# yifangao112/DinoUNet

Measured on AMD Instinct MI355X. Metric: 2D slices/sec training, dinounet_l 512x512 bf16, higher is better.
Workload: dtype bf16; 1 GPU; dinounet_l train step (fwd+loss+bwd+clip+SGD), 512x512x3 slices, batch 8/GPU, frozen ViT + adapter + FAPM + U-Net decoder, random-init weights; global_batch=8, parallelism=dp1

## Files before the change

### dinounet_amd/_build.py

```python
import hashlib
import os
import subprocess
import sys

HERE = os.path.dirname(os.path.abspath(__file__))
CSRC = os.path.join(HERE, "csrc")
LIB = os.path.join(HERE, "libdinounet_hip.so")
SOURCES = ["gemm.hip", "gemm_bf16.hip", "gemm_glds.hip", "gemm_p8.hip", "gemm_rk.hip", "gemm_skinny.hip", "conv_halo.hip", "conv_strip.hip", "attention.hip", "norm.hip", "norm_gemm.hip", "msda.hip", "elementwise.hip", "dwconv.hip", "loss.hip", "optim.hip", "augment.hip", "export.hip", "ensemble.hip", "surface.hip", "cc.hip", "preprocess.hip", "dataload.hip", "fingerprint.hip"]
FLAGS = ["--offload-arch=gfx950", "-O3", "-std=c++17", "-fPIC", "-munsafe-fp-atomics", "-fno-gpu-rdc"]
if os.environ.get("DINOUNET_DEBUG_KNOBS") == "1":
    FLAGS.append("-DDU_DEBUG_KNOBS")
EXTRA_FLAGS = {"attention.hip": ["-mllvm", "-amdgpu-mfma-vgpr-form"], "conv_strip.hip": ["-mllvm", "-amdgpu-mfma-vgpr-form"]}
NO_SCRATCH = ("gemm_bf16.hip", "gemm_glds.hip", "gemm_p8.hip", "gemm_rk.hip", "gemm_skinny.hip", "conv_halo.hip", "conv_strip.hip", "attention.hip", "norm_gemm.hip", "surface.hip", "dwconv.hip", "cc.hip", "preprocess.hip", "dataload.hip", "fingerprint.hip", "ensemble.hip")
REMARK = "-Rpass-analysis=kernel-resource-usage"
import re as _re
_ABLATION = _re.compile(
    r"attn_fwd_kernelILi\d+ELb1EEE"
    r"|attn_fwd_w64_kernelILi\d+ELi\d+ELb1E"
    r"|attn_fwd_w64_kernelILi\d+ELi\d+ELb\dELi\d+ELi[1-9]\d*ELi\d+EEE"
    r"|attn_fwd_pipe_kernelILb1ELi\d+EEE|attn_fwd_pipe_kernelILb\dELi[1-9]\d*EEE")


def _digest():
    h = hashlib.sha256()
    for f in sorted(os.listdir(CSRC)) + ["../../include/dinounet_hip.h"]:
        p = os.path.join(CSRC, f)
        if os.path.isfile(p):
            h.update(f.encode())
            h.update(open(p, "rb").read())
    h.update(" ".join(FLAGS).encode())
    h.update(repr(sorted(EXTRA_FLAGS.items())).encode())
    return h.hexdigest()


def build(force: bool = False, verbose: bool = True) -> str:
    stamp = LIB + ".stamp"
    dig = _digest()
    if not force and os.path.exists(LIB) and os.path.exists(stamp) and open(stamp).read() == dig:
        return LIB
    hipcc = os.environ.get("HIPCC", "/opt/rocm/bin/hipcc")
    objs, procs = [], []
    os.makedirs(os.path.join(HERE, "build"), exist_ok=True)
    for s in SOURCES:
        o = os.path.join(HERE, "build", s.replace(".hip", ".o"))
        objs.append(o)
        cmd = [hipcc, *FLAGS, *EXTRA_FLAGS.get(s, []), *([REMARK] if s in NO_SCRATCH else []), "-c", os.path.join(CSRC, s), "-o", o]
        if verbose:
            print("[dinounet_amd build]", " ".join(cmd), flush=True)
        procs.append((s, subprocess.Popen(cmd, stdout=subprocess.PIPE, stderr=subprocess.STDOUT)))
    for s, p in procs:
        out, _ = p.communicate()
        if p.returncode != 0:
            sys.stderr.write(out.decode())
            raise RuntimeError(f"hipcc failed on {s}")
        if s in NO_SCRATCH:
            name, spills = None, []
            for ln in out.decode().splitlines():
                if "Function Name:" in ln:
                    name = ln.split("Function Name:")[1].split("[")[0].strip()
                elif "ScratchSize [bytes/lane]:" in ln and int(ln.split("ScratchSize [bytes/lane]:")[1].split("[")[0]) > 0 and not _ABLATION.search(name or ""):
                    spills.append(f"{name} ({ln.split('ScratchSize [bytes/lane]:')[1].split('[')[0].strip()} B/lane)")
            if spills:
                raise RuntimeError(f"{s}: kernels spill to scratch: " + "; ".join(spills[:6]))
    cmd = [hipcc, "--offload-arch=gfx950", "-shared", "-fPIC", *objs, "-o", LIB]
    subprocess.check_call(cmd)
    und = subprocess.run(["nm", "-D", "--undefined-only", LIB], capture_output=True, text=True).stdout
    bad = [ln.split()[-1] for ln in und.splitlines() if "_GLOBAL__N_" in ln or ("_Z" in ln and "du_" in ln)]
    if bad:
        os.remove(LIB)
        raise RuntimeError("undefined file-local symbols in libdinounet_hip.so (dropped kernel stubs?): " + ", ".join(bad[:4]))
    open(stamp, "w").write(dig)
    return LIB


if __name__ == "__main__":
    print(build(force="--force" in sys.argv))
```

### dinounet_amd/csrc/gemm_p8.hip

```cpp
#include <algorithm>
#include <vector>
#include "common.h"
#include "gemm_params.h"
#include "gemm_plan.h"
#include "gemm_skinny_body.h"

namespace {

typedef __attribute__((address_space(3))) void lds_void;

constexpr int PBM = 256, PBN = 256, PBK = 64;
constexpr int HALF_B = 128 * PBK * 2;
constexpr int BUF_B = 4 * HALF_B;
constexpr int STG_LD = PBN + 4;

template <typename TC> struct Out4p;
template <> struct Out4p<float> {
  static __device__ __forceinline__ void load(const float* p, float* v) { float4 t = *(const float4*)p; v[0] = t.x; v[1] = t.y; v[2] = t.z; v[3] = t.w; }
  static __device__ __forceinline__ void store(float* p, const float* v) { *(float4*)p = make_float4(v[0], v[1], v[2], v[3]); }
};
template <> struct Out4p<bf16_t> {
  static __device__ __forceinline__ void load(const bf16_t* p, float* v) {
    bf16x4 t = __builtin_bit_cast(bf16x4, *(const uint2*)p);
#pragma unroll
    for (int j = 0; j < 4; j++) v[j] = (float)t[j];
  }
  static __device__ __forceinline__ void store(bf16_t* p, const float* v) {
    bf16x4 t;
#pragma unroll
    for (int j = 0; j < 4; j++) t[j] = (bf16_t)v[j];
    *(uint2*)p = __builtin_bit_cast(uint2, t);
  }
};

typedef unsigned u32x4_t __attribute__((ext_vector_type(4)));
template <int N> struct IC { static constexpr int value = N; };

__device__ __forceinline__ void wait_vm_count(int n) {
  switch (n) {
    case 12: asm volatile("s_waitcnt vmcnt(12)" ::: "memory"); break;
    case 10: asm volatile("s_waitcnt vmcnt(10)" ::: "memory"); break;
    case 8: asm volatile("s_waitcnt vmcnt(8)" ::: "memory"); break;
    case 6: asm volatile("s_waitcnt vmcnt(6)" ::: "memory"); break;
    case 4: asm volatile("s_waitcnt vmcnt(4)" ::: "memory"); break;
    case 2: asm volatile("s_waitcnt vmcnt(2)" ::: "memory"); break;
    default: asm volatile("s_waitcnt vmcnt(0)" ::: "memory"); break;
  }
}

__device__ __forceinline__ void tile_coords_of(const GemmParams& P, int nwg, int bid, int& tm, int& tn);
__device__ __forceinline__ void tile_coords(const GemmParams& P, int& tm, int& tn) {
  tile_coords_of(P, P.main_wgs ? P.main_wgs : (int)gridDim.x, blockIdx.x, tm, tn);
}
__device__ __forceinline__ void tile_coords_of(const GemmParams& P, int nwg, int bid, int& tm, int& tn) {
  const int q = nwg >> 3, r = nwg & 7, xcd = bid & 7, idx = bid >> 3;
  const int tile = (xcd < r ? xcd * (q + 1) : r * (q + 1) + (xcd - r) * q) + idx;
  if (P.group_m > 1) {
    const int band = P.group_m * P.tiles_n;
    const int g = tile / band, l = tile - g * band;
    const int first = g * P.group_m;
    const int gsz = min(P.tiles_m - first, P.group_m);
    tn = l / gsz; tm = first + (l - tn * gsz);
  } else {
    tm = tile / P.tiles_n; tn = tile - tm * P.tiles_n;
  }
}


typedef float f32x2 __attribute__((ext_vector_type(2)));
__device__ __forceinline__ f32x2 splat2(float c) { f32x2 r; r.x = c; r.y = c; return r; }
__device__ __forceinline__ f32x2 gelu_pk(f32x2 v) {
  f32x2 u, m, e;
  u.x = __builtin_amdgcn_fmed3f(fabsf(v.x), 0.f, 5.6f); u.y = __builtin_amdgcn_fmed3f(fabsf(v.y), 0.f, 5.6f);
  m.x = __builtin_amdgcn_fmed3f(v.x, 0.f, __builtin_inff()); m.y = __builtin_amdgcn_fmed3f(v.y, 0.f, __builtin_inff());
  f32x2 q = splat2(-1.99582904e-06f);
  q = q * u + splat2(6.48327432e-05f);
  q = q * u + splat2(-9.56180914e-04f);
  q = q * u + splat2(8.60978469e-03f);
  q = q * u + splat2(-5.41717858e-02f);
  q = q * u + splat2(-4.58246213e-01f);
  q = q * u + splat2(-1.15134465e+00f);
  q = q * u + splat2(-9.99985061e-01f);
  e.x = __builtin_amdgcn_exp2f(q.x); e.y = __builtin_amdgcn_exp2f(q.y);
  return m - u * e;
}

template <int ACT>
__device__ __forceinline__ void stage_block_bf16(const f32x16& a, const float4 (&bv)[4], bf16_t* stg, int ldb, int srow, int scol, int hi) {
#pragma unroll
  for (int g = 0; g < 4; g++) {
    float o[4] = {a[4 * g] + bv[g].x, a[4 * g + 1] + bv[g].y, a[4 * g + 2] + bv[g].z, a[4 * g + 3] + bv[g].w};
    if constexpr (ACT == DU_ACT_SWIGLU) {
      bf16x2 t;
      t[0] = (bf16_t)(o[0] * __builtin_amdgcn_rcpf(1.0f + __expf(-o[0])) * o[1]);
      t[1] = (bf16_t)(o[2] * __builtin_amdgcn_rcpf(1.0f + __expf(-o[2])) * o[3]);
      *(unsigned*)(stg + srow * ldb + ((scol + 8 * g + 4 * hi) >> 1)) = __builtin_bit_cast(unsigned, t);
    } else {
      if constexpr (ACT == DU_ACT_GELU) {
        f32x2 p0 = {o[0], o[1]}, p1 = {o[2], o[3]};
        p0 = gelu_pk(p0); p1 = gelu_pk(p1);
        o[0] = p0.x; o[1] = p0.y; o[2] = p1.x; o[3] = p1.y;
      }
      bf16x4 t;
#pragma unroll
      for (int e = 0; e < 4; e++) t[e] = (bf16_t)o[e];
      *(uint2*)(stg + srow * ldb + scol + 8 * g + 4 * hi) = __builtin_bit_cast(uint2, t);
    }
  }
}
__device__ __forceinline__ void stage_head_rope(const GemmParams& P, const f32x16& lo, const f32x16& hi_, const float4 (&blo)[4],
                                                const float4 (&bhi)[4], bf16_t* stg, int ldb, int srow, int scol, int hi, int m, int which) {
  const int b = m / P.ps_H, t = m - b * P.ps_H;
  const bool rot = which < 2 && t >= P.rope_prefix && m < P.M;
  const float qs = which == 0 ? P.rope_qscale : 1.0f;
  const long trow = rot ? (long)(t - P.rope_prefix) * 64 : 0;
#pragma unroll
  for (int g = 0; g < 4; g++) {
    const int d = 8 * g + 4 * hi;
    float x1[4] = {lo[4 * g] + blo[g].x, lo[4 * g + 1] + blo[g].y, lo[4 * g + 2] + blo[g].z, lo[4 * g + 3] + blo[g].w};
    float x2[4] = {hi_[4 * g] + bhi[g].x, hi_[4 * g + 1] + bhi[g].y, hi_[4 * g + 2] + bhi[g].z, hi_[4 * g + 3] + bhi[g].w};
    float o1[4], o2[4];
    if (rot) {
      const float4 c1 = *(const float4*)(P.rope_cos + trow + d), s1 = *(const float4*)(P.rope_sin + trow + d);
      const float4 c2 = *(const float4*)(P.rope_cos + trow + 32 + d), s2 = *(const float4*)(P.rope_sin + trow + 32 + d);
      const float cc1[4] = {c1.x, c1.y, c1.z, c1.w}, ss1[4] = {s1.x, s1.y, s1.z, s1.w};
      const float cc2[4] = {c2.x, c2.y, c2.z, c2.w}, ss2[4] = {s2.x, s2.y, s2.z, s2.w};
#pragma unroll
      for (int e = 0; e < 4; e++) { o1[e] = x1[e] * cc1[e] - x2[e] * ss1[e]; o2[e] = x2[e] * cc2[e] + x1[e] * ss2[e]; }
    } else {
#pragma unroll
      for (int e = 0; e < 4; e++) { o1[e] = x1[e]; o2[e] = x2[e]; }
    }
    bf16x4 t1, t2;
#pragma unroll
    for (int e = 0; e < 4; e++) { t1[e] = (bf16_t)(o1[e] * qs); t2[e] = (bf16_t)(o2[e] * qs); }
    *(uint2*)(stg + srow * ldb + scol + d) = __builtin_bit_cast(uint2, t1);
    *(uint2*)(stg + srow * ldb + scol + 32 + d) = __builtin_bit_cast(uint2, t2);
  }
}
__device__ __forceinline__ void load_bias4(const GemmParams& P, int ncol0, int hi, float4 (&bv)[4]) {
#pragma unroll
  for (int g = 0; g < 4; g++) {
    const int n = ncol0 + 8 * g + 4 * hi;
    bv[g] = P.bias ? *(const float4*)(P.bias + (n < P.N ? n : 0)) : make_float4(0.f, 0.f, 0.f, 0.f);
  }
}
__device__ __forceinline__ void stage_block_f32(const f32x16& a, float* stg, int ldf, int srow, int scol, int lane) {
  const int hi = lane >> 5;
#pragma unroll
  for (int g = 0; g < 4; g++)
    *(float4*)(stg + srow * ldf + scol + 8 * g + 4 * hi) = make_float4(a[4 * g], a[4 * g + 1], a[4 * g + 2], a[4 * g + 3]);
}
template <int TBN, bool QKV = false, int NTHR = 512>
__device__ __forceinline__ void readout_bf16(const GemmParams& P, const bf16_t* stg, int ldb, int nrows, int mrow0, int n0, int ncols,
                                             bf16_t* Cb, int tid) {
  constexpr int C8 = TBN / 8;
  const bool wide = ((((uintptr_t)Cb) & 15) == 0) && P.ldc % 8 == 0 && (QKV || P.store_mode == DU_STORE_PLAIN || P.ps_C % 8 == 0);
#pragma unroll 4
  for (int v = tid; v < nrows * C8; v += NTHR) {
    const int row = v / C8, c8 = v % C8;
    const int m = mrow0 + row, n = n0 + c8 * 8;
    if (m >= P.M || n >= ncols) continue;
    const uint4 t = *(const uint4*)(stg + row * ldb + c8 * 8);
    if ((P.dbg & 1) && t.x != 0x12345678u) continue;
    bf16_t* dst = Cb + (QKV ? qkv_heads_offset(P, m, n, P.ldc) : out_offset(P, m, n, P.ldc));
    if (wide && n + 8 <= ncols) *(uint4*)dst = t;
    else {
      *(uint2*)dst = make_uint2(t.x, t.y);
      if (n + 4 < ncols) *(uint2*)(dst + 4) = make_uint2(t.z, t.w);
    }
  }
}
template <typename TC, int W> struct RowVec;
template <> struct RowVec<float, 4> {
  static __device__ __forceinline__ void load(const float* p, float* v) { const float4 t = *(const float4*)p; v[0] = t.x; v[1] = t.y; v[2] = t.z; v[3] = t.w; }
  static __device__ __forceinline__ void store(float* p, const float* v) { *(float4*)p = make_float4(v[0], v[1], v[2], v[3]); }
};
template <> struct RowVec<bf16_t, 4> {
  static __device__ __forceinline__ void load(const bf16_t* p, float* v) { Out4p<bf16_t>::load(p, v); }
  static __device__ __forceinline__ void store(bf16_t* p, const float* v) { Out4p<bf16_t>::store(p, v); }
};
template <> struct RowVec<bf16_t, 8> {
  static __device__ __forceinline__ void load(const bf16_t* p, float* v) {
    const bf16x8 t = __builtin_bit_cast(bf16x8, *(const uint4*)p);
#pragma unroll
    for (int j = 0; j < 8; j++) v[j] = (float)t[j];
  }
  static __device__ __forceinline__ void store(bf16_t* p, const float* v) {
    bf16x8 t;
#pragma unroll
    for (int j = 0; j < 8; j++) t[j] = (bf16_t)v[j];
    *(uint4*)p = __builtin_bit_cast(uint4, t);
  }
};

template <typename TC, int TBN, int ACT, int W, int NTHR = 512>
__device__ __forceinline__ void readout_f32(const GemmParams& P, const float* stg, int ldf, int nrows, int mrow0, int n0, TC* Cb, const TC* Rb,
                                            int tid) {
  constexpr int CW = TBN / W, U = W == 8 ? 2 : 4;
  const int total = nrows * CW;
  for (int v0 = tid; v0 < total; v0 += NTHR * U) {
    float rr[U][W];
    bool live[U];
#pragma unroll
    for (int u = 0; u < U; u++) {
      const int v = v0 + u * NTHR;
      const int row = v / CW, cw = v % CW;
      const int m = mrow0 + row, n = n0 + cw * W;
      live[u] = v < total && m < P.M && n < P.N;
#pragma unroll
      for (int e = 0; e < W; e++) rr[u][e] = 0.f;
      if (Rb && live[u]) RowVec<TC, W>::load(Rb + out_offset(P, m, n, P.ldr), rr[u]);
    }
#pragma unroll
    for (int u = 0; u < U; u++) {
      if (!live[u]) continue;
      const int v = v0 + u * NTHR;
      const int row = v / CW, cw = v % CW;
      const int m = mrow0 + row, n = n0 + cw * W;
      float o[W];
#pragma unroll
      for (int h = 0; h < W / 4; h++) {
        const float4 tt = *(const float4*)(stg + row * ldf + cw * W + 4 * h);
        o[4 * h] = tt.x * P.alpha; o[4 * h + 1] = tt.y * P.alpha; o[4 * h + 2] = tt.z * P.alpha; o[4 * h + 3] = tt.w * P.alpha;
        if (P.bias) {
          const float4 bb = *(const float4*)(P.bias + n + 4 * h);
          o[4 * h] += bb.x; o[4 * h + 1] += bb.y; o[4 * h + 2] += bb.z; o[4 * h + 3] += bb.w;
        }
      }
      if constexpr (ACT == DU_ACT_GELU) {
#pragma unroll
        for (int e = 0; e < W; e++) o[e] = apply_act(o[e], DU_ACT_GELU);
      } else if constexpr (ACT < 0) {
#pragma unroll
        for (int e = 0; e < W; e++) o[e] = apply_act(o[e], P.act);
      }
      if (P.gamma) {
#pragma unroll
        for (int h = 0; h < W / 4; h++) {
          const float4 gg = *(const float4*)(P.gamma + n + 4 * h);
          o[4 * h] *= gg.x; o[4 * h + 1] *= gg.y; o[4 * h + 2] *= gg.z; o[4 * h + 3] *= gg.w;
        }
      }
      if (P.row_scale) {
        const float rs = P.row_scale[m / P.rs_rows];
#pragma unroll
        for (int e = 0; e < W; e++) o[e] *= rs;
      }
#pragma unroll
      for (int e = 0; e < W; e++) o[e] += rr[u][e];
      RowVec<TC, W>::store(Cb + out_offset(P, m, n, P.ldc), o);
    }
  }
}
struct ResidualTile { float4 r[16]; };
template <int TBN, int NTHR = 512>
__device__ __forceinline__ void residual_prefetch(const GemmParams& P, const float* Rb, int mrow0, int n0, int tid, ResidualTile& R) {
  constexpr int CW = TBN / 4;
#pragma unroll
  for (int u = 0; u < 16; u++) {
    const int v = tid + u * NTHR;
    const int m = mrow0 + v / CW, n = n0 + (v % CW) * 4;
    R.r[u] = (m < P.M && n < P.N) ? *(const float4*)(Rb + (long)m * P.ldr + n) : make_float4(0.f, 0.f, 0.f, 0.f);
  }
}
template <int TBN, int NTHR = 512>
__device__ __forceinline__ void readout_f32_prefetched(const GemmParams& P, const float* stg, int ldf, int mrow0, int n0, float* Cb, int tid,
                                                       const ResidualTile& R) {
  constexpr int CW = TBN / 4;
#pragma unroll
  for (int u = 0; u < 16; u++) {
    const int v = tid + u * NTHR;
    const int row = v / CW, cw = v % CW;
    const int m = mrow0 + row, n = n0 + cw * 4;
    if (m >= P.M || n >= P.N) continue;
    const float4 tt = *(const float4*)(stg + row * ldf + cw * 4);
    float o[4] = {tt.x * P.alpha, tt.y * P.alpha, tt.z * P.alpha, tt.w * P.alpha};
    if (P.bias) {
      const float4 bb = *(const float4*)(P.bias + n);
      o[0] += bb.x; o[1] += bb.y; o[2] += bb.z; o[3] += bb.w;
    }
    if (P.act != DU_ACT_NONE) {
#pragma unroll
      for (int e = 0; e < 4; e++) o[e] = apply_act(o[e], P.act);
    }
    if (P.gamma) {
      const float4 gg = *(const float4*)(P.gamma + n);
      o[0] *= gg.x; o[1] *= gg.y; o[2] *= gg.z; o[3] *= gg.w;
    }
    if (P.row_scale) {
      const float rs = P.row_scale[m / P.rs_rows];
#pragma unroll
      for (int e = 0; e < 4; e++) o[e] *= rs;
    }
    *(float4*)(Cb + (long)m * P.ldc + n) = make_float4(o[0] + R.r[u].x, o[1] + R.r[u].y, o[2] + R.r[u].z, o[3] + R.r[u].w);
  }
}
template <typename TC, int TBN, int NTHR = 512>
__device__ __forceinline__ void readout_f32_any(const GemmParams& P, const float* stg, int ldf, int nrows, int mrow0, int n0, TC* Cb,
                                                const TC* Rb, int tid) {
  if constexpr (sizeof(TC) == 2) {
    const bool w8 = P.N % 8 == 0 && P.ldc % 8 == 0 && ((((uintptr_t)Cb) & 15) == 0) && (!Rb || (P.ldr % 8 == 0 && ((((uintptr_t)Rb) & 15) == 0))) &&
                    (P.store_mode == DU_STORE_PLAIN || P.ps_C % 8 == 0);
    if (w8) {
      if (P.act == DU_ACT_NONE) readout_f32<TC, TBN, DU_ACT_NONE, 8, NTHR>(P, stg, ldf, nrows, mrow0, n0, Cb, Rb, tid);
      else readout_f32<TC, TBN, -1, 8, NTHR>(P, stg, ldf, nrows, mrow0, n0, Cb, Rb, tid);
      return;
    }
  }
  if (P.act == DU_ACT_NONE) readout_f32<TC, TBN, DU_ACT_NONE, 4, NTHR>(P, stg, ldf, nrows, mrow0, n0, Cb, Rb, tid);
  else if (P.act == DU_ACT_GELU) readout_f32<TC, TBN, DU_ACT_GELU, 4, NTHR>(P, stg, ldf, nrows, mrow0, n0, Cb, Rb, tid);
  else readout_f32<TC, TBN, -1, 4, NTHR>(P, stg, ldf, nrows, mrow0, n0, Cb, Rb, tid);
}
template <int NTHR = 512>
__device__ __forceinline__ void readout_msda_prep(const GemmParams& P, const float* stg, int ldf, int nrows, int mrow0, int tid) {
  const int Mh = P.N / 12, Lq = P.ps_C;
  const float invW = 1.0f / (float)P.ps_W, invH = 1.0f / (float)P.ps_H;
  float* loc = (float*)P.C;
  for (int v = tid; v < nrows * Mh; v += NTHR) {
    const int row = v / Mh, h = v - row * Mh;
    const int m = mrow0 + row;
    if (m >= P.M) continue;
    const int q = m % Lq;
    const float rx = P.rope_sin[q * 2], ry = P.rope_sin[q * 2 + 1];
    const float* so = stg + row * ldf + h * 8;
    const float* sl = stg + row * ldf + Mh * 8 + h * 4;
    float off[8], lg[4];
#pragma unroll
    for (int e = 0; e < 8; e++) off[e] = so[e] + (P.bias ? P.bias[h * 8 + e] : 0.f);
#pragma unroll
    for (int e = 0; e < 4; e++) lg[e] = sl[e] + (P.bias ? P.bias[Mh * 8 + h * 4 + e] : 0.f);
    const float mx = fmaxf(fmaxf(lg[0], lg[1]), fmaxf(lg[2], lg[3]));
    float ex[4], sm = 0.f;
#pragma unroll
    for (int e = 0; e < 4; e++) { ex[e] = expf(lg[e] - mx); sm += ex[e]; }
    const float inv = 1.f / sm;
    float* lo = loc + ((long)m * Mh + h) * 8;
    *(float4*)lo = make_float4(rx + off[0] * invW, ry + off[1] * invH, rx + off[2] * invW, ry + off[3] * invH);
    *(float4*)(lo + 4) = make_float4(rx + off[4] * invW, ry + off[5] * invH, rx + off[6] * invW, ry + off[7] * invH);
    *(float4*)(P.C2 + ((long)m * Mh + h) * 4) = make_float4(ex[0] * inv, ex[1] * inv, ex[2] * inv, ex[3] * inv);
  }
}
__device__ __forceinline__ bool bf16_simple(const GemmParams& P, const void* Rb) {
  return !Rb && !P.gamma && !P.row_scale && P.alpha == 1.0f && (P.act == DU_ACT_NONE || P.act == DU_ACT_GELU || P.act == DU_ACT_SWIGLU);
}

constexpr int P8_STG_LDB = PBN + 8;
constexpr int P8_STG_LDF = PBN + 4;
constexpr int P8_LDS = 256 * P8_STG_LDB * 2;

template <typename TC, int NW = 8, bool SL = false>
__device__ __forceinline__ void p8_tail(const GemmParams& P, unsigned char* smem, int unit = -1) {
  SkinnyEpi E;
  E.qkv_H = 0; E.qkv_N = 0; E.qkv_Npad = 0;
  E.C = (TC*)P.C + (long)P.M * P.ldc; E.ldc = P.ldc;
  if (P.store_mode == DU_STORE_QKV_HEADS) { E.C = P.C; E.qkv_H = P.ps_C; E.qkv_N = P.ps_H; E.qkv_Npad = P.ps_W; }
  E.residual = P.residual ? (const void*)((const TC*)P.residual + (long)P.M * P.ldr) : nullptr; E.ldr = P.ldr;
  E.bias = P.bias; E.gamma = P.gamma; E.row_scale = P.row_scale;
  E.alpha = P.alpha; E.act = P.act; E.rs_rows = P.rs_rows; E.out_bf16 = sizeof(TC) == 2; E.row0 = P.M;
  E.slices = 1; E.slice = 0; E.slab = nullptr; E.cnt = nullptr;
  int u = unit >= 0 ? unit : (int)blockIdx.x - P.main_wgs;
  int k0 = 0, klen = P.K;
  if (SL && P.tail_slices > 1) {
    const int cb = u / P.tail_slices;
    E.slices = P.tail_slices; E.slice = u - cb * P.tail_slices;
    klen = P.K / P.tail_slices; k0 = E.slice * klen;
    E.cnt = (int*)((char*)P.ks_ws + 65536) + cb;
    E.slab = (float*)((char*)P.ks_ws + 131072) + (long)cb * P.tail_slices * (64 * SK_BN);
    u = cb;
  }
  skinny_fused_body<NW, 2, SL, (NW == 8)>((const bf16_t*)P.a.p + (long)P.M * P.a.ld + k0, P.a.ld, (const bf16_t*)P.b.p + k0, P.b.ld, P.tail_rows, P.N, klen, E,
                       (float*)smem, u);
}

template <typename TC, int NW = 8>
__device__ __forceinline__ void p8_tail_inline(const GemmParams& P, unsigned char* smem, int w, int G) {
  const int nunits = (P.N + SK_BN - 1) / SK_BN;
  if (w >= nunits) return;
  asm volatile("s_waitcnt vmcnt(0)" ::: "memory");
  __syncthreads();
  for (int u = w; u < nunits; u += G) {
    p8_tail<TC, NW>(P, smem, u);
    __syncthreads();
  }
}

__device__ __forceinline__ int xcd_linear_index() {
  const int nwg = gridDim.x, bid = blockIdx.x;
  const int q = nwg >> 3, r = nwg & 7, xcd = bid & 7, idx = bid >> 3;
  return (xcd < r ? xcd * (q + 1) : r * (q + 1) + (xcd - r) * q) + idx;
}

template <typename TC, int SCHED, bool TN, bool GA, int GG = 0, bool KS = false>
__device__ __forceinline__ void p8_tile_body(const GemmParams& P, unsigned char* smem, const int lin) {
  static_assert(GG == 0 || ((GG == 2 || GG == 3) && TN && !GA), "general gather: weight-gradient form only");
  static_assert(!KS || (!TN && !GA && sizeof(TC) == 4), "K-split pairs: plain NT products with an fp32 result");
  const int tid = threadIdx.x, lane = tid & 63;
  const int wave = __builtin_amdgcn_readfirstlane(tid >> 6);
  const int wm = wave >> 2, wn = wave & 3;
  int tm, tn;
  int nk = P.K / PBK;
  long kbeg = 0;
  int my_split = 0;
  int ks_split = 0, ks_tile = 0, ks_kt0 = 0;
  if constexpr (TN) {
    const int ntiles = P.tiles_m * P.tiles_n;
    const int split = lin / ntiles, tile = lin - split * ntiles;
    tm = tile / P.tiles_n; tn = tile - tm * P.tiles_n;
    const int npairs = P.K / (2 * PBK), base = npairs / P.split_k, extra = npairs - base * P.split_k;
    const int first = split * base + min(split, extra);
    kbeg = (long)first * (2 * PBK);
    nk = 2 * (base + (split < extra ? 1 : 0));
    my_split = split;
  } else if constexpr (KS) {
    const int bid = blockIdx.x;
    ks_split = (bid >> 3) & 1;
    ks_tile = ((bid >> 4) << 3) | (bid & 7);
    tile_coords_of(P, P.main_wgs >> 1, ks_tile, tm, tn);
    nk >>= 1;
    ks_kt0 = ks_split * nk;
  } else {
    tile_coords(P, tm, tn);
  }
  const int m0 = tm * PBM, n0 = tn * PBN;
  const int batch = TN ? 0 : blockIdx.y;

  const bf16_t *Ab, *Bb;
  long abytes, bbytes;
  if constexpr (TN) {
    Ab = (const bf16_t*)P.a.p + (long)batch * P.a.bstride + kbeg * P.a.ld + m0;
    abytes = ((P.K - kbeg - 1) * P.a.ld + (P.M - m0)) * 2;
    if constexpr (GG != 0) {
      Bb = (const bf16_t*)P.b.p;
      bbytes = P.b.bstride;
      if constexpr (GG == 3) {
        Bb -= (long)(P.b.Wi + 1) * P.b.ld;
        bbytes += (long)(P.b.Wi + 1) * P.b.ld * 2;
      }
    } else if constexpr (GA) {
      const int tapn = n0 / P.b.C, co0 = n0 - tapn * P.b.C;
      const long off = ((long)(tapn >> 1) * P.b.Wi + (tapn & 1)) * P.b.ld + co0;
      Bb = (const bf16_t*)P.b.p + off;
      bbytes = ((long)(P.K / (P.b.Ho * P.b.Wo)) * P.b.Hi * P.b.Wi * P.b.ld - off) * 2;
    } else {
      Bb = (const bf16_t*)P.b.p + (long)batch * P.b.bstride + kbeg * P.b.ld + n0;
      bbytes = ((P.K - kbeg - 1) * P.b.ld + (P.N - n0)) * 2;
    }
  } else {
    if constexpr (GA) {
      Ab = (const bf16_t*)P.a.p;
      abytes = (long)(P.M / (P.a.Ho * P.a.Wo)) * P.a.Hi * P.a.Wi * P.a.ld * 2;
    } else {
      Ab = (const bf16_t*)P.a.p + (long)batch * P.a.bstride + (long)m0 * P.a.ld;
      abytes = ((long)(P.M - m0) * P.a.ld - (P.a.ld - P.K)) * 2;
    }
    Bb = (const bf16_t*)P.b.p + (long)batch * P.b.bstride + (long)n0 * P.b.ld;
    bbytes = ((long)(P.N - n0) * P.b.ld - (P.b.ld - P.K)) * 2;
  }
  if (abytes > 0x7fffffffL) abytes = 0x7fffffffL;
  if (bbytes > 0x7fffff00L) bbytes = 0x7fffff00L;
  const auto ra = __builtin_amdgcn_make_buffer_rsrc((void*)Ab, 0, (int)abytes, 0x00020000);
  const auto rb = __builtin_amdgcn_make_buffer_rsrc((void*)Bb, 0, (int)bbytes, 0x00020000);

  unsigned va[2][2], vb[2][2];
  unsigned kstep_a = PBK * 2, kstep_b = PBK * 2;
  if constexpr (TN) {
    kstep_a = (unsigned)(P.a.ld * 2 * PBK); kstep_b = (unsigned)(P.b.ld * 2 * PBK);
    const int r4 = lane >> 4, lc = (lane & 15) ^ (4 * r4);
#pragma unroll
    for (int h = 0; h < 2; h++)
#pragma unroll
      for (int r = 0; r < 2; r++) {
        const int krow = (r * 8 + wave) * 4 + r4;
        va[h][r] = (unsigned)krow * (unsigned)(P.a.ld * 2) + (h * 128 + lc * 8) * 2;
        vb[h][r] = (unsigned)krow * (unsigned)(P.b.ld * 2) + (h * 128 + lc * 8) * 2;
      }
  } else {
    const int sw = ((wave & 1) << 2) | (lane >> 4);
    const int lc = (lane & 7) ^ sw;
#pragma unroll
    for (int h = 0; h < 2; h++)
#pragma unroll
      for (int r = 0; r < 2; r++) {
        const int row = h * 128 + (r * 8 + wave) * 8 + (lane >> 3);
        if constexpr (GA) {
          const int m = min(m0 + row, P.M - 1);
          const int xo = m % P.a.Wo, t2 = m / P.a.Wo, yo = t2 % P.a.Ho, bb = t2 / P.a.Ho;
          va[h][r] = (unsigned)(((bb * P.a.Hi + 2 * yo) * P.a.Wi + 2 * xo)) * (unsigned)(P.a.ld * 2) + lc * 16;
        } else {
          va[h][r] = (unsigned)row * (unsigned)(P.a.ld * 2) + lc * 16;
        }
        vb[h][r] = (unsigned)row * (unsigned)(P.b.ld * 2) + lc * 16;
      }
  }
  int logW = 0;
  if constexpr ((GA || GG != 0) && TN) logW = __builtin_ctz(P.b.Wo);
  int g_off[2] = {1, 1};
  unsigned g_pv[2][2] = {{0u, 0u}, {0u, 0u}};
  unsigned g_mask = 0u;
  const unsigned g_ldb = (unsigned)(P.b.ld * 2);
  if constexpr (GG != 0) {
    const int r4 = lane >> 4, lc = (lane & 15) ^ (4 * r4);
#pragma unroll
    for (int h = 0; h < 2; h++) {
      const int col0 = n0 + h * 128, tap0 = col0 / P.b.C, ci0 = col0 - tap0 * P.b.C;
      const int ld = (int)P.b.ld;
      int ci = ci0 + lc * 8, tap = tap0;
      while (ci >= P.b.C) { ci -= P.b.C; tap++; }
      const bool exists = col0 + lc * 8 < P.N;
      if constexpr (GG == 2) {
        g_off[h] = exists ? (((tap >> 1) * P.b.Wi + (tap & 1)) * ld + ci) * 2 : 1;
      } else {
        const int ty = tap / 3, tx = tap - ty * 3;
#pragma unroll
        for (int r = 0; r < 2; r++) {
          const int lr = (r * 8 + wave) * 4 + r4;
          g_pv[h][r] = exists ? (unsigned)(((lr + ty * P.b.Wi + tx) * ld + ci) * 2) : 0x7fffff00u;
          const unsigned bits = (ty == 0 ? 1u : 0u) | (ty == 2 ? 2u : 0u) | ((tx == 0 && lr == 0) ? 4u : 0u) | ((tx == 2 && lr == 63) ? 8u : 0u);
          g_mask |= bits << (4 * (2 * h + r));
        }
      }
    }
  }
  const unsigned lds_base = (unsigned)(unsigned long long)(__attribute__((address_space(3))) unsigned char*)smem;
  auto stage = [&](auto which_c, auto buf_c, int kt) {
    constexpr int which = decltype(which_c)::value, buf = decltype(buf_c)::value;
    constexpr int h = which & 1;
    unsigned soff = (KS ? kt + ks_kt0 : kt) * (which < 2 ? kstep_a : kstep_b);
    if constexpr (GA && !TN && which < 2) {
      const int k = kt * PBK, tap = k >> P.a.logC, within = k - (tap << P.a.logC);
      soff = (unsigned)((((tap >> 1) * P.a.Wi + (tap & 1)) * (int)P.a.ld + within) * 2);
    }
    if constexpr ((GA || GG == 2) && TN && which >= 2) soff = 0;
    unsigned tile_bits = 0u;
    if constexpr (GG == 3 && which >= 2) {
      const int p0 = (int)kbeg + kt * PBK;
      const int x0 = p0 & (P.b.Wo - 1), y = (p0 >> logW) & (P.b.Ho - 1);
      soff = (unsigned)p0 * g_ldb;
      tile_bits = (y == 0 ? 1u : 0u) | (y == P.b.Ho - 1 ? 2u : 0u) | (x0 == 0 ? 4u : 0u) | (x0 + PBK == P.b.Wo ? 8u : 0u);
    }
#pragma unroll
    for (int r = 0; r < 2; r++) {
      unsigned voff = which < 2 ? va[h][r] : vb[h][r];
      if constexpr (GG == 3 && which >= 2) {
        voff = ((g_mask >> (4 * (2 * h + r))) & tile_bits) ? 0x7fffff00u : g_pv[h][r];
      }
      if constexpr (GG == 2 && which >= 2) {
        const int krow = (int)kbeg + kt * PBK + (r * 8 + wave) * 4 + (lane >> 4);
        const int x = krow & (P.b.Wo - 1), yy = krow >> logW;
        const int bp = 4 * (yy << logW) + 2 * x;
        voff = g_off[h] != 1 ? (unsigned)bp * g_ldb + (unsigned)g_off[h] : 0x7fffff00u;
      }
      if constexpr (GA && TN && which >= 2) {
        const int r4 = lane >> 4, lc = (lane & 15) ^ (4 * r4);
        const int krow = (int)kbeg + kt * PBK + (r * 8 + wave) * 4 + r4;
        const int yy = krow >> logW, x = krow & (P.b.Wo - 1);
        voff = (unsigned)(2 * yy * P.b.Wi + 2 * x) * (unsigned)(P.b.ld * 2) + (h * 128 + lc * 8) * 2;
      }
      unsigned char* dst = smem + buf * BUF_B + which * HALF_B + (r * 8 + wave) * 1024;
      if constexpr (TN) {
        const unsigned lds_dst = __builtin_amdgcn_readfirstlane(lds_base + buf * BUF_B + which * HALF_B + (r * 8 + wave) * 1024);
        unsigned keep;
        const auto srd = which < 2 ? ra : rb;
        asm volatile("s_mov_b32 %0, m0\n\ts_mov_b32 m0, %4\n\ts_nop 0\n\tbuffer_load_dwordx4 %1, %2, %3 offen lds\n\ts_mov_b32 m0, %0"
                     : "=&s"(keep) : "v"(voff), "s"(srd), "s"(soff), "s"(lds_dst) : "memory");
      } else {
        if constexpr (which < 2) __builtin_amdgcn_raw_ptr_buffer_load_lds(ra, (lds_void*)dst, 16, voff, soff, 0, 0);
        else __builtin_amdgcn_raw_ptr_buffer_load_lds(rb, (lds_void*)dst, 16, voff, soff, 0, 0);
      }
    }
  };

  int L[4];
  int LT[3];
  const int aoff = wm * 64 * 128, boff = wn * 32 * 128;
  if constexpr (TN) {
    const int g = lane >> 4, p = lane & 15, r4 = p >> 2;
    const int common = (g >> 1) * 2048 + r4 * 256 + (2 * (g & 1) + ((p >> 1) & 1)) * 16 + (p & 1) * 8;
    LT[0] = common + (((wm * 2 + 0) ^ r4) << 6);
    LT[1] = common + (((wm * 2 + 1) ^ r4) << 6);
    LT[2] = common + ((wn ^ r4) << 6);
  } else {
    const int x = (lane >> 5) ^ ((lane >> 1) & 7);
#pragma unroll
    for (int kk = 0; kk < 4; kk++) L[kk] = (lane & 31) * 128 + ((x ^ (2 * kk)) << 4);
  }
  auto tr_frag = [&](const unsigned char* q) -> bf16x8 {
    typedef short s16x4_t __attribute__((ext_vector_type(4)));
    typedef short s16x8_t __attribute__((ext_vector_type(8)));
    typedef __attribute__((address_space(3))) s16x4_t lds_v4;
    s16x4_t lo = __builtin_amdgcn_ds_read_tr16_b64_v4i16((lds_v4*)q);
    s16x4_t hi = __builtin_amdgcn_ds_read_tr16_b64_v4i16((lds_v4*)(q + 1024));
    s16x8_t v = __builtin_shufflevector(lo, hi, 0, 1, 2, 3, 4, 5, 6, 7);
    return __builtin_bit_cast(bf16x8, v);
  };

  bf16x8 Af[2][2][4];
  bf16x8 Bf[2][4];
  f32x16 acc[2][2][2];
#pragma unroll
  for (int i = 0; i < 2; i++)
#pragma unroll
    for (int j = 0; j < 2; j++)
#pragma unroll
      for (int b = 0; b < 2; b++)
#pragma unroll
        for (int r = 0; r < 16; r++) acc[i][j][b][r] = 0.f;

  auto readA = [&](auto set_c, auto buf_c) {
    constexpr int set = decltype(set_c)::value, buf = decltype(buf_c)::value;
#pragma unroll
    for (int b = 0; b < 2; b++)
#pragma unroll
      for (int kk = 0; kk < 4; kk++) {
        if constexpr (TN) Af[set][b][kk] = tr_frag(smem + buf * BUF_B + set * HALF_B + kk * 4096 + LT[b]);
        else Af[set][b][kk] = *(const bf16x8*)(smem + buf * BUF_B + set * HALF_B + aoff + b * 4096 + L[kk]);
      }
  };
  auto readB = [&](auto set_c, auto half_c, auto buf_c) {
    constexpr int set = decltype(set_c)::value, half = decltype(half_c)::value, buf = decltype(buf_c)::value;
#pragma unroll
    for (int kk = 0; kk < 4; kk++) {
      if constexpr (TN) Bf[set][kk] = tr_frag(smem + buf * BUF_B + (2 + half) * HALF_B + kk * 4096 + LT[2]);
      else Bf[set][kk] = *(const bf16x8*)(smem + buf * BUF_B + (2 + half) * HALF_B + boff + L[kk]);
    }
  };
  auto mma = [&](auto i_c, auto j_c, auto bset_c) {
    constexpr int i = decltype(i_c)::value, j = decltype(j_c)::value, bset = decltype(bset_c)::value;
#pragma unroll
    for (int kk = 0; kk < 4; kk++)
#pragma unroll
      for (int b = 0; b < 2; b++) {
        if constexpr (TN) acc[i][j][b] = __builtin_amdgcn_mfma_f32_32x32x16_bf16(Af[i][b][kk], Bf[bset][kk], acc[i][j][b], 0, 0, 0);
        else acc[i][j][b] = __builtin_amdgcn_mfma_f32_32x32x16_bf16(Bf[bset][kk], Af[i][b][kk], acc[i][j][b], 0, 0, 0);
      }
  };
  const bool colsum_on = TN && P.a_colsum != nullptr && wn == 0 && tn == my_split % P.tiles_n;
  float csum[2][2] = {{0.f, 0.f}, {0.f, 0.f}};
  auto colsum_acc = [&](auto i_c) {
    constexpr int i = decltype(i_c)::value;
    if constexpr (TN) {
      if (colsum_on) {
#pragma unroll
// ... 1733 lines not shown
```

### dinounet_amd/ops.py

```python
import ctypes as C
import math
import os
import weakref

import torch

from . import _lib
from ._lib import (ACT_GELU, ACT_LEAKY, ACT_NONE, ACT_RELU, ACT_SWIGLU, DU_BF16, DU_F32, IM2COL_COL, IM2COL_ROW, PLAIN_COL,
                   PLAIN_ROW, STORE_MSDA_PREP, STORE_PIXEL_SHUFFLE2, STORE_QKV_HEADS, STORE_QKV_ROPE, STORE_SLABS, ConvGeom, GemmArgs)

__all__ = ["mm", "linear", "conv2d", "conv_transpose2x2", "norm_act", "layer_norm", "msda", "dwconv3x3",
           "maxpool3x3s2", "bilinear_add", "bilinear_resize", "squeeze_excite", "dice_ce_loss", "dice_ce_masked_loss", "dice_bce_loss",
           "labels_to_regions", "val_dice_ce", "val_dice_bce"]


def _code(dt):
    if dt == torch.bfloat16:
        return DU_BF16
    if dt == torch.float32:
        return DU_F32
    raise RuntimeError(f"dinounet_amd: unsupported dtype {dt} (bf16 / fp32 only)")


def _req(*ts):
    for t in ts:
        if t is not None and not t.is_cuda:
            raise RuntimeError("dinounet_amd ops run on the GPU through libdinounet_hip.so only (no CPU fallback); "
                               "got a CPU tensor")


def _p(t):
    return None if t is None else C.c_void_p(t.data_ptr())


def _st():
    return C.c_void_p(torch.cuda.current_stream().cuda_stream)


def _f32(t):
    if t is None:
        return None
    return t if (t.dtype == torch.float32 and t.is_contiguous()) else t.float().contiguous()


def _rows2d(t):
    assert t.dim() == 2 and t.stride(1) == 1, (t.shape, t.stride())
    return t.shape[0], t.shape[1], t.stride(0)


def _nhwc(t):
    assert t.dim() == 4 and t.stride(3) == 1, (t.shape, t.stride())
    B, H, W, Cc = t.shape
    ld = t.stride(2)
    assert (H == 1 or t.stride(1) == W * ld) and (B == 1 or t.stride(0) == H * W * ld), (t.shape, t.stride())
    return B, H, W, Cc, ld


class KernelProfile:

    def __init__(self, detail=False):
        self.rec = []
        self.detail = detail

    def start(self):
        e = torch.cuda.Event(enable_timing=True)
        e.record()
        return e

    def stop(self, name, e0, flops, nbytes):
        e1 = torch.cuda.Event(enable_timing=True)
        e1.record()
        self.rec.append((name, e0, e1, flops, nbytes))

    def roofline(self, peak_tflops, peak_gbs, steps):
        torch.cuda.synchronize()
        agg = {}
        for name, e0, e1, fl, nb in self.rec:
            a = agg.setdefault(name, [0.0, 0, 0.0, 0.0])
            a[0] += e0.elapsed_time(e1) * 1e-3
            a[1] += 1
            a[2] += fl
            a[3] += nb
        rows = sorted(agg.items(), key=lambda kv: -kv[1][0])
        brk = [{"kernel": k, "launches_per_step": round(v[1] / steps, 1), "ms_per_step": round(v[0] / steps * 1e3, 3),
                "tflops": round(v[2] / v[0] / 1e12, 1), "gbs": round(v[3] / v[0] / 1e9, 1)} for k, v in rows[:12]]
        k, v = rows[0]
        mfma_frac = v[2] / v[0] / 1e12 / peak_tflops
        hbm_frac = v[3] / v[0] / 1e9 / peak_gbs
        if mfma_frac >= hbm_frac:
            roof = {"kernel": k, "bound": "mfma", "achieved": round(v[2] / v[0] / 1e12, 2), "peak": peak_tflops, "unit": "TFLOP/s",
                    "frac": round(mfma_frac, 4), "traffic": None, "avg_launch_us": round(v[0] / v[1] * 1e6, 2)}
        else:
            roof = {"kernel": k, "bound": "hbm", "achieved": round(v[3] / v[0] / 1e9, 1), "peak": peak_gbs, "unit": "GB/s",
                    "frac": round(hbm_frac, 4), "traffic": None, "avg_launch_us": round(v[0] / v[1] * 1e6, 2)}
        return roof, brk


PROFILE = None


CAPTURE_CUT = None
SMALL_COLLECTIVES = None


_FORCE_SMALL = os.environ.get("DINOUNET_FORCE_SMALL_COLLECTIVES") == "1"


def sync_active(group=None):
    d = torch.distributed
    if not (d.is_available() and d.is_initialized()):
        return False
    return d.get_world_size(group) > 1 or _FORCE_SMALL


def _small_all_reduce(t, group, what):
    capturing = t.is_cuda and torch.cuda.is_current_stream_capturing()
    if capturing and CAPTURE_CUT is not None:
        CAPTURE_CUT(lambda: torch.distributed.all_reduce(t, group=group), what)
        return
    rec = SMALL_COLLECTIVES is not None and t.is_cuda and not capturing
    if rec:
        e0 = torch.cuda.Event(enable_timing=True)
        e0.record()
    torch.distributed.all_reduce(t, group=group)
    if rec:
        e1 = torch.cuda.Event(enable_timing=True)
        e1.record()
        SMALL_COLLECTIVES.append((what, e0, e1))
_MODE_NAMES = {(0, 0): "linear", (0, 1): "linear_dgrad", (1, 1): "linear_wgrad", (2, 0): "conv_im2col", (1, 3): "conv_wgrad"}


_ROUTE_NAMES = {0: "gemm_kernel", 1: "gemm_bf16_kernel", 2: "gemm_nt_glds_kernel", 3: "gemm_nt_p8_kernel", 4: "gemm_nt_p8n_kernel", 5: "gemm_tn_p8_kernel",
                6: "gemm_nt_pp_kernel", 7: "gemm_nt_rk_kernel", 8: "gemm_nt_p8ks_kernel"}


_AB_KNOBS = os.environ.get("DINOUNET_AB_KNOBS") == "1"


def _ab_env(name, default):
    return os.environ.get(name, default) if _AB_KNOBS else default


_WGRAD_COLSUM = _ab_env("DINOUNET_WGRAD_COLSUM", "1") == "1"
_KSCALE = _ab_env("DINOUNET_WGRAD_KSCALE", "1") == "1"


def gemm_route(**kw):
    return gemm_raw(route_only=True, **kw)


TRACK_ROUTE = False
LAST_GEMM_ROUTE = -1
ROUTES = []


_KS_PAIRS = _ab_env("DINOUNET_KS_PAIRS", "1") == "1"
_KS_SCRATCH = {}
_KS_RETIRED = []
_KS_NEED = 4 << 20


def _ks_scratch(nbytes, stream=None):
    global _KS_NEED
    _KS_NEED = max(_KS_NEED, nbytes)
    st = torch.cuda.current_stream() if stream is None else stream
    key = (st.device.index, st.cuda_stream)
    buf = _KS_SCRATCH.get(key)
    if buf is None or buf.numel() < nbytes:
        if torch.cuda.is_current_stream_capturing():
            return None
        if buf is not None:
            _KS_RETIRED.append(buf)
        buf = torch.empty(_KS_NEED, dtype=torch.uint8, device=torch.device("cuda", key[0]))
        buf[:131072].zero_()
        if stream is not None:
            torch.cuda.current_stream().synchronize()
        _KS_SCRATCH[key] = buf
    return buf


def ks_scratch_prepare(stream):
    assert not torch.cuda.is_current_stream_capturing()
    return _ks_scratch(_KS_NEED, stream)


def capture(graph, **kw):
    ctx = torch.cuda.graph(graph, **kw)
    ks_scratch_prepare(ctx.capture_stream)
    return ctx


def gemm_raw(*, dtype, out_dtype, a_mode, b_mode, M, N, K, A, lda, B, ldb, Cmat, ldc, batch=1, abs_=0, bbs=0, cbs=0,
             split_k=1, alpha=1.0, bias=None, act=ACT_NONE, gamma=None, row_scale=None, rs_rows=0, residual=None, ldr=0,
             store_mode=0, ps=(0, 0, 0), geom=None, a_colsum=None, b_colsum=None, rope=None, c2=None, route_only=False):
    a = GemmArgs()
    a.dtype, a.out_dtype, a.a_mode, a.b_mode = dtype, out_dtype, a_mode, b_mode
    a.M, a.N, a.K = M, N, K
    a.A, a.lda, a.a_batch_stride = A, lda, abs_
    a.B, a.ldb, a.b_batch_stride = B, ldb, bbs
    a.C, a.ldc, a.c_batch_stride = Cmat, ldc, cbs
    a.batch, a.split_k, a.alpha = batch, split_k, alpha
    a.bias = bias
    a.act = act
    a.gamma = gamma
    a.row_scale, a.rs_rows = row_scale, rs_rows
    a.residual, a.ldr = residual, ldr
    a.store_mode = store_mode
    a.ps_H, a.ps_W, a.ps_C = ps
    if geom is not None:
        a.geom = geom
    a.a_colsum = a_colsum
    a.b_colsum = b_colsum
    a.C2 = c2
    if rope is not None:
        a.rope_sin, a.rope_cos, a.rope_prefix, a.rope_qscale = rope
    if route_only:
        return int(_lib.lib().du_gemm_route(C.byref(a)))
    ws = None
    if dtype == DU_BF16 and a_mode == PLAIN_ROW and b_mode == PLAIN_ROW and M >= 1024 and 0 < M % 128 <= 64:
        n_ws = int(_lib.lib().du_gemm_ws_elems(C.byref(a)))
        if n_ws > 0:
            ws = torch.empty(n_ws, dtype=torch.float32, device=torch.device("cuda", torch.cuda.current_device()))
            a.ws, a.ws_elems = ws.data_ptr(), n_ws
    if _KS_PAIRS and dtype == DU_BF16 and a_mode == PLAIN_ROW and b_mode == PLAIN_ROW and store_mode == 0 and M >= 1024 and K >= 1024 and (
            out_dtype == DU_F32 or 0 < M % 256 <= 64):
        n_ks = int(_lib.lib().du_gemm_ks_ws_bytes(C.byref(a)))
        if n_ks > 0:
            ks = _ks_scratch(n_ks)
            if ks is not None:
                a.ks_ws, a.ks_ws_bytes = ks.data_ptr(), n_ks
    global LAST_GEMM_ROUTE
    if TRACK_ROUTE:
        LAST_GEMM_ROUTE = int(_lib.lib().du_gemm_route(C.byref(a)))
        ROUTES.append((a_mode, b_mode, LAST_GEMM_ROUTE))
    if PROFILE is not None:
        e0 = PROFILE.start()
        _lib.check(_lib.lib().du_gemm(C.byref(a), _st()), "du_gemm")
        es = 2 if dtype == DU_BF16 else 4
        eo = 2 if out_dtype == DU_BF16 else 4
        kin = K if geom is None else K // max(geom.KH * geom.KW, 1) if a_mode == IM2COL_ROW else K
        kname = _ROUTE_NAMES[int(_lib.lib().du_gemm_route(C.byref(a)))]
        mode = _MODE_NAMES.get((a_mode, b_mode), 'other')
        if residual is not None and out_dtype == DU_BF16:
            mode += "+res"
        tag = f"{kname}<{'bf16' if dtype == DU_BF16 else 'f32'},{mode}>"
        if PROFILE.detail:
            tag += f" M{M} N{N} K{K} b{batch} sk{split_k}" + (f" k{geom.KH}s{geom.stride}t{geom.transposed}" if geom is not None else "")
        PROFILE.stop(tag, e0,
                     2.0 * M * N * K * batch, float(batch) * (M * kin * es + N * K * es + M * N * eo * (2 if residual is not None else 1)))
        return
    _lib.check(_lib.lib().du_gemm(C.byref(a), _st()), "du_gemm")


def set_corun(n):
    _lib.check(_lib.lib().du_set_option(9, int(n)), "du_set_option(9)")


def _dp(t):
    return None if t is None else t.data_ptr()



PK_CAST, PK_CONV_FWD, PK_CONV_DGRAD, PK_CONV_DGRAD_FLIP, PK_CONVT_FWD, PK_CONVT_DGRAD, PK_TRANSPOSE = 0, 1, 2, 3, 4, 5, 6


class WeightPack:

    def __init__(self):
        self.enabled = _ab_env("DINOUNET_WEIGHT_PACK", "1") != "0"
        self.entries = {}
        self.order = []
        self.dirty = False
        self.table = None
        self.prefix = None
        self.total = 0
        self.nbuilt = 0

    @staticmethod
    def _shape(srcs, kind, cp):
        w = srcs[0]
        if kind == PK_CAST:
            rows = sum(t.shape[0] for t in srcs)
            return (rows,) + tuple(w.flatten(1).shape[1:]) if w.dim() > 1 else (rows,)
        if kind == PK_CONV_FWD:
            return (w.shape[0], w.shape[2] * w.shape[3] * cp)
        if kind in (PK_CONV_DGRAD, PK_CONV_DGRAD_FLIP):
            return (w.shape[1], w.shape[2] * w.shape[3] * w.shape[0])
        if kind == PK_CONVT_FWD:
            return (4 * w.shape[1], w.shape[0])
        if kind == PK_CONVT_DGRAD:
            return (w.shape[0], 4 * w.shape[1])
        if kind == PK_TRANSPOSE:
            return (w.flatten(1).shape[1], sum(t.shape[0] for t in srcs))
        raise ValueError(kind)

    @staticmethod
    def _base(t):
        return t._base if t._base is not None else t

    def get(self, srcs, kind, dt=torch.bfloat16, cp=0):
        if not self.enabled:
            return None
        if torch.is_tensor(srcs):
            srcs = (srcs,)
        w = srcs[0]
        if not w.is_cuda or w.dtype != torch.float32 or dt not in (torch.bfloat16, torch.float32):
            return None
        for t in srcs:
            bt = self._base(t)
            if not (t.is_contiguous() and bt.is_leaf and isinstance(bt, torch.nn.Parameter)):
                return None
        if kind == PK_CONV_FWD and cp == 0:
            cp = w.shape[1]
        key = (tuple(t.data_ptr() for t in srcs), tuple(w.shape), kind, dt, cp)
        e = self.entries.get(key)
        if e is not None and any(r() is None for r in e["refs"]):
            self._drop(key)
            e = None
        if e is None:
            dst = torch.zeros(self._shape(srcs, kind, cp), dtype=dt, device=w.device)
            e = {"key": key, "refs": [weakref.ref(self._base(t)) for t in srcs], "ptrs": [t.data_ptr() for t in srcs],
                 "nels": [t.numel() for t in srcs], "wshape": tuple(w.shape), "dst": dst, "kind": kind, "cp": cp, "vers": None,
                 "built": False}
            self.entries[key] = e
            self.order.append(e)
            self.dirty = True
            return None
        if not e["built"] or e["vers"] != tuple(r()._version for r in e["refs"]):
            return None
        return e["dst"]

    def invalidate(self):
        for e in self.order:
            e["vers"] = None

    def _drop(self, key):
        e = self.entries.pop(key, None)
        if e is not None:
            self.order = [x for x in self.order if x is not e]
            self.dirty = True

    def refresh(self):
        if not self.enabled or not self.order:
            return
        capturing = torch.cuda.is_current_stream_capturing()
        if not capturing:
            for e in [x for x in self.order if any(r() is None for r in x["refs"])]:
                self._drop(e["key"])
        if self.dirty and not capturing:
            if not self.order:
                self.table = None
                return
            rows, prefix, tot = [], [0], 0
            dev = self.order[0]["dst"].device
            for e in self.order:
                off = 0
                k = e["kind"]
                ws = e["wshape"]
                for ptr, nel in zip(e["ptrs"], e["nels"]):
                    if k == PK_CAST:
                        A, B, T, Cp, n = 0, 0, 0, 0, nel
                    elif k == PK_TRANSPOSE:
                        rows_i = nel // e["dst"].shape[0]
                        A, B, T, Cp, n = rows_i, e["dst"].shape[0], (e["dst"].shape[1] if len(e["ptrs"]) > 1 else 0), 0, nel
                    elif k in (PK_CONV_FWD, PK_CONV_DGRAD, PK_CONV_DGRAD_FLIP):
                        A, B, T, Cp, n = ws[0], ws[1], ws[2] * ws[3], e["cp"], e["dst"].numel()
                    else:
                        A, B, T, Cp, n = ws[0], ws[1], 4, 0, e["dst"].numel()
                    rows.append([ptr, e["dst"].data_ptr() + off * e["dst"].element_size(),
                                 k | ((1 if e["dst"].dtype == torch.float32 else 0) << 8), A, B, T, Cp, n])
                    off += A if (k == PK_TRANSPOSE and T) else n
                    tot += ((A + 63) // 64) * ((B + 63) // 64) if k == PK_TRANSPOSE else (n + 4095) // 4096
                    prefix.append(tot)
                e["built"] = True
            self.table = torch.tensor(rows, dtype=torch.int64).to(dev)
            self.prefix = torch.tensor(prefix, dtype=torch.int64).to(dev)
            self.total, self.nbuilt, self.dirty = tot, len(rows), False
        if self.table is None:
            return
        _lib.check(_lib.lib().du_pack_weights(_p(self.table), _p(self.prefix), self.nbuilt, self.total, _st()), "du_pack_weights")
        for e in self.order:
            if e["built"]:
                e["vers"] = tuple((r()._version if r() is not None else -1) for r in e["refs"])


PACK = WeightPack()

def mm(x, w, *, out=None, out_dtype=None, bias=None, act=ACT_NONE, gamma=None, residual=None, row_scale=None,
       rs_rows=0, alpha=1.0):
    _req(x, w)
    M, K, lda = _rows2d(x)
    N, K2, ldb = _rows2d(w)
    assert K == K2 and x.dtype == w.dtype, (x.shape, w.shape, x.dtype, w.dtype)
    od = out_dtype or (out.dtype if out is not None else x.dtype)
    if out is None:
        out = torch.empty((M, N), dtype=od, device=x.device)
    _, _, ldc = _rows2d(out)
    ldr = 0
    if residual is not None:
        assert residual.dtype == out.dtype
        ldr = residual.stride(0)
    gemm_raw(dtype=_code(x.dtype), out_dtype=_code(out.dtype), a_mode=PLAIN_ROW, b_mode=PLAIN_ROW, M=M, N=N, K=K,
             A=x.data_ptr(), lda=lda, B=w.data_ptr(), ldb=ldb, Cmat=out.data_ptr(), ldc=ldc, alpha=alpha,
             bias=_dp(bias), act=act, gamma=_dp(gamma), row_scale=_dp(row_scale), rs_rows=rs_rows,
             residual=_dp(residual), ldr=ldr)
    return out


def interleave_pairs(w1, w2):
    return torch.stack((w1, w2), dim=1).reshape((2 * w1.shape[0],) + tuple(w1.shape[1:])).contiguous()


def mm_swiglu(x, w12, b12=None):
    _req(x, w12)
    M, K, lda = _rows2d(x)
    N2, K2, ldb = _rows2d(w12)
    assert K == K2 and N2 % 2 == 0 and x.dtype == w12.dtype
    h = N2 // 2
    out = torch.empty((M, h), dtype=x.dtype, device=x.device)
    if x.dtype == torch.bfloat16:
        a = GemmArgs()
        a.dtype = a.out_dtype = DU_BF16
        a.a_mode = a.b_mode = PLAIN_ROW
        a.M, a.N, a.K = M, N2, K
        a.A, a.lda, a.B, a.ldb, a.C, a.ldc = x.data_ptr(), lda, w12.data_ptr(), ldb, out.data_ptr(), h
        a.batch, a.split_k, a.alpha, a.act = 1, 1, 1.0, ACT_SWIGLU
        a.bias = _dp(b12)
        e0 = PROFILE.start() if PROFILE is not None else None
        rc = _lib.lib().du_gemm(C.byref(a), _st())
        if rc == 0:
            if PROFILE is not None:
                PROFILE.stop("gemm_nt_p8_kernel<bf16,swiglu>", e0, 2.0 * M * N2 * K, 2.0 * (M * K + N2 * K + M * h))
            return out
        if rc != -2:
            _lib.check(rc, "du_gemm (swiglu)")
    u = mm(x, w12, bias=b12)
    _lib.check(_lib.lib().du_swiglu_pairs(_code(x.dtype), _p(u), _p(out), M, h, _st()), "du_swiglu_pairs")
    return out


def sample_gather(x, idx):
    _req(x, idx)
    assert x.dtype == torch.float32 and x.is_contiguous() and idx.dtype == torch.int64
    n = x[0].numel()
    out = torch.empty((idx.numel(),) + tuple(x.shape[1:]), dtype=torch.float32, device=x.device)
    _lib.check(_lib.lib().du_sample_copy(_p(x), _p(out), _p(idx), idx.numel(), n, 0, _st()), "du_sample_copy")
    return out


def sample_scatter_(x, src, idx):
    _req(x, src, idx)
    assert x.dtype == torch.float32 and src.dtype == torch.float32 and x.is_contiguous() and src.is_contiguous()
    _lib.check(_lib.lib().du_sample_copy(_p(src), _p(x), _p(idx), idx.numel(), x[0].numel(), 1, _st()), "du_sample_copy")
    return x


def mm_dgrad(dy, w, out=None):
    _req(dy, w)
    M, N, lda = _rows2d(dy)
    N2, K, ldb = _rows2d(w)
    assert N == N2 and dy.dtype == w.dtype
    if out is None:
        out = torch.empty((M, K), dtype=dy.dtype, device=dy.device)
    gemm_raw(dtype=_code(dy.dtype), out_dtype=_code(out.dtype), a_mode=PLAIN_ROW, b_mode=PLAIN_COL, M=M, N=K, K=N,
             A=dy.data_ptr(), lda=lda, B=w.data_ptr(), ldb=ldb, Cmat=out.data_ptr(), ldc=out.stride(0))
    return out


class ZeroPool:
    ALIGN = 64

    def __init__(self):
        self.enabled = _ab_env("DINOUNET_ZERO_POOL", "1") != "0"
        self.plan = None
        self.rec = []
        self._reset()

    def _reset(self):
        self.buf = None
        self.idx = 0
        self.off = 0
        self.ok = True

    def new_step(self):
        if self.rec:
            self.plan = self.rec
        self.rec = []
        self._reset()

    def zeros(self, shape, device):
        n = 1
        for d in shape:
            n *= int(d)
        if not self.enabled:
            return torch.zeros(shape, dtype=torch.float32, device=device)
        self.rec.append(n)
        if self.ok and self.plan is not None and self.idx < len(self.plan) and self.plan[self.idx] == n and \
                (self.buf is None or self.buf.device == device):
            if self.buf is None:
                if self.idx != 0:
                    self.ok = False
                    return torch.zeros(shape, dtype=torch.float32, device=device)
                total = sum((m + self.ALIGN - 1) // self.ALIGN * self.ALIGN for m in self.plan)
                self.buf = torch.zeros(total, dtype=torch.float32, device=device)
            v = self.buf[self.off:self.off + n].view(shape)
            self.off += (n + self.ALIGN - 1) // self.ALIGN * self.ALIGN
            self.idx += 1
            return v
        self.ok = False
        return torch.zeros(shape, dtype=torch.float32, device=device)


ZEROS = ZeroPool()

_SPLIT_TARGET = int(_ab_env("DU_SPLIT_TARGET", "0"))
_SPLIT_MINK = int(_ab_env("DU_SPLIT_MINK", "1024"))


def _split_for(tiles, kdim, target=512):
    s = max(1, min((_SPLIT_TARGET or target) // max(tiles, 1), kdim // _SPLIT_MINK))
    return max(1, s)


class WgradQueue:

    trace = None

    def __init__(self):
        self.enabled = os.environ.get("DINOUNET_WGRAD_DEFER", "1") != "0"
        self.jobs = []
        self.keep = []
        self.flops = 0.0
        self.nbytes = 0.0
        self._armed_task = None
        self.keep_bytes = 0
        self.keep_limit = int(os.environ.get("DINOUNET_WGRAD_KEEP_MB", "16384")) << 20
        self.state = {}
        self.groups = {}
        self.flush_aware_hooks = 0
        self.launches = 0
        self.queued = 0

    @staticmethod
    def _param(w):
        b = w._base if w._base is not None else w
        if not (isinstance(b, torch.nn.Parameter) and b.is_leaf):
            return None
        if w is not b and not (w.numel() == b.numel() and w.is_contiguous() and b.is_contiguous()):
            return None
        return b

    def note_use(self, *ws):
        if not self.enabled:
            return None
        if getattr(torch.nn.parallel.DistributedDataParallel, "_active_ddp_module", None) is not None:
            return None
        ps = [self._param(w) for w in ws]
        if any(p is None for p in ps):
            return None
        return [weakref.ref(p) for p in ps]

    def _arm(self):
        tid = torch._C._current_graph_task_id()
        if tid == -1:
            return False
        if self._armed_task != tid:
            if self._armed_task is not None:
                self._armed_task = None
                self.flush()
            try:
                torch.autograd.Variable._execution_engine.queue_callback(self._end_of_pass)
            except RuntimeError:
                return False
            self._armed_task = tid
        return True

    def _drop(self):
        self.jobs, self.keep, self.flops, self.nbytes, self.keep_bytes = [], [], 0.0, 0.0, 0
        self.groups.clear()
        self.state.clear()
        self._armed_task = None

    def reset(self):
        self._drop()

    def _hand_over(self, ids):
        for i in ids:
            key = self.state.get(i)
            if key not in (None, "done") and self.groups.get(key, {}).get("jobs"):
                self.flush()
                break
        for i in ids:
            key = self.state.get(i)
            if key not in (None, "done"):
                self.groups.pop(key, None)
            self.state[i] = "done"

    def begin(self, refs):
        if not self.enabled or refs is None:
            return None
        ps = [r() for r in refs]
        if any(p is None for p in ps) or not self._arm():
            return None
        ids = tuple(id(p) for p in ps)
        ok = True
        for p in ps:
            if p.grad is not None or p._backward_hooks:
                ok = False
            if getattr(p, "_post_accumulate_grad_hooks", None) and not self.flush_aware_hooks:
                ok = False
        if not ok or any(self.state.get(i) not in (None, ids) for i in ids):
            self._hand_over(ids)
            return None
        grp = self.groups.get(ids)
        if grp is None:
            grp = {"key": ids, "bufs": {}, "jobs": [], "first": True, "ret": True, "refs": list(refs)}
            self.groups[ids] = grp
            for i in ids:
                self.state[i] = ids
        else:
            grp["first"] = grp["ret"] = False
            for j in grp["jobs"]:
                j.accumulate = 1
        return grp

    def abort(self, grp):
        self._hand_over(grp["key"])
        self.groups.pop(grp["key"], None)
        grp["ret"] = True

    def buffer(self, grp, name, shape, device):
        if grp is None:
            return ZEROS.zeros(shape, device)
        t = grp["bufs"].get(name)
        if t is None:
            t = grp["bufs"][name] = ZEROS.zeros(shape, device)
        return t.view(t.shape)

    def legal(self, job):
        return bool(_lib.lib().du_gemm_tn_group_legal(C.byref(job)))

    def add(self, job, keep, grp=None):
        if grp is not None:
            if not grp["first"]:
                job.accumulate = 1
            grp["jobs"].append(job)
        self.jobs.append(job)
        self.keep.extend(keep)
        self.keep_bytes += sum(t.numel() * t.element_size() for t in keep)
        self.queued += 1
        self.flops += 2.0 * job.M * job.N * job.K
        self.nbytes += 2.0 * job.K * (job.M + job.N) + 4.0 * job.M * job.N
        if not self._arm():
            self.flush()
        elif self.keep_bytes > self.keep_limit:
            self.flush()

    def _end_of_pass(self):
        self._armed_task = None
        self.flush()
        self.state.clear()
        self.groups.clear()

    def flush(self):
        done = []
        for ids, grp in list(self.groups.items()):
            if not grp["jobs"]:
                continue
            for i in ids:
                self.state[i] = "done"
            done.append(self.groups.pop(ids))
        if not self.jobs:
            return
        n = len(self.jobs)
        arr = (_lib.TnJob * n)(*self.jobs)
        if self.trace is not None:
            self.trace.append([(int(j.gather), int(j.M), int(j.N), int(j.K), bool(j.alpha), int(j.accumulate)) for j in self.jobs])
        e0 = PROFILE.start() if PROFILE is not None else None
        rc = _lib.lib().du_gemm_tn_group(arr, n, _st())
        fl, nb = self.flops, self.nbytes
        self.jobs, self.keep, self.flops, self.nbytes, self.keep_bytes = [], [], 0.0, 0.0, 0
        _lib.check(rc, "du_gemm_tn_group")
        self.launches += 1
        for grp in done:
            refs = grp.get("refs", ())
            if len(refs) > 2:
                continue
            for name, r in zip(("dw", "db"), refs):
                buf, p = grp["bufs"].get(name), r()
                if buf is None or p is None or p.grad is None or p.grad.numel() != buf.numel():
                    continue
                if p.grad.untyped_storage().data_ptr() != buf.untyped_storage().data_ptr():
                    p.grad.add_(buf.view(p.grad.shape).to(p.grad.dtype))
        if PROFILE is not None:
            PROFILE.stop("gemm_tn_group_kernel<bf16,wgrad>" + (f" jobs{n}" if PROFILE.detail else ""), e0, fl, nb)


WGRAD = WgradQueue()


def _pow2(v):
    return v > 0 and (v & (v - 1)) == 0


def _queue_conv_wgrad(grp, kind, a, lda, srcs, dyB, Hs, Ws, M, w_shape, want_bias):
    K = dyB * Hs * Ws
    taps = 9 if kind == 3 else 4
    ctot = sum(c for _, _, c in srcs)
# ... 72 lines not shown

def _reduce_ws(dt, G, P, Cc, device):
    n = int(_lib.lib().du_reduce_ws_elems(_code(dt), G, P, Cc))
    return torch.empty(max(n, 1), dtype=torch.float32, device=device), n


def colsum(x2d):
    rows, Cc, ld = _rows2d(x2d)
    out = torch.empty(Cc, dtype=torch.float32, device=x2d.device)
    ws, n = _reduce_ws(x2d.dtype, 1, rows, Cc, x2d.device)
    _lib.check(_lib.lib().du_colsum(_code(x2d.dtype), _p(x2d), ld, _p(out), rows, Cc, _p(ws), n, _st()), "du_colsum")
    return out


def _geom(src, KH, KW, stride, pad, Ho, Wo, transposed, src2=None):
    B, Hi, Wi, C1, ld = _nhwc(src)
    g = ConvGeom()
    Ct = C1
    if src2 is not None:
        B2, H2, W2, C2, ld2 = _nhwc(src2)
        assert (B2, H2, W2) == (B, Hi, Wi) and src2.dtype == src.dtype
        g.p2, g.ld2 = src2.data_ptr(), ld2
        Ct = C1 + C2
    g.C1 = C1
    g.Hi, g.Wi, g.C = Hi, Wi, Ct
    g.KH, g.KW, g.stride, g.pad = KH, KW, stride, pad
    g.Ho, g.Wo, g.transposed = Ho, Wo, transposed
    return g, B, ld, Ct


def pack_conv_weight(w, dt):
    return w.permute(0, 2, 3, 1).reshape(w.shape[0], -1).to(dt).contiguous()


def pack_conv_weight_dgrad(w, dt):
    return w.permute(1, 2, 3, 0).reshape(w.shape[1], -1).to(dt).contiguous()


def pack_conv_weight_dgrad_flipped(w, dt):
    return w.flip(2, 3).permute(1, 2, 3, 0).reshape(w.shape[1], -1).to(dt).contiguous()


def conv3x3_halo(x, wp, bias, x2=None, want_stats=False):
    if x.dtype != torch.bfloat16:
        return None
    B, H, W, C1, ld = _nhwc(x)
    Cout, Kc, ldb = _rows2d(wp)
    Cin = Kc // 9
    if ldb != Kc or Kc != 9 * Cin:
        return None
    C2, ld2 = _nhwc(x2)[3:] if x2 is not None else (0, 0)
    if C1 + C2 != Cin or (x2 is not None and x2.shape[:3] != x.shape[:3]):
        return None
    p2 = _p(x2)
    y = torch.empty((B, H, W, Cout), dtype=x.dtype, device=x.device)
    L, plan = _lib.lib(), (C.c_int64 * 4)()
    L.du_conv3x3_plan_describe(_p(x), ld, p2, ld2, C1, Cin, Cout, B, H, W, _p(wp), _p(y), Cout, 1 if want_stats else 0, plan, 4)
    rc, kernel, _, nparts = plan
    if rc == -2:
        return None
    _lib.check(rc, "du_conv3x3_plan_describe")
    part = torch.empty((nparts, Cout, 2), dtype=torch.float32, device=x.device) if nparts else None
    e0 = PROFILE.start() if PROFILE is not None else None
    _lib.check(L.du_conv3x3_halo(_p(x), ld, p2, ld2, C1, Cin, Cout, B, H, W, _p(wp), _p(bias), _p(y), Cout, _p(part), _st()), "du_conv3x3_halo")
    if PROFILE is not None:
        kname = "conv3x3_strip_kernel<bf16>" if kernel == 1 else ("conv3x3_halo_kernel<bf16>" if Cout <= 64 else "conv3x3_halo_c128_kernel<bf16>")
        PROFILE.stop(kname + (f" {H}x{W} {Cin}->{Cout}" if PROFILE.detail else ""), e0,
                     2.0 * B * H * W * Cin * Cout * 9, 2.0 * B * H * W * (Cin + Cout))
    return y, part


_CONV_SPLITK = _ab_env("DINOUNET_CONV_SPLITK", "1") == "1"


def _im2col_split(M, N, K):
    tiles = ((M + 127) // 128) * ((N + 127) // 128)
    if not _CONV_SPLITK or tiles > 128 or K < 1024 or N % 4:
        return 0
    return max(2, min(8, 256 // tiles, K // 256))


def _conv_splitk(sk, M, N, K, a, lda, w, ldb, g, out):
    slabs = torch.empty((sk, M, N), dtype=torch.float32, device=a.device)
    kw = dict(dtype=DU_BF16, out_dtype=DU_F32, a_mode=IM2COL_ROW, b_mode=PLAIN_ROW, M=M, N=N, K=K, A=a.data_ptr(), lda=lda,
              B=w.data_ptr(), ldb=ldb, Cmat=slabs.data_ptr(), ldc=N, split_k=sk, store_mode=STORE_SLABS, geom=g)
    if gemm_route(**kw) != 1:
        return False
    used = int(_lib.lib().du_gemm_slab_count(K, sk))
    gemm_raw(**kw)
    _lib.check(_lib.lib().du_splitk_reduce_bf16(_p(slabs), _p(out), used, M * N, _st()), "du_splitk_reduce_bf16")
    return True


def conv_fwd(x, wp, bias, KH, KW, stride, pad, x2=None, out=None, act=ACT_NONE):
    _req(x, wp)
    if KH == 3 and KW == 3 and stride == 1 and pad == 1 and out is None and act == ACT_NONE:
        r = conv3x3_halo(x, wp, bias, x2)
        if r is not None:
            return r[0]
    B, Hi, Wi, _, _ = _nhwc(x)
    Ho = (Hi + 2 * pad - KH) // stride + 1
    Wo = (Wi + 2 * pad - KW) // stride + 1
    g, B, ld, Ct = _geom(x, KH, KW, stride, pad, Ho, Wo, 0, x2)
    Cout, Kc, ldb = _rows2d(wp)
    assert Kc == KH * KW * Ct and wp.dtype == x.dtype, (wp.shape, KH, KW, Ct)
    if out is None:
        out = torch.empty((B, Ho, Wo, Cout), dtype=x.dtype, device=x.device)
    _, _, _, _, ldc = _nhwc(out)
    sk = _im2col_split(B * Ho * Wo, Cout, Kc) if (x.dtype == torch.bfloat16 and bias is None and act == ACT_NONE and out.is_contiguous()) else 0
    if sk and _conv_splitk(sk, B * Ho * Wo, Cout, Kc, x, ld, wp, ldb, g, out):
        return out
    gemm_raw(dtype=_code(x.dtype), out_dtype=_code(out.dtype), a_mode=IM2COL_ROW, b_mode=PLAIN_ROW, M=B * Ho * Wo, N=Cout,
             K=Kc, A=x.data_ptr(), lda=ld, B=wp.data_ptr(), ldb=ldb, Cmat=out.data_ptr(), ldc=ldc, bias=_dp(bias), act=act,
             geom=g)
    return out


def conv_dgrad(dy, wd, KH, KW, stride, pad, Hin, Win, out=None):
    _req(dy, wd)
    g, B, ld, Cout = _geom(dy, KH, KW, stride, pad, Hin, Win, 1)
    Cin, Kc, ldb = _rows2d(wd)
    assert Kc == KH * KW * Cout
    if out is None:
        out = torch.empty((B, Hin, Win, Cin), dtype=dy.dtype, device=dy.device)
    _, _, _, _, ldc = _nhwc(out)
    sk = _im2col_split(B * Hin * Win, Cin, Kc) if (dy.dtype == torch.bfloat16 and out.is_contiguous()) else 0
    if sk and _conv_splitk(sk, B * Hin * Win, Cin, Kc, dy, ld, wd, ldb, g, out):
        return out
    gemm_raw(dtype=_code(dy.dtype), out_dtype=_code(out.dtype), a_mode=IM2COL_ROW, b_mode=PLAIN_ROW, M=B * Hin * Win, N=Cin,
             K=Kc, A=dy.data_ptr(), lda=ld, B=wd.data_ptr(), ldb=ldb, Cmat=out.data_ptr(), ldc=ldc, geom=g)
    return out


def _wgrad3x3_args(x, dy, x2):
    B, H, W, C1, ld = _nhwc(x)
    C2, ld2 = _nhwc(x2)[3:] if x2 is not None else (0, 0)
    return _p(x), ld, _p(x2), ld2, C1, C1 + C2, dy.shape[-1], B, H, W, _p(dy), _nhwc(dy)[4]


def conv3x3_wgrad_plan(x, dy, x2=None):
    plan = (C.c_int64 * 4)(-2)
    if x.dtype == torch.bfloat16 and dy.shape[1:3] == x.shape[1:3]:
        _lib.lib().du_conv3x3_wgrad_plan_describe(*_wgrad3x3_args(x, dy, x2), plan, 4)
    return plan


def conv3x3_wgrad_halo(x, dy, x2=None, with_db=False, plan=None):
    rc, kernel, _, blocks = plan if plan is not None else conv3x3_wgrad_plan(x, dy, x2)
    if rc == -2:
        return None
    _lib.check(rc, "du_conv3x3_wgrad_plan_describe")
    args = _wgrad3x3_args(x, dy, x2)
    Cin, Cout, B, H, W = args[5:10]
    nel = Cout * 9 * Cin + (Cout if with_db else 0)
    part = torch.empty((blocks, nel), dtype=torch.float32, device=x.device)
    out = torch.empty(nel, dtype=torch.float32, device=x.device)
    dw = out[:Cout * 9 * Cin].view(Cout, 9 * Cin)
    e0 = PROFILE.start() if PROFILE is not None else None
    _lib.check(_lib.lib().du_conv3x3_wgrad_halo(*args, _p(part), _p(out), 1 if with_db else 0, _st()), "du_conv3x3_wgrad_halo")
    if PROFILE is not None:
        wk = "conv3x3_wgrad_rows_kernel<bf16>" if kernel == 1 else "conv3x3_wgrad_halo_kernel<bf16>"
        PROFILE.stop(wk + (f" {H}x{W} {Cin}->{Cout}" if PROFILE.detail else ""), e0,
                     2.0 * B * H * W * Cin * Cout * 9, 2.0 * B * H * W * (Cin + Cout))
    return (dw, out[Cout * 9 * Cin:]) if with_db else dw


def conv_wgrad(x, dy, KH, KW, stride, pad, x2=None, with_db=False, plan3x3=None):
    _req(x, dy)
    if KH == 3 and KW == 3 and stride == 1 and pad == 1:
        r = conv3x3_wgrad_halo(x, dy, x2, with_db and _WGRAD_COLSUM, plan3x3)
        if r is not None:
            if with_db and not _WGRAD_COLSUM:
                return r, colsum(dy.view(-1, dy.shape[-1]))
            return r
    Bo, Ho, Wo, Cout, lddy = _nhwc(dy)
    g, B, ld, Ct = _geom(x, KH, KW, stride, pad, Ho, Wo, 0, x2)
    Ncol = KH * KW * Ct
    out = ZEROS.zeros((Cout, Ncol), x.device)
    npix = B * Ho * Wo
    tiles = ((Cout + 127) // 128) * ((Ncol + 127) // 128)
    kw = dict(dtype=_code(x.dtype), out_dtype=DU_F32, a_mode=PLAIN_COL, b_mode=IM2COL_COL, M=Cout, N=Ncol, K=npix,
              A=dy.data_ptr(), lda=lddy, B=x.data_ptr(), ldb=ld, Cmat=out.data_ptr(), ldc=Ncol,
              split_k=_split_for(tiles, npix, 1024), geom=g)
    if not with_db:
        gemm_raw(**kw)
        return out
    if _WGRAD_COLSUM and x.dtype == torch.bfloat16 and gemm_route(**kw) == 1:
        db = ZEROS.zeros((Cout,), x.device)
        gemm_raw(a_colsum=db.data_ptr(), **kw)
        return out, db
    gemm_raw(**kw)
    return out, colsum(dy.view(-1, dy.shape[-1]))


_STATS32 = _ab_env("DINOUNET_CONV_STATS32", "1") != "0"


class _Conv2d(torch.autograd.Function):

    @staticmethod
    def forward(ctx, x, x2, w, bias, stride, pad, want_stats):
        KH, KW = w.shape[2], w.shape[3]
        wp = PACK.get(w, PK_CONV_FWD, x.dtype)
        if wp is None:
            wp = pack_conv_weight(w, x.dtype)
        part = None
        r = None
        if KH == 3 and KW == 3 and stride == 1 and pad == 1:
            r = conv3x3_halo(x, wp, _f32(bias), x2, want_stats and (w.shape[0] >= 64 or _STATS32))
        if r is not None:
            y, part = r
        else:
            y = conv_fwd(x, wp, _f32(bias), KH, KW, stride, pad, x2)
        ctx.save_for_backward(x, x2, w)
        ctx.conf = (KH, KW, stride, pad, bias is not None)
        ctx.wrefs = WGRAD.note_use(*([w] if bias is None else [w, bias]))
        if part is None:
            part = torch.empty(0, device=x.device)
        ctx.mark_non_differentiable(part)
        ctx.set_materialize_grads(False)
        return y, part

    @staticmethod
    def backward(ctx, dy, _dpart):
        x, x2, w = ctx.saved_tensors
        KH, KW, stride, pad, has_bias = ctx.conf
        dy = dy.contiguous()
        B, Hi, Wi, C1, _ = _nhwc(x)
        dx = dx2 = dw = db = None
        need_dx = ctx.needs_input_grad[0] or (x2 is not None and ctx.needs_input_grad[1])
        if need_dx:
            done = False
            if KH == 3 and KW == 3 and stride == 1 and pad == 1 and dy.dtype == torch.bfloat16:
                wf = PACK.get(w, PK_CONV_DGRAD_FLIP, dy.dtype)
                if wf is None:
                    wf = pack_conv_weight_dgrad_flipped(w, dy.dtype)
                if x2 is None:
                    r = conv3x3_halo(dy, wf, None)
                    if r is not None:
                        dx, done = r[0], True
                else:
                    r1 = conv3x3_halo(dy, wf[:C1], None)
                    r2 = conv3x3_halo(dy, wf[C1:], None) if r1 is not None else None
                    if r1 is not None and r2 is not None:
                        dx, dx2, done = r1[0], r2[0], True
            if not done:
                wd = PACK.get(w, PK_CONV_DGRAD, dy.dtype)
                if wd is None:
                    wd = pack_conv_weight_dgrad(w, dy.dtype)
                dfull = conv_dgrad(dy, wd, KH, KW, stride, pad, Hi, Wi)
                if x2 is None:
                    dx = dfull
                else:
                    dx, dx2 = dfull[..., :C1], dfull[..., C1:]
        want_db = has_bias and ctx.needs_input_grad[3]
        if ctx.needs_input_grad[2]:
            r = None
            Bo, Ho, Wo, Cout, lddy = _nhwc(dy)
            wplan = conv3x3_wgrad_plan(x, dy, x2) if (KH, KW, stride, pad) == (3, 3, 1, 1) else None
            if wplan is not None and dy.dtype == torch.bfloat16 and wplan[0] != 0 and _pow2(Hi) and _pow2(Wi) and (_WGRAD_COLSUM or not want_db):
                grp = WGRAD.begin(ctx.wrefs)
                if grp is not None:
                    srcs = [(x, _nhwc(x)[4], C1)] + ([(x2, _nhwc(x2)[4], x2.shape[-1])] if x2 is not None else [])
                    r = _queue_conv_wgrad(grp, 3, dy, lddy, srcs, B, Hi, Wi, Cout, tuple(w.shape), want_db)
                    if r is None:
                        WGRAD.abort(grp)
                    elif not grp["ret"]:
                        r = (None, None)
            if r is not None:
                dw, db = r
            else:
                g = conv_wgrad(x, dy, KH, KW, stride, pad, x2, with_db=want_db, plan3x3=wplan)
                if want_db:
                    g, db = g
                dw = g.view(w.shape[0], KH, KW, w.shape[1]).permute(0, 3, 1, 2).contiguous()
        elif want_db:
            db = colsum(dy.view(-1, dy.shape[-1]))
        return dx, dx2, dw, db, None, None, None


def conv2d(x, w, bias=None, stride=1, pad=1, x2=None):
    return _Conv2d.apply(x, x2, w, bias, stride, pad, False)[0]


def conv2d_stats(x, w, bias=None, stride=1, pad=1, x2=None):
    y, part = _Conv2d.apply(x, x2, w, bias, stride, pad, True)
    return y, (part if part.numel() else None)


_DGRAD_NT = _ab_env("DINOUNET_DGRAD_NT", "1") == "1"


class _Linear(torch.autograd.Function):

    @staticmethod
    def forward(ctx, x, w, bias, residual, row_scale, rs_rows, out_dtype):
        wq = w
        if w.dtype != x.dtype:
            wq = PACK.get(w, PK_CAST, x.dtype)
            if wq is None:
                wq = w.to(x.dtype)
            elif wq.dim() != 2:
                wq = wq.view(w.shape[0], -1)
        y = mm(x, wq, bias=_f32(bias), residual=residual, row_scale=row_scale, rs_rows=rs_rows, out_dtype=out_dtype)
        ctx.wT = PACK.get(w, PK_TRANSPOSE, x.dtype) if (_DGRAD_NT and w.dtype != x.dtype and w.shape[0] % 64 == 0) else None
        ctx.save_for_backward(x, wq, row_scale)
        ctx.wrefs = WGRAD.note_use(*([w] if bias is None else [w, bias]))
        ctx.rs_rows = rs_rows
        ctx.has_bias = bias is not None
        ctx.has_res = residual is not None
        return y

    @staticmethod
    def backward(ctx, dy):
        x, wq, row_scale = ctx.saved_tensors
        dres = dy if ctx.has_res else None
        dyc = dy if dy.stride(1) == 1 else dy.contiguous()
        if dyc.dtype != x.dtype:
            dyc = cast(dyc, x.dtype)
        ks = None
        if row_scale is not None:
            if _KSCALE and dyc.dtype == torch.bfloat16 and ctx.rs_rows % 64 == 0 and ctx.wT is not None:
                ks = (row_scale, ctx.rs_rows)
            else:
                dyc = (dyc.view(row_scale.numel(), ctx.rs_rows, -1) * row_scale.view(-1, 1, 1).to(dyc.dtype)).view(dyc.shape)
        dx = None
        if ctx.needs_input_grad[0]:
            if ctx.wT is not None:
                dx = mm(dyc, ctx.wT, row_scale=ks[0], rs_rows=ks[1]) if ks is not None else mm(dyc, ctx.wT)
            else:
                dx = mm_dgrad(dyc, wq)
        dw = db = None
        want_db = ctx.has_bias and ctx.needs_input_grad[2]
        if ctx.needs_input_grad[1]:
            grp = WGRAD.begin(ctx.wrefs)
            if want_db:
                dw, db = mm_wgrad(dyc, x, with_colsum=True, k_scale=ks, defer=grp)
            else:
                dw = mm_wgrad(dyc, x, k_scale=ks, defer=grp)
            if grp is not None and not grp["ret"]:
                dw = db = None
        elif want_db:
            dys = dyc if ks is None else (dyc.view(row_scale.numel(), ctx.rs_rows, -1) * row_scale.view(-1, 1, 1).to(dyc.dtype)).view(dyc.shape)
            db = colsum(dys)
        return dx, dw, db, dres, None, None, None


def linear(x, w, bias=None, residual=None, row_scale=None, rs_rows=0, out_dtype=None):
    shp = x.shape
    x2 = x.reshape(-1, shp[-1])
    r2 = residual.reshape(-1, residual.shape[-1]) if residual is not None else None
    y = _Linear.apply(x2, w, bias, r2, row_scale, rs_rows, out_dtype)
    return y.view(*shp[:-1], w.shape[0])


class _LinearCat(torch.autograd.Function):

    @staticmethod
    def forward(ctx, x, w1, w2, b1, b2, out_dtype):
        y = _linear_cat_fwd(ctx, x, w1, w2, b1, b2, out_dtype)
        ctx.save_for_backward(*ctx.lc_saved)
        ctx.lc_saved = None
        return y

    @staticmethod
    def backward(ctx, dy):
        x = ctx.saved_tensors[0]
        dyc = dy if dy.stride(1) == 1 else dy.contiguous()
        if dyc.dtype != x.dtype:
            dyc = cast(dyc, x.dtype)
        return (*_linear_cat_bwd(ctx, dyc), None)


def _linear_cat_fwd(ctx, x, w1, w2, b1, b2, out_dtype, product=None):
    n1 = w1.shape[0]
    wq = PACK.get((w1.reshape(n1, -1), w2.reshape(w2.shape[0], -1)), PK_CAST, x.dtype)
    if wq is None:
        wq = torch.cat([w1.reshape(n1, -1), w2.reshape(w2.shape[0], -1)], 0).to(x.dtype)
    bq = None
    if b1 is not None:
        bq = PACK.get((b1, b2), PK_CAST, torch.float32)
        if bq is None:
            bq = torch.cat([b1, b2], 0).float()
    y = mm(x, wq, bias=bq, out_dtype=out_dtype) if product is None else product(x, wq, bq)
    ctx.wT = None
    if _DGRAD_NT and w1.dtype != x.dtype and (n1 + w2.shape[0]) % 64 == 0:
        ctx.wT = PACK.get((w1.reshape(n1, -1), w2.reshape(w2.shape[0], -1)), PK_TRANSPOSE, x.dtype)
    ctx.lc_saved = (x, wq)
    ctx.conf = (n1, tuple(w1.shape), tuple(w2.shape), b1 is not None)
    ctx.wrefs = WGRAD.note_use(*([w1, w2] if b1 is None else [w1, w2, b1, b2]))
    return y


def _linear_cat_bwd(ctx, dyc, x=None, wq=None):
    if x is None:
        x, wq = ctx.saved_tensors[:2]
    n1, s1, s2, has_bias = ctx.conf
    dx = None
    if ctx.needs_input_grad[0]:
        dx = mm(dyc, ctx.wT) if ctx.wT is not None else mm_dgrad(dyc, wq)
    db1 = db2 = None
    grp = WGRAD.begin(ctx.wrefs)
    if has_bias:
        dw, db = mm_wgrad(dyc, x, with_colsum=True, defer=grp)
        db1, db2 = db[:n1], db[n1:]
    else:
        dw = mm_wgrad(dyc, x, defer=grp)
    if grp is not None and not grp["ret"]:
        return dx, None, None, None, None
    return dx, dw[:n1].view(s1), dw[n1:].view(s2), db1, db2


def linear_cat(x, w1, w2, b1=None, b2=None, out_dtype=None):
    shp = x.shape
    y = _LinearCat.apply(x.reshape(-1, shp[-1]), w1, w2, b1, b2, out_dtype)
    return y.view(*shp[:-1], y.shape[-1])


def _pixel_rows(x, rows, Cc, ld):
    if ld == Cc and x.is_contiguous():
        return x.view(rows, Cc)
    return x.as_strided((rows, Cc), (ld, 1), x.storage_offset())


def conv1x1_cat(x, w1, w2, b1=None, b2=None, out_dtype=None):
    B, H, W, Cc, ld = _nhwc(x)
    xm = _pixel_rows(x, B * H * W, Cc, ld)
    y = _LinearCat.apply(xm, w1, w2, b1, b2, out_dtype)
    return y.view(B, H, W, y.shape[-1])


class _FAPMProject(torch.autograd.Function):

    @staticmethod
    def forward(ctx, x, ws, wp, bs, bp, wf, bf):
        B, H, W, Cc, ld = _nhwc(x)
        rows = B * H * W
        R = ws.shape[0]
        xm = x.as_strided((rows, Cc), (ld, 1), x.storage_offset())
        dt = x.dtype
        wq = PACK.get((ws.reshape(R, -1), wp.reshape(R, -1)), PK_CAST, dt)
        if wq is None:
            wq = torch.cat([ws.reshape(R, -1), wp.reshape(R, -1)], 0).to(dt)
        bq = None
        if bs is not None:
            bq = PACK.get((bs, bp), PK_CAST, torch.float32)
            if bq is None:
                bq = torch.cat([bs, bp], 0).float()
        wfq = PACK.get(wf.reshape(2 * R, -1), PK_CAST, dt)
        if wfq is None:
            wfq = wf.reshape(2 * R, -1).to(dt)
        ctx.wqT = ctx.wfT = None
        if _DGRAD_NT and ws.dtype != dt and (2 * R) % 64 == 0:
            ctx.wqT = PACK.get((ws.reshape(R, -1), wp.reshape(R, -1)), PK_TRANSPOSE, dt)
            ctx.wfT = PACK.get(wf.reshape(2 * R, -1), PK_TRANSPOSE, dt)
        ctx.wrefs = (WGRAD.note_use(*([ws] if bs is None else [ws, bs])), WGRAD.note_use(*([wp] if bp is None else [wp, bp])),
                     WGRAD.note_use(*([wf] if bf is None else [wf, bf])))
        z2 = mm(xm, wq, bias=bq)
        gb = mm(z2[:, :R], wfq, bias=_f32(bf))
        z = torch.empty((rows, R), dtype=dt, device=x.device)
        _lib.check(_lib.lib().du_film_fwd(_code(dt), _p(gb), _p(z2), _p(z), rows, R, _st()), "du_film_fwd")
        ctx.save_for_backward(xm, wq, wfq, z2, gb)
        ctx.conf = (R, tuple(ws.shape), tuple(wp.shape), tuple(wf.shape), bs is not None, bf is not None, (B, H, W, Cc))
        return z.view(B, H, W, R)

    @staticmethod
    def backward(ctx, dz):
        xm, wq, wfq, z2, gb = ctx.saved_tensors
        R, s_ws, s_wp, s_wf, has_b, has_bf, (B, H, W, Cc) = ctx.conf
        rows = xm.shape[0]
        dt = xm.dtype
        dz = dz.contiguous().view(rows, R)
        dgb = torch.empty((rows, 2 * R), dtype=dt, device=dz.device)
        dz2 = torch.empty((rows, 2 * R), dtype=dt, device=dz.device)
        _lib.check(_lib.lib().du_film_bwd(_code(dt), _p(dz), _p(gb), _p(z2), _p(dgb), _p(dz2), rows, R, _st()), "du_film_bwd")
        if ctx.wfT is not None:
            mm(dgb, ctx.wfT, out=dz2[:, :R])
        else:
            mm_dgrad(dgb, wfq, out=dz2[:, :R])
        g_s, g_p, g_f = (WGRAD.begin(r) for r in ctx.wrefs)
        if has_bf:
            dwf, dbf = mm_wgrad(dgb, z2[:, :R], with_colsum=True, defer=g_f if g_f is not None else False)
        else:
            dwf, dbf = mm_wgrad(dgb, z2[:, :R], defer=g_f if g_f is not None else False), None
        if g_f is not None and not g_f["ret"]:
            dwf = dbf = None
        dx = None
        if ctx.needs_input_grad[0]:
            dx = (mm(dz2, ctx.wqT) if ctx.wqT is not None else mm_dgrad(dz2, wq)).view(B, H, W, Cc)
        dbs = dbp = None
        if g_s is None and g_p is None:
            if has_b:
                dw, db = mm_wgrad(dz2, xm, with_colsum=True)
                dbs, dbp = db[:R], db[R:]
            else:
                dw = mm_wgrad(dz2, xm)
            dws, dwp = dw[:R], dw[R:]
        else:
            rs = mm_wgrad(dz2[:, :R], xm, with_colsum=has_b, defer=g_s if g_s is not None else False)
            rp = mm_wgrad(dz2[:, R:], xm, with_colsum=has_b, defer=g_p if g_p is not None else False)
            (dws, dbs), (dwp, dbp) = (rs, rp) if has_b else ((rs, None), (rp, None))
            if g_s is not None and not g_s["ret"]:
                dws = dbs = None
            if g_p is not None and not g_p["ret"]:
                dwp = dbp = None
        return (dx, None if dws is None else dws.view(s_ws), None if dwp is None else dwp.view(s_wp), dbs, dbp,
                None if dwf is None else dwf.view(s_wf), dbf)


def fapm_project(x, ws, wp, bs, bp, wf, bf):
    return _FAPMProject.apply(x, ws, wp, bs, bp, wf, bf)


def conv1x1(x, w, bias=None, out_dtype=None):
    B, H, W, Cc, ld = _nhwc(x)
    xm = _pixel_rows(x, B * H * W, Cc, ld)
    y = _Linear.apply(xm, w.view(w.shape[0], -1), bias, None, None, 0, out_dtype)
    return y.view(B, H, W, w.shape[0])


class _ConvT2x2(torch.autograd.Function):

    @staticmethod
    def forward(ctx, x, w, bias, residual=None):
        B, H, W, Cin, ld = _nhwc(x)
        Cout = w.shape[1]
        wp = PACK.get(w, PK_CONVT_FWD, x.dtype)
        if wp is None:
            wp = w.permute(2, 3, 1, 0).reshape(4 * Cout, Cin).to(x.dtype).contiguous()
        out = torch.empty((B, 2 * H, 2 * W, Cout), dtype=x.dtype, device=x.device)
        _, _, _, _, ldc = _nhwc(out)
        b4 = None
        if bias is not None:
            b4 = PACK.get((bias, bias, bias, bias), PK_CAST, torch.float32)
            if b4 is None:
                b4 = _f32(bias).repeat(4)
        ldr = 0
        if residual is not None:
            Br, Hr, Wr, Cr, ldr = _nhwc(residual)
            assert (Br, Hr, Wr, Cr) == (B, 2 * H, 2 * W, Cout) and residual.dtype == x.dtype
        gemm_raw(dtype=_code(x.dtype), out_dtype=_code(out.dtype), a_mode=PLAIN_ROW, b_mode=PLAIN_ROW, M=B * H * W,
                 N=4 * Cout, K=Cin, A=x.data_ptr(), lda=ld, B=wp.data_ptr(), ldb=Cin, Cmat=out.data_ptr(), ldc=ldc,
                 bias=_dp(b4), residual=_dp(residual), ldr=ldr, store_mode=STORE_PIXEL_SHUFFLE2, ps=(H, W, Cout))
        ctx.save_for_backward(x, w)
        ctx.has_bias = bias is not None
        ctx.has_res = residual is not None
        ctx.wrefs = WGRAD.note_use(*([w] if bias is None else [w, bias]))
        return out

    @staticmethod
    def backward(ctx, dy):
        x, w = ctx.saved_tensors
        B, H, W, Cin, ld = _nhwc(x)
        Cout = w.shape[1]
        if not (dy.stride(3) == 1 and dy.stride(1) == dy.shape[2] * dy.stride(2)):
            dy = dy.contiguous()
        dx = dw = db = None
        g, _, lddy, _ = _geom(dy, 2, 2, 2, 0, H, W, 0)
        if ctx.needs_input_grad[0]:
            wd = PACK.get(w, PK_CONVT_DGRAD, dy.dtype)
            if wd is None:
                wd = w.permute(0, 2, 3, 1).reshape(Cin, 4 * Cout).to(dy.dtype).contiguous()
            dx = torch.empty((B, H, W, Cin), dtype=dy.dtype, device=dy.device)
            gemm_raw(dtype=_code(dy.dtype), out_dtype=_code(dx.dtype), a_mode=IM2COL_ROW, b_mode=PLAIN_ROW, M=B * H * W,
                     N=Cin, K=4 * Cout, A=dy.data_ptr(), lda=lddy, B=wd.data_ptr(), ldb=4 * Cout, Cmat=dx.data_ptr(),
                     ldc=Cin, geom=g)
        want_db = ctx.has_bias and ctx.needs_input_grad[2]
        queued = None
        if ctx.needs_input_grad[1] and dy.dtype == torch.bfloat16 and _pow2(W) and (_WGRAD_COLSUM or not want_db):
            grp = WGRAD.begin(ctx.wrefs)
            if grp is not None:
                queued = _queue_conv_wgrad(grp, 2, x, ld, [(dy, lddy, Cout)], B, H, W, Cin, tuple(w.shape), want_db)
                if queued is None:
                    WGRAD.abort(grp)
                elif not grp["ret"]:
                    queued = (None, None)
        if queued is not None:
            dw, db = queued
            want_db = False
        elif ctx.needs_input_grad[1]:
            gw = ZEROS.zeros((Cin, 4 * Cout), dy.device)
            npix = B * H * W
            tiles = ((Cin + 127) // 128) * ((4 * Cout + 127) // 128)
            kw = dict(dtype=_code(dy.dtype), out_dtype=DU_F32, a_mode=PLAIN_COL, b_mode=IM2COL_COL, M=Cin, N=4 * Cout,
                      K=npix, A=x.data_ptr(), lda=ld, B=dy.data_ptr(), ldb=lddy, Cmat=gw.data_ptr(), ldc=4 * Cout,
                      split_k=_split_for(tiles, npix, 1024), geom=g)
            if want_db and _WGRAD_COLSUM and dy.dtype == torch.bfloat16 and gemm_route(**kw) in (1, 5):
                db = ZEROS.zeros((Cout,), dy.device)
                gemm_raw(b_colsum=db.data_ptr(), **kw)
                want_db = False
            else:
                gemm_raw(**kw)
            dw = gw.view(Cin, 2, 2, Cout).permute(0, 3, 1, 2).contiguous()
        if want_db:
            Bo, Ho, Wo, Co, ldo = _nhwc(dy)
            db = colsum(dy.as_strided((Bo * Ho * Wo, Co), (ldo, 1), dy.storage_offset()))
        return dx, dw, db, (dy if ctx.has_res else None)


def conv_transpose2x2(x, w, bias=None, residual=None):
    return _ConvT2x2.apply(x, w, bias, residual)


def chan_stats(x, G):
    B, H, W, Cc, ld = _nhwc(x)
    P = (B // G) * H * W
    sums = torch.empty((G, Cc, 2), dtype=torch.float32, device=x.device)
    ws, n = _reduce_ws(x.dtype, G, P, Cc, x.device)
    _lib.check(_lib.lib().du_chan_stats(_code(x.dtype), _p(x), ld, _p(sums), G, P, Cc, _p(ws), n, _st()), "du_chan_stats")
    return sums, P


def _norm_fwd(x, mean, rstd, w, b, G, P, act):
    B, H, W, Cc, ld = _nhwc(x)
    y = torch.empty((B, H, W, Cc), dtype=x.dtype, device=x.device)
    _lib.check(_lib.lib().du_norm_act_fwd(_code(x.dtype), _p(x), ld, _p(y), Cc, _p(mean), _p(rstd), _p(w), _p(b), G, P, Cc, act,
                                          _st()), "du_norm_act_fwd")
    return y


class _NormAct(torch.autograd.Function):

    @staticmethod
    def forward(ctx, x, w, b, kind, act, eps, training, running_mean, running_var, momentum, group, stats_part=None):
        B, H, W, Cc, ld = _nhwc(x)
        wf, bf = _f32(w), _f32(b)
        use_batch = (kind == "in") or training
        count = None
        if use_batch:
            G = B if kind == "in" else 1
            P = (B // G) * H * W
            count = float(P)
# ... 7 lines not shown
                if stats_part is not None:
                    _lib.check(L.du_strip_finalize_norm(_p(stats_part), None, G, stats_part.shape[0] // G, Cc, count, eps, _p(mean), _p(rstd),
                                                        rm, rv, float(momentum), _st()), "du_strip_finalize_norm")
                else:
                    ws, n = _reduce_ws(x.dtype, G, P, Cc, x.device)
                    _lib.check(L.du_chan_stats_norm(_code(x.dtype), _p(x), ld, None, G, P, Cc, _p(ws), n, count, eps, _p(mean), _p(rstd),
                                                    rm, rv, float(momentum), _st()), "du_chan_stats_norm")
            else:
                if stats_part is not None:
                    sums = torch.empty((G, Cc, 2), dtype=torch.float32, device=x.device)
                    _lib.check(L.du_strip_finalize(_p(stats_part), _p(sums), G, stats_part.shape[0] // G, Cc, _st()), "du_strip_finalize")
                else:
                    sums, P = chan_stats(x, G)
                sums = sums.clone()
                _small_all_reduce(sums, group, "syncbn_fwd")
                count = count * torch.distributed.get_world_size(group)
                _lib.check(L.du_norm_stats_finalize(_p(sums), count, eps, _p(mean), _p(rstd), G, Cc, rm, rv, float(momentum), _st()),
                           "du_norm_stats_finalize")
        else:
            G, P = 1, B * H * W
            mean = running_mean.float().view(1, Cc)
            rstd = torch.rsqrt(running_var.float() + eps).view(1, Cc)
        mean, rstd = mean.contiguous(), rstd.contiguous()
        y = _norm_fwd(x, mean, rstd, wf, bf, G, P, act)
        ctx.save_for_backward(x, mean, rstd, wf, bf)
        ctx.conf = (G, P, act, use_batch, count, kind, group)
        return y

    @staticmethod
    def backward(ctx, dy):
        x, mean, rstd, wf, bf = ctx.saved_tensors
        G, P, act, use_batch, count, kind, group = ctx.conf
        B, H, W, Cc, ld = _nhwc(x)
        dy = dy.contiguous()
        L = _lib.lib()
        bs = torch.empty((G, Cc, 2), dtype=torch.float32, device=x.device)
        ws, n = _reduce_ws(x.dtype, G, P, Cc, x.device)
        dw = torch.empty(Cc, dtype=torch.float32, device=x.device)
        db = torch.empty(Cc, dtype=torch.float32, device=x.device)
        _lib.check(L.du_norm_act_bwd_stats_grads(_code(x.dtype), _p(x), ld, _p(dy), Cc, _p(mean), _p(rstd), _p(wf), _p(bf), _p(bs), _p(dw),
                                                 _p(db), G, P, Cc, act, _p(ws), n, _st()), "du_norm_act_bwd_stats_grads")
        bsr = bs
        if kind == "bn" and use_batch and group is not None and sync_active(group):
            bsr = bs.clone()
            _small_all_reduce(bsr, group, "syncbn_bwd")
        dx = torch.empty((B, H, W, Cc), dtype=x.dtype, device=x.device)
        _lib.check(L.du_norm_act_bwd_dx(_code(x.dtype), _p(x), ld, _p(dy), Cc, _p(dx), Cc, _p(mean), _p(rstd), _p(wf), _p(bf),
                                        _p(bsr), G, P, Cc, act, float(count or 0.0), 1 if use_batch else 0, _st()),
                   "du_norm_act_bwd_dx")
        return dx, dw, db, None, None, None, None, None, None, None, None, None


def norm_act(x, w, b, kind, act=ACT_NONE, eps=1e-5, training=True, running_mean=None, running_var=None, momentum=0.1,
             group=None, stats_part=None):
    return _NormAct.apply(x, w, b, kind, act, eps, training, running_mean, running_var, momentum, group, stats_part)


class _SyncBNMulti(torch.autograd.Function):

    @staticmethod
    def forward(ctx, group, act, n, *args):
        xs, ws, bs = args[:n], args[n:2 * n], args[2 * n:3 * n]
        mods = args[3 * n]
        L = _lib.lib()
        world = torch.distributed.get_world_size(group)
        geo = [_nhwc(x) for x in xs]
        offs, tot = [], 0
        for (_, _, _, Cc, _) in geo:
            offs.append(tot)
            tot += 2 * Cc
        flat = torch.empty(tot, dtype=torch.float32, device=xs[0].device)
        for x, (B, H, W, Cc, ld), o in zip(xs, geo, offs):
            wsb, nws = _reduce_ws(x.dtype, 1, B * H * W, Cc, x.device)
            _lib.check(L.du_chan_stats(_code(x.dtype), _p(x), ld, C.c_void_p(flat.data_ptr() + 4 * o), 1, B * H * W, Cc, _p(wsb), nws, _st()),
                       "du_chan_stats")
        _small_all_reduce(flat, group, "syncbn_fwd")
        ys, saved = [], []
        for j, (x, (B, H, W, Cc, ld), o) in enumerate(zip(xs, geo, offs)):
            eps, rm, rv, mom = mods[j]
            count = float(B * H * W * world)
            mean = torch.empty((1, Cc), dtype=torch.float32, device=x.device)
            rstd = torch.empty((1, Cc), dtype=torch.float32, device=x.device)
            _lib.check(L.du_norm_stats_finalize(C.c_void_p(flat.data_ptr() + 4 * o), count, eps, _p(mean), _p(rstd), 1, Cc,
                                                _p(rm) if rm is not None else None, _p(rv) if rm is not None else None, float(mom), _st()),
                       "du_norm_stats_finalize")
            wf, bf = _f32(ws[j]), _f32(bs[j])
            ys.append(_norm_fwd(x, mean, rstd, wf, bf, 1, B * H * W, act))
            saved += [x, mean, rstd, wf, bf]
        ctx.save_for_backward(*saved)
        ctx.conf = (group, act, n, world, geo, offs, tot)
        return tuple(ys)

    @staticmethod
    def backward(ctx, *dys):
        group, act, n, world, geo, offs, tot = ctx.conf
        sv = ctx.saved_tensors
        L = _lib.lib()
        dev = sv[0].device
        flat = torch.empty(tot, dtype=torch.float32, device=dev)
        dws, dbs, dyc = [], [], []
        for j in range(n):
            x, mean, rstd, wf, bf = sv[5 * j:5 * j + 5]
            B, H, W, Cc, ld = geo[j]
            dy = dys[j].contiguous()
            dyc.append(dy)
            wsb, nws = _reduce_ws(x.dtype, 1, B * H * W, Cc, dev)
            bsj = C.c_void_p(flat.data_ptr() + 4 * offs[j])
            _lib.check(L.du_norm_act_bwd_stats(_code(x.dtype), _p(x), ld, _p(dy), Cc, _p(mean), _p(rstd), _p(wf), _p(bf), bsj, 1, B * H * W,
                                               Cc, act, _p(wsb), nws, _st()), "du_norm_act_bwd_stats")
            dw = torch.empty(Cc, dtype=torch.float32, device=dev)
            db = torch.empty(Cc, dtype=torch.float32, device=dev)
            _lib.check(L.du_norm_param_grads(bsj, _p(dw), _p(db), 1, Cc, _st()), "du_norm_param_grads")
            dws.append(dw); dbs.append(db)
        _small_all_reduce(flat, group, "syncbn_bwd")
        dxs = []
        for j in range(n):
            x, mean, rstd, wf, bf = sv[5 * j:5 * j + 5]
            B, H, W, Cc, ld = geo[j]
            dx = torch.empty((B, H, W, Cc), dtype=x.dtype, device=dev)
            _lib.check(L.du_norm_act_bwd_dx(_code(x.dtype), _p(x), ld, _p(dyc[j]), Cc, _p(dx), Cc, _p(mean), _p(rstd), _p(wf), _p(bf),
                                            C.c_void_p(flat.data_ptr() + 4 * offs[j]), 1, B * H * W, Cc, act, float(B * H * W * world), 1, _st()),
                       "du_norm_act_bwd_dx")
            dxs.append(dx)
        return (None, None, None, *dxs, *dws, *dbs, None)


def sync_bn_multi(xs, bns, act, group):
    n = len(xs)
    mods = [(bn.eps, bn.running_mean, bn.running_var, bn.momentum if bn.momentum is not None else 0.1) for bn in bns]
    return list(_SyncBNMulti.apply(group, act, n, *xs, *[bn.weight for bn in bns], *[bn.bias for bn in bns], mods))


def layernorm_raw(x2d, w, b, eps, out_dtype, want_stats=False, out=None):
    rows, D, ld = _rows2d(x2d)
    if out is None:
        y = torch.empty((rows, D), dtype=out_dtype, device=x2d.device)
    else:
        y = out
        assert y.shape == (rows, D) and y.dtype == out_dtype and y.is_contiguous()
    mean = rstd = None
    if want_stats:
        mean = torch.empty(rows, dtype=torch.float32, device=x2d.device)
        rstd = torch.empty(rows, dtype=torch.float32, device=x2d.device)
    _lib.check(_lib.lib().du_layernorm_fwd(_code(x2d.dtype), _code(out_dtype), _p(x2d), ld, _p(w), _p(b), _p(y), D, _p(mean),
                                           _p(rstd), rows, D, eps, _st()), "du_layernorm_fwd")
    return y, mean, rstd


class _LayerNorm(torch.autograd.Function):

    @staticmethod
    def forward(ctx, x, w, b, eps, with_res):
        xc = x.contiguous()
        wf, bf = _f32(w), _f32(b)
        y, mean, rstd = layernorm_raw(xc.view(-1, xc.shape[-1]), wf, bf, eps, xc.dtype, True)
        ctx.save_for_backward(xc, wf, mean, rstd)
        ctx.with_res = with_res
        ctx.set_materialize_grads(False)
        if with_res:
            return y.view(x.shape), xc.view(x.shape).view_as(xc)
        return y.view(x.shape)

    @staticmethod
    def backward(ctx, dy, dres=None):
        xc, wf, mean, rstd = ctx.saved_tensors
        D = xc.shape[-1]
        if dy is None:
            return dres, None, None, None, None
        dyc = dy.contiguous()
        dx = torch.empty_like(xc)
        dwdb = torch.empty((2, D), dtype=torch.float32, device=xc.device)
        ws, n = _reduce_ws(xc.dtype, 1, xc.numel() // D, D, xc.device)
        dr = None
        if dres is not None:
            dr = dres.contiguous()
            if dr.dtype != xc.dtype:
                dr = cast(dr, xc.dtype)
        _lib.check(_lib.lib().du_layernorm_bwd(_code(xc.dtype), _p(xc), _p(dyc), _p(wf), _p(mean), _p(rstd), _p(dx), _p(dwdb),
                                               xc.numel() // D, D, _p(ws), n, _p(dr), _st()), "du_layernorm_bwd")
        return dx, dwdb[0], dwdb[1], None, None


def layer_norm(x, w, b, eps):
    return _LayerNorm.apply(x, w, b, eps, False)


def layer_norm_res(x, w, b, eps):
    return _LayerNorm.apply(x, w, b, eps, True)


def msda_forward_raw(value, shapes, lsi, loc, attn):
    _req(value, shapes, lsi, loc, attn)
    N, S, M, D = value.shape
    _, Lq, _, L, P, _ = loc.shape
    out = torch.empty((N, Lq, M * D), dtype=value.dtype, device=value.device)
    e0 = PROFILE.start() if PROFILE is not None else None
    _lib.check(_lib.lib().du_msda_forward(_code(value.dtype), _p(value), _p(shapes), _p(lsi), _p(loc), _p(attn), _p(out), N, S, M, D,
                                          L, Lq, P, _st()), "du_msda_forward")
    if PROFILE is not None:
        PROFILE.stop("msda_fwd<gather>", e0, 8.0 * N * Lq * M * L * P * D,
                     float(value.numel() * value.element_size() + loc.numel() * 4 + attn.numel() * 4 + out.numel() * out.element_size()))
    return out


def msda_backward_raw(value, shapes, lsi, loc, attn, grad_out, gv_like_value=False):
    _req(value, shapes, lsi, loc, attn, grad_out)
    N, S, M, D = value.shape
    _, Lq, _, L, P, _ = loc.shape
    gl = torch.empty(loc.shape, dtype=torch.float32, device=value.device)
    ga = torch.empty(attn.shape, dtype=torch.float32, device=value.device)
    n = int(_lib.lib().du_msda_bwd_ws_elems(N, S, M, D, L, Lq, P))
    ws = torch.empty(max(n, 1), dtype=torch.float32, device=value.device)
    e0 = PROFILE.start() if PROFILE is not None else None

    def _prof(gv):
        if PROFILE is not None:
            PROFILE.stop("msda_bwd<gather>", e0, 24.0 * N * Lq * M * L * P * D,
                         float(value.numel() * value.element_size() + loc.numel() * 8 + attn.numel() * 8
                               + grad_out.numel() * grad_out.element_size() + gv.numel() * gv.element_size()))
    if gv_like_value and value.dtype == torch.bfloat16:
        gvb = torch.empty((N, S, M, D), dtype=torch.bfloat16, device=value.device)
        rc = _lib.lib().du_msda_backward_bf16gv(_p(value), _p(shapes), _p(lsi), _p(loc), _p(attn), _p(grad_out), _p(gvb), _p(gl), _p(ga),
                                                N, S, M, D, L, Lq, P, _p(ws), n, _st())
        if rc == 0:
            _prof(gvb)
            return gvb, gl, ga
        if rc != -2:
            _lib.check(rc, "du_msda_backward_bf16gv")
    gv = torch.empty((N, S, M, D), dtype=torch.float32, device=value.device)
    _lib.check(_lib.lib().du_msda_backward(_code(value.dtype), _p(value), _p(shapes), _p(lsi), _p(loc), _p(attn), _p(grad_out), _p(gv),
                                           _p(gl), _p(ga), N, S, M, D, L, Lq, P, _p(ws), n, _st()), "du_msda_backward")
    _prof(gv)
    return gv, gl, ga


class _MSDA(torch.autograd.Function):

    @staticmethod
    def forward(ctx, value, shapes, lsi, loc, attn):
        value, loc, attn = value.contiguous(), loc.contiguous(), attn.contiguous()
        out = msda_forward_raw(value, shapes, lsi, loc, attn)
        ctx.save_for_backward(value, shapes, lsi, loc, attn)
        return out

    @staticmethod
    def backward(ctx, go):
        value, shapes, lsi, loc, attn = ctx.saved_tensors
        gv, gl, ga = msda_backward_raw(value, shapes, lsi, loc, attn, go.contiguous(), gv_like_value=True)
        return (gv if gv.dtype == value.dtype else gv.to(value.dtype)), None, None, gl, ga


def msda(value, shapes, lsi, loc, attn):
    return _MSDA.apply(value, shapes, lsi, loc, attn)


class _MSDAPrep(torch.autograd.Function):

    @staticmethod
    def forward(ctx, raw, ref, Lq, M, P, Hs, Ws):
        rows, ncol, ld = _rows2d(raw)
        assert ncol == M * P * 3
        loc = torch.empty((rows, M, P, 2), dtype=torch.float32, device=raw.device)
        attn = torch.empty((rows, M, P), dtype=torch.float32, device=raw.device)
        _lib.check(_lib.lib().du_msda_prep(_code(raw.dtype), _p(raw), ld, _p(ref), _p(loc), _p(attn), rows, Lq, M, P, Hs, Ws, _st()),
                   "du_msda_prep")
        ctx.save_for_backward(attn)
        ctx.conf = (M, P, Hs, Ws, raw.dtype, ncol)
        return loc, attn

    @staticmethod
    def backward(ctx, gloc, gattn):
        (attn,) = ctx.saved_tensors
        M, P, Hs, Ws, dt, ncol = ctx.conf
        rows = attn.shape[0]
        graw = torch.empty((rows, ncol), dtype=dt, device=attn.device)
        _lib.check(_lib.lib().du_msda_prep_bwd(_code(dt), _p(attn), _p(gloc.contiguous()), _p(gattn.contiguous()), _p(graw), ncol, rows,
                                               M, P, Hs, Ws, _st()), "du_msda_prep_bwd")
        return graw, None, None, None, None, None, None


def msda_prep(raw, ref, Lq, M, P, Hs, Ws):
    return _MSDAPrep.apply(raw, ref, Lq, M, P, Hs, Ws)


_MSDA_PREP_FUSED = _ab_env("DINOUNET_MSDA_PREP_FUSED", "1") == "1"


class _OffsetsPrep(torch.autograd.Function):

    @staticmethod
    def forward(ctx, x, w1, w2, b1, b2, ref, Lq, M, P, Hs, Ws):
        rows = x.shape[0]
        ncol = M * P * 3
        loc = torch.empty((rows, M, P, 2), dtype=torch.float32, device=x.device)
        attn = torch.empty((rows, M, P), dtype=torch.float32, device=x.device)

        def product(xm, wq, bq):
            _, K, lda = _rows2d(xm)
            Nw, _, ldb = _rows2d(wq)
            if _MSDA_PREP_FUSED and P == 4 and xm.dtype == torch.bfloat16 and Nw == ncol:
                kw = dict(dtype=DU_BF16, out_dtype=DU_F32, a_mode=PLAIN_ROW, b_mode=PLAIN_ROW, M=rows, N=Nw, K=K, A=xm.data_ptr(), lda=lda,
                          B=wq.data_ptr(), ldb=ldb, Cmat=loc.data_ptr(), ldc=Nw, bias=_dp(bq), store_mode=STORE_MSDA_PREP, ps=(Hs, Ws, Lq),
                          rope=(ref.data_ptr(), None, 0, 1.0), c2=attn.data_ptr())
                if gemm_route(**kw) == 3:
                    gemm_raw(**kw)
                    return None
            raw = mm(xm, wq, bias=bq, out_dtype=torch.float32)
            _, _, ld = _rows2d(raw)
            _lib.check(_lib.lib().du_msda_prep(_code(raw.dtype), _p(raw), ld, _p(ref), _p(loc), _p(attn), rows, Lq, M, P, Hs, Ws, _st()),
                       "du_msda_prep")
            return None

        assert w1.shape[0] + w2.shape[0] == ncol
        _linear_cat_fwd(ctx, x, w1, w2, b1, b2, torch.float32, product=product)
        xs, wq = ctx.lc_saved
        ctx.lc_saved = None
        ctx.save_for_backward(xs, wq, attn)
        ctx.prep = (M, P, Hs, Ws, ncol)
        return loc, attn

    @staticmethod
    def backward(ctx, gloc, gattn):
        x, wq, attn = ctx.saved_tensors
        M, P, Hs, Ws, ncol = ctx.prep
        rows = attn.shape[0]
        graw = torch.empty((rows, ncol), dtype=x.dtype, device=attn.device)
        _lib.check(_lib.lib().du_msda_prep_bwd(_code(x.dtype), _p(attn), _p(gloc.contiguous()), _p(gattn.contiguous()), _p(graw), ncol, rows,
                                               M, P, Hs, Ws, _st()), "du_msda_prep_bwd")
        return (*_linear_cat_bwd(ctx, graw, x, wq), None, None, None, None, None, None)


def offsets_prep(x, w1, w2, b1, b2, ref, Lq, M, P, Hs, Ws):
    return _OffsetsPrep.apply(x.reshape(-1, x.shape[-1]), w1, w2, b1, b2, ref, Lq, M, P, Hs, Ws)


_LN_BWD_PROD = _ab_env("DINOUNET_LN_BWD_PROD", "1") == "1"


class _SubCtx:

    def save_for_backward(self, *ts):
        self.saved_tensors = ts

    def set_materialize_grads(self, v):
        pass


def layernorm_bwd_prod_plan(xc, G, wT, dx, dres):
    if wT is None or G.dim() != 2 or wT.dim() != 2 or G.stride(1) != 1 or wT.stride(1) != 1 or G.shape[1] != wT.shape[1]:
        return None
    if not (xc.is_contiguous() and dx.is_contiguous() and (dres is None or dres.is_contiguous())) or wT.shape[0] != xc.shape[-1]:
        return None
    if G.dtype != xc.dtype or wT.dtype != xc.dtype or xc.dtype not in (torch.bfloat16, torch.float32):
        return None
    D = xc.shape[-1]
    out = (C.c_int64 * 6)()
    rc = _lib.lib().du_layernorm_bwd_prod_plan(_code(xc.dtype), _p(xc), _p(G), G.stride(0), _p(wT), wT.stride(0), G.shape[1], _p(dx), _p(dres),
                                               xc.numel() // D, D, out, 6)
    return list(out) if rc == 6 and out[0] == 1 else None


def _ln_bwd_of_product(ln_saved, G, wT, wq, dres):
    xc, wf, mean, rstd = ln_saved
    D = xc.shape[-1]
    rows = xc.numel() // D
    dx = torch.empty_like(xc)
    dwdb = torch.empty((2, D), dtype=torch.float32, device=xc.device)
    dr = None
    if dres is not None:
        dr = dres.contiguous()
        if dr.dtype != xc.dtype:
            dr = cast(dr, xc.dtype)
    L = _lib.lib()
    plan = layernorm_bwd_prod_plan(xc, G, wT, dx, dr) if _LN_BWD_PROD else None
    if plan is not None:
        K = G.shape[1]
        ws = torch.empty(max(plan[4], 1), dtype=torch.float32, device=xc.device)
        e0 = PROFILE.start() if PROFILE is not None else None
        _lib.check(L.du_layernorm_bwd_prod(_code(xc.dtype), _p(xc), _p(G), G.stride(0), _p(wT), wT.stride(0), K, _p(wf), _p(mean), _p(rstd),
                                           _p(dx), _p(dwdb), rows, D, _p(ws), plan[4], _p(dr), _st()), "du_layernorm_bwd_prod")
        if PROFILE is not None:
            PROFILE.stop(f"layernorm_bwd_prod<K{K}>", e0, 2.0 * rows * D * K,
                         float(xc.element_size() * (rows * D * (3 if dr is not None else 2) + rows * K)))
        return dx, dwdb[0], dwdb[1]
    dy = mm(G, wT) if wT is not None else mm_dgrad(G, wq)
    ws, n = _reduce_ws(xc.dtype, 1, rows, D, xc.device)
    _lib.check(L.du_layernorm_bwd(_code(xc.dtype), _p(xc), _p(dy), _p(wf), _p(mean), _p(rstd), _p(dx), _p(dwdb), rows, D, _p(ws), n, _p(dr),
                                  _st()), "du_layernorm_bwd")
    return dx, dwdb[0], dwdb[1]


class _LayerNormLinear(torch.autograd.Function):

    @staticmethod
    def forward(ctx, x, lnw, lnb, eps, w, bias):
        ln, li = _SubCtx(), _SubCtx()
        y, xres = _LayerNorm.forward(ln, x, lnw, lnb, eps, True)
        h = _Linear.forward(li, y.view(-1, y.shape[-1]), w, bias, None, None, 0, None)
        ctx.save_for_backward(*ln.saved_tensors, *li.saved_tensors[:2])
        ctx.wT, ctx.wrefs, ctx.has_bias = li.wT, li.wrefs, li.has_bias
        ctx.set_materialize_grads(False)
        return h, xres

    @staticmethod
    def backward(ctx, dh, dres=None):
        xc, wf, mean, rstd, y, wq = ctx.saved_tensors
        if dh is None:
            return dres, None, None, None, None, None
        G = dh if dh.stride(1) == 1 else dh.contiguous()
        if G.dtype != y.dtype:
            G = cast(G, y.dtype)
        li = _SubCtx()
        li.saved_tensors = (y, wq, None)
        li.wT, li.wrefs, li.has_bias, li.has_res, li.rs_rows = ctx.wT, ctx.wrefs, ctx.has_bias, False, 0
        li.needs_input_grad = (False, ctx.needs_input_grad[4], ctx.needs_input_grad[5])
        _, dw, db, *_ = _Linear.backward(li, G)
        dx, dlw, dlb = _ln_bwd_of_product((xc, wf, mean, rstd), G, ctx.wT, wq, dres)
        return dx, dlw, dlb, None, dw, db


def layer_norm_linear(x, lnw, lnb, eps, w, bias=None):
    if not x.is_cuda:
        f, xres = layer_norm_res(x, lnw, lnb, eps)
        return linear(f, w, bias), xres
    h, xres = _LayerNormLinear.apply(x, lnw, lnb, eps, w, bias)
    return h.view(*x.shape[:-1], w.shape[0]), xres


class _LayerNormOffsetsPrep(torch.autograd.Function):

    @staticmethod
    def forward(ctx, x, lnw, lnb, eps, w1, w2, b1, b2, ref, Lq, M, P, Hs, Ws):
        ln, op = _SubCtx(), _SubCtx()
        y, xres = _LayerNorm.forward(ln, x, lnw, lnb, eps, True)
        loc, attn = _OffsetsPrep.forward(op, y.view(-1, y.shape[-1]), w1, w2, b1, b2, ref, Lq, M, P, Hs, Ws)
        ctx.save_for_backward(*ln.saved_tensors, *op.saved_tensors)
        ctx.wT, ctx.wrefs, ctx.conf, ctx.prep = op.wT, op.wrefs, op.conf, op.prep
        ctx.set_materialize_grads(False)
        return loc, attn, xres

    @staticmethod
    def backward(ctx, gloc, gattn, dres=None):
        xc, wf, mean, rstd, y, wq, attn = ctx.saved_tensors
        if gloc is None and gattn is None:
            return (dres,) + (None,) * 13
        if gloc is None:
            gloc = torch.zeros((*attn.shape, 2), dtype=torch.float32, device=attn.device)
        if gattn is None:
            gattn = torch.zeros_like(attn)
        M, P, Hs, Ws, ncol = ctx.prep
        rows = attn.shape[0]
        graw = torch.empty((rows, ncol), dtype=y.dtype, device=attn.device)
        _lib.check(_lib.lib().du_msda_prep_bwd(_code(y.dtype), _p(attn), _p(gloc.contiguous()), _p(gattn.contiguous()), _p(graw), ncol, rows,
                                               M, P, Hs, Ws, _st()), "du_msda_prep_bwd")
        op = _SubCtx()
        op.wT, op.wrefs, op.conf = ctx.wT, ctx.wrefs, ctx.conf
        op.needs_input_grad = (False,)
        _, dw1, dw2, db1, db2 = _linear_cat_bwd(op, graw, y, wq)
        dx, dlw, dlb = _ln_bwd_of_product((xc, wf, mean, rstd), graw, ctx.wT, wq, dres)
        return dx, dlw, dlb, None, dw1, dw2, db1, db2, None, None, None, None, None, None


def layer_norm_offsets_prep(x, lnw, lnb, eps, w1, w2, b1, b2, ref, Lq, M, P, Hs, Ws):
    if not x.is_cuda:
        q, xres = layer_norm_res(x, lnw, lnb, eps)
        return (*offsets_prep(q, w1, w2, b1, b2, ref, Lq, M, P, Hs, Ws), xres)
    return _LayerNormOffsetsPrep.apply(x, lnw, lnb, eps, w1, w2, b1, b2, ref, Lq, M, P, Hs, Ws)


def _dwconv_fwd(ctx, x, w, bias, geom, act):
    x = x.contiguous()
    Cc = w.shape[0]
    wf = _f32(w).view(Cc, 9)
    y = torch.empty_like(x)
    z = torch.empty_like(x) if act != ACT_NONE else None
    ld, bs, B, H, W, pyramid = geom
    _lib.check(_lib.lib().du_dwconv3x3_fwd(_code(x.dtype), _p(x), _p(wf), _p(_f32(bias)), _p(y), _p(z), ld, bs, B, H, W, Cc, pyramid, act, _st()),
               "du_dwconv3x3_fwd")
    ctx.save_for_backward(x, wf, z)
    ctx.conf = (geom, act, bias is not None)
    return y


def _dwconv_bwd(ctx, dy):
    x, wf, z = ctx.saved_tensors
    (ld, bs, B, H, W, pyramid), act, has_bias = ctx.conf
    Cc = wf.shape[0]
    L = _lib.lib()
    code = _code(x.dtype)
    dy = dy.contiguous()
    dz = torch.empty_like(dy) if act != ACT_NONE else None
    dx = torch.empty_like(x)
    dw = torch.empty((Cc, 9), dtype=torch.float32, device=x.device)
    db = torch.empty(Cc, dtype=torch.float32, device=x.device) if has_bias else None
    n = int(L.du_dwconv3x3_bwd_ws_elems(code, ld, bs, B, H, W, Cc, pyramid, act))
    ws = torch.empty(max(n, 1), dtype=torch.float32, device=x.device)
    _lib.check(L.du_dwconv3x3_bwd(code, _p(z), _p(dy), _p(x), _p(wf), _p(dx), _p(dw), _p(db), _p(dz), ld, bs, B, H, W, Cc, pyramid, act,
                                  _p(ws), n, _st()), "du_dwconv3x3_bwd")
    return dx, dw.view(Cc, 1, 3, 3), db


class _DWConv(torch.autograd.Function):

    @staticmethod
    def forward(ctx, x, w, bias, act):
        B, H, W, Cc = x.shape
        return _dwconv_fwd(ctx, x, w, bias, (Cc, H * W * Cc, B, H, W, 0), act)

    @staticmethod
    def backward(ctx, dy):
        return (*_dwconv_bwd(ctx, dy), None)


def dwconv3x3(x, w, bias=None, act=ACT_NONE):
    return _DWConv.apply(x, w, bias, act)


class _DWConvTokens(torch.autograd.Function):

    @staticmethod
    def forward(ctx, x, w, bias, H, W, act):
        B, N, Cc = x.shape
        return _dwconv_fwd(ctx, x, w, bias, (Cc, N * Cc, B, H, W, 1), act)

    @staticmethod
    def backward(ctx, dy):
        return (*_dwconv_bwd(ctx, dy), None, None, None)


def dwconv_tokens(x, w, bias, H, W, act=ACT_GELU):
    B, N, Cc = x.shape
    assert N == 21 * ((H * W) // 4) and H % 2 == 0 and W % 2 == 0, (N, H, W)
    return _DWConvTokens.apply(x, w, bias, H, W, act)


class _MaxPool(torch.autograd.Function):
    @staticmethod
    def forward(ctx, x):
        x = x.contiguous()
        B, H, W, Cc = x.shape
        Ho, Wo = (H - 1) // 2 + 1, (W - 1) // 2 + 1
        y = torch.empty((B, Ho, Wo, Cc), dtype=x.dtype, device=x.device)
        idx = torch.empty((B, Ho, Wo, Cc), dtype=torch.uint8, device=x.device)
        _lib.check(_lib.lib().du_maxpool3x3s2_fwd(_code(x.dtype), _p(x), _p(y), _p(idx), B, H, W, Cc, _st()), "du_maxpool3x3s2_fwd")
        ctx.save_for_backward(idx)
        ctx.shape = (B, H, W, Cc, x.dtype)
        return y

    @staticmethod
    def backward(ctx, dy):
        (idx,) = ctx.saved_tensors
        B, H, W, Cc, dt = ctx.shape
        dx = torch.empty((B, H, W, Cc), dtype=dt, device=dy.device)
        _lib.check(_lib.lib().du_maxpool3x3s2_bwd(_code(dt), _p(idx), _p(dy.contiguous()), _p(dx), B, H, W, Cc, _st()),
                   "du_maxpool3x3s2_bwd")
        return dx


def maxpool3x3s2(x):
    return _MaxPool.apply(x)


class _BilinearAdd(torch.autograd.Function):

    @staticmethod
    def forward(ctx, src, base):
        B, Hs, Ws, Cc, lds = _nhwc(src)
        Bo, Ho, Wo, Co, ldb = _nhwc(base)
        out = torch.empty((Bo, Ho, Wo, Co), dtype=base.dtype, device=base.device)
        _lib.check(_lib.lib().du_bilinear_add_fwd(_code(src.dtype), _code(base.dtype), _p(src), lds, _p(base), ldb, _p(out), Co, B, Hs,
                                                  Ws, Ho, Wo, Cc, _st()), "du_bilinear_add_fwd")
        return out

    @staticmethod
    def backward(ctx, dy):
        return None, dy


def bilinear_add(src, base):
    return _BilinearAdd.apply(src, base)


class _BilinearResize(torch.autograd.Function):

    @staticmethod
    def forward(ctx, x, Ho, Wo):
        B, Hs, Ws, Cc, lds = _nhwc(x)
        out = torch.empty((B, Ho, Wo, Cc), dtype=x.dtype, device=x.device)
        _lib.check(_lib.lib().du_bilinear_add_fwd(_code(x.dtype), _code(x.dtype), _p(x), lds, None, 0, _p(out), Cc, B, Hs, Ws, Ho, Wo,
                                                  Cc, _st()), "du_bilinear_add_fwd")
        ctx.geo = (B, Hs, Ws, Ho, Wo, Cc)
        return out

    @staticmethod
    def backward(ctx, dy):
        B, Hs, Ws, Ho, Wo, Cc = ctx.geo
        dy = dy.contiguous()
        dx = torch.empty((B, Hs, Ws, Cc), dtype=dy.dtype, device=dy.device)
        _lib.check(_lib.lib().du_bilinear_resize_bwd(_code(dy.dtype), _p(dy), Cc, _p(dx), Cc, B, Hs, Ws, Ho, Wo, Cc, _st()),
                   "du_bilinear_resize_bwd")
        return dx, None, None


def bilinear_resize(x, size):
    return _BilinearResize.apply(x, int(size[0]), int(size[1]))


class _SqueezeExcite(torch.autograd.Function):

    @staticmethod
    def forward(ctx, x, w1, b1, w2, b2, shortcut):
        B, H, W, Cc, ld = _nhwc(x)
        P = H * W
        R = w1.shape[0]
        L = _lib.lib()
        w1f, b1f, w2f, b2f = _f32(w1.reshape(R, Cc)), _f32(b1), _f32(w2.reshape(Cc, R)), _f32(b2)
        sums, _ = chan_stats(x, B)
        hidden = torch.empty((B, R), dtype=torch.float32, device=x.device)
        gate = torch.empty((B, Cc), dtype=torch.float32, device=x.device)
        _lib.check(L.du_se_gate_fwd(_p(sums), 1.0 / P, _p(w1f), _p(b1f), _p(w2f), _p(b2f), _p(hidden), _p(gate), B, Cc, R, _st()),
                   "du_se_gate_fwd")
        y = torch.empty((B, H, W, Cc), dtype=x.dtype, device=x.device)
        lds = 0
        if shortcut is not None:
            Bs, Hs, Ws, Cs, lds = _nhwc(shortcut)
            assert (Bs, Hs, Ws, Cs) == (B, H, W, Cc) and shortcut.dtype == x.dtype
        _lib.check(L.du_se_scale_fwd(_code(x.dtype), _p(x), ld, _p(gate), _p(shortcut), lds, _p(y), Cc, B, P, Cc, _st()), "du_se_scale_fwd")
        ctx.save_for_backward(x, sums, hidden, gate, w1f, w2f)
        ctx.shapes = (w1.shape, w2.shape, shortcut is not None)
        return y

    @staticmethod
    def backward(ctx, dy):
        x, sums, hidden, gate, w1f, w2f = ctx.saved_tensors
        w1s, w2s, has_sc = ctx.shapes
        B, H, W, Cc, ld = _nhwc(x)
        P = H * W
        R = w1f.shape[0]
        L = _lib.lib()
        dy = dy.contiguous()
        dsum = torch.empty((B, Cc, 2), dtype=torch.float32, device=x.device)
        ws, n = _reduce_ws(x.dtype, B, P, Cc, x.device)
        _lib.check(L.du_chan_dot(_code(x.dtype), _p(dy), Cc, _p(x), ld, _p(dsum), B, P, Cc, _p(ws), n, _st()), "du_chan_dot")
        dpool = torch.empty((B, Cc), dtype=torch.float32, device=x.device)
        dw1 = torch.empty((R, Cc), dtype=torch.float32, device=x.device)
        db1 = torch.empty(R, dtype=torch.float32, device=x.device)
        dw2 = torch.empty((Cc, R), dtype=torch.float32, device=x.device)
        db2 = torch.empty(Cc, dtype=torch.float32, device=x.device)
        _lib.check(L.du_se_gate_bwd(_p(dsum), _p(sums), 1.0 / P, _p(gate), _p(hidden), _p(w1f), _p(w2f), _p(dpool), _p(dw1), _p(db1),
                                    _p(dw2), _p(db2), B, Cc, R, _st()), "du_se_gate_bwd")
        dx = torch.empty((B, H, W, Cc), dtype=x.dtype, device=x.device)
        _lib.check(L.du_se_scale_bwd(_code(x.dtype), _p(dy), Cc, _p(gate), _p(dpool), _p(dx), Cc, B, P, Cc, _st()), "du_se_scale_bwd")
        return dx, dw1.view(w1s), db1, dw2.view(w2s), db2, (dy if has_sc else None)


def squeeze_excite(x, w1, b1, w2, b2, shortcut=None):
    return _SqueezeExcite.apply(x, w1, b1, w2, b2, shortcut)


class _DiceCE(torch.autograd.Function):

    @staticmethod
    def forward(ctx, logits, target, smooth, group):
        logits = logits.float().contiguous()
        B, K, H, W = logits.shape
        HW = H * W
        tgt = target.reshape(B, HW)
        if tgt.dtype != torch.int64:
            tgt = tgt.long()
        tgt = tgt.contiguous()
        L = _lib.lib()
        n = int(L.du_dice_ce_ws_elems(B, K, HW))
        if n <= 0:
            raise RuntimeError(f"dinounet_hip: fused Dice+CE supports 2..8 classes, got {K}")
        ws = torch.empty(n, dtype=torch.float32, device=logits.device)
        sums = torch.empty(1 + 3 * (K - 1), dtype=torch.float32, device=logits.device)
        _lib.check(L.du_dice_ce_sums(_p(logits), _p(tgt), _p(sums), B, K, HW, _p(ws), n, _st()), "du_dice_ce_sums")
        mult = 1.0
        if group is not None and torch.distributed.is_initialized():
            _small_all_reduce(sums[1:], group, "dice_sums")
            mult = float(torch.distributed.get_world_size(group))
        loss = torch.empty(1, dtype=torch.float32, device=logits.device)
        coef = torch.empty(2 * (K - 1), dtype=torch.float32, device=logits.device)
        _lib.check(L.du_dice_ce_finish(_p(sums), _p(loss), _p(coef), K, B * HW, float(smooth), mult, _st()), "du_dice_ce_finish")
        ctx.save_for_backward(logits, tgt, coef)
        return loss.view(())

    @staticmethod
    def backward(ctx, go):
        logits, tgt, coef = ctx.saved_tensors
        B, K, H, W = logits.shape
        dl = torch.empty_like(logits)
        gof = go.float().contiguous()
        _lib.check(_lib.lib().du_dice_ce_bwd(_p(logits), _p(tgt), _p(coef), _p(gof), _p(dl), B, K, H * W, _st()), "du_dice_ce_bwd")
        return dl, None, None, None


def dice_ce_loss(logits, target, smooth=1e-5, group=None):
    _req(logits, target)
# ... 380 lines not shown
```

### include/dinounet_hip.h

```cpp
#ifndef DINOUNET_HIP_H
#define DINOUNET_HIP_H

#include <stdint.h>

#ifdef __cplusplus
extern "C" {
#endif

#define DU_OK 0
#define DU_ERR_BAD_ARG (-1)
#define DU_ERR_UNSUPPORTED (-2)
#define DU_ERR_LAUNCH (-3)

#define DU_F32 0
#define DU_BF16 1

#define DU_PLAIN_ROW 0
#define DU_PLAIN_COL 1
#define DU_IM2COL_ROW 2
#define DU_IM2COL_COL 3

#define DU_ACT_NONE 0
#define DU_ACT_GELU 1
#define DU_ACT_RELU 2
#define DU_ACT_LEAKY 3
#define DU_ACT_SWIGLU 4

#define DU_STORE_PLAIN 0
#define DU_STORE_SLABS 4
#define DU_STORE_QKV_HEADS 5
#define DU_STORE_MSDA_PREP 6
#define DU_STORE_TAPS 3
#define DU_STORE_QKV_ROPE 2
#define DU_STORE_PIXEL_SHUFFLE2 1

typedef struct {
  const void* p2;
  int64_t ld2;
  int32_t C1;
  int32_t Hi, Wi;
  int32_t C;
  int32_t KH, KW, stride, pad;
  int32_t Ho, Wo;
  int32_t transposed;
} du_conv_geom;

typedef struct {
  int32_t dtype;
  int32_t out_dtype;
  int32_t a_mode, b_mode;
  int32_t M, N, K;
  const void* A; int64_t lda; int64_t a_batch_stride;
  const void* B; int64_t ldb; int64_t b_batch_stride;
  void* C; int64_t ldc; int64_t c_batch_stride;
  int32_t batch;
  int32_t split_k;
  float alpha;
  const float* bias;
  int32_t act;
  const float* gamma;
  const float* row_scale; int32_t rs_rows;
  const void* residual; int64_t ldr;
  int32_t store_mode;
  int32_t ps_H, ps_W, ps_C;
  du_conv_geom geom;
  float* ws; int64_t ws_elems;
  const float* rope_sin; const float* rope_cos; int32_t rope_prefix; float rope_qscale;
  float* a_colsum;
  float* b_colsum;
  float* C2;
  void* ks_ws;
  int64_t ks_ws_bytes;
} du_gemm_args;

int du_gemm(const du_gemm_args* args, void* stream);
int64_t du_gemm_ws_elems(const du_gemm_args* args);
int64_t du_gemm_ks_ws_bytes(const du_gemm_args* args);
int du_gemm_route(const du_gemm_args* args);
int du_gemm_plan_describe(const du_gemm_args* args, int64_t* out, int n);

typedef struct du_tn_job {
  const void* A; int64_t lda;
  const void* B; int64_t ldb;
  float* C; int64_t ldc;
  float* a_colsum;
  const float* alpha;
  int32_t M, N, K;
  int32_t accumulate;
  float* b_colsum;
  int32_t gather, Hs, Ws, Cb, taps, inner, inner_total, c_off;
} du_tn_job;
int du_gemm_tn_group_legal(const du_tn_job* job);
int du_gemm_tn_group(const du_tn_job* jobs, int njobs, void* stream);

int du_conv3x3_halo(const void* x, int64_t ldx, const void* x2, int64_t ldx2, int C1, int Cin, int Cout, int B, int H, int W,
                    const void* w, const float* bias, void* y, int64_t ldy, float* stats_part, void* stream);
int du_conv3x3_plan_describe(const void* x, int64_t ldx, const void* x2, int64_t ldx2, int C1, int Cin, int Cout, int B, int H, int W,
                             const void* w, const void* y, int64_t ldy, int want_stats, int64_t* out, int n);
int du_conv3x3_halo_parts(int C1, int Cin, int Cout, int B, int H, int W);
int du_conv3x3_strip(const void* x, int64_t ldx, const void* x2, int64_t ldx2, int C1, int Cin, int Cout, int B, int H, int W,
                     const void* w, const float* bias, void* y, int64_t ldy, float* stats_part, void* stream);
int du_conv3x3_wgrad_halo(const void* x, int64_t ldx, const void* x2, int64_t ldx2, int C1, int Cin, int Cout, int B, int H, int W,
                          const void* dy, int64_t lddy, float* part, float* dw, int with_db, void* stream);
int du_conv3x3_wgrad_plan_describe(const void* x, int64_t ldx, const void* x2, int64_t ldx2, int C1, int Cin, int Cout, int B, int H, int W,
                                   const void* dy, int64_t lddy, int64_t* out, int n);
int du_conv3x3_wgrad_halo_blocks(int C1, int Cin, int Cout, int B, int H, int W);
int du_strip_finalize(const float* part, float* out, int G, int strips, int C, void* stream);

int du_qkv_rope_split(int dtype, const void* qkv, void* q, void* k, void* v, const float* sin_t, const float* cos_t,
                      int B, int N, int Npad, int H, int Dh, int prefix, float qscale, void* stream);
int du_qkv_rope_split_rows(int dtype, const void* qkv_rows, void* q, void* k, void* v, const float* sin_t, const float* cos_t, int B, int N,
                           int Npad, int H, int Dh, int prefix, float qscale, int64_t m_begin, int m_count, void* stream);
int du_qkv_rope_inplace(int dtype, void* q, void* k, const float* sin_t, const float* cos_t, int B, int N, int Npad, int H, int Dh,
                        int prefix, float qscale, int64_t m_limit, void* stream);
int du_attention_fwd(const void* q, const void* k, const void* v, void* out, int B, int H, int N, int Npad, int Dh,
                     void* stream);
int du_softmax_rows_f32(float* x, int64_t rows, int cols, int64_t ld, void* stream);

int du_layernorm_fwd(int in_dtype, int out_dtype, const void* x, int64_t ldx, const float* w, const float* b, void* y,
                     int64_t ldy, float* mean_out, float* rstd_out, int64_t rows, int D, float eps, void* stream);
int64_t du_reduce_ws_elems(int dtype, int G, int64_t pix_per_group, int C);
int du_layernorm_bwd(int dtype, const void* x, const void* dy, const float* w, const float* mean, const float* rstd,
                     void* dx, float* dwdb, int64_t rows, int D, float* ws, int64_t ws_elems, const void* dres, void* stream);
int du_layernorm_bwd_prod_plan(int dtype, const void* x, const void* G, int64_t ldg, const void* Wt, int64_t ldw, int K, const void* dx,
                               const void* dres, int64_t rows, int D, int64_t* out, int n);
int du_layernorm_bwd_prod(int dtype, const void* x, const void* G, int64_t ldg, const void* Wt, int64_t ldw, int K, const float* w,
                          const float* mean, const float* rstd, void* dx, float* dwdb, int64_t rows, int D, float* ws, int64_t ws_elems,
                          const void* dres, void* stream);

int du_chan_stats(int dtype, const void* x, int64_t ldx, float* sums, int G, int64_t pix_per_group, int C, float* ws,
                  int64_t ws_elems, void* stream);
int du_colsum(int dtype, const void* x, int64_t ldx, float* out, int64_t rows, int C, float* ws, int64_t ws_elems, void* stream);
int du_chan_dot(int dtype, const void* a, int64_t lda, const void* b, int64_t ldb, float* sums, int G, int64_t pix_per_group, int C,
                float* ws, int64_t ws_elems, void* stream);
int du_norm_stats_finalize(const float* sums, float count, float eps, float* mean, float* rstd, int G, int C, float* run_mean,
                           float* run_var, float momentum, void* stream);
int du_norm_param_grads(const float* bsums, float* dw, float* db, int G, int C, void* stream);
int du_chan_stats_norm(int dtype, const void* x, int64_t ldx, float* sums, int G, int64_t pix_per_group, int C, float* ws, int64_t ws_elems,
                       float count, float eps, float* mean, float* rstd, float* run_mean, float* run_var, float momentum, void* stream);
int du_strip_finalize_norm(const float* part, float* sums, int G, int strips, int C, float count, float eps, float* mean, float* rstd,
                           float* run_mean, float* run_var, float momentum, void* stream);
int du_norm_act_bwd_stats_grads(int dtype, const void* x, int64_t ldx, const void* dy, int64_t lddy, const float* mean, const float* rstd,
                                const float* w, const float* b, float* bsums, float* dw, float* db, int G, int64_t pix_per_group, int C,
                                int act, float* ws, int64_t ws_elems, void* stream);
int du_norm_act_fwd(int dtype, const void* x, int64_t ldx, void* y, int64_t ldy, const float* mean, const float* rstd,
                    const float* w, const float* b, int G, int64_t pix_per_group, int C, int act, void* stream);
int du_norm_act_bwd_stats(int dtype, const void* x, int64_t ldx, const void* dy, int64_t lddy, const float* mean,
                          const float* rstd, const float* w, const float* b, float* bsums, int G, int64_t pix_per_group,
                          int C, int act, float* ws, int64_t ws_elems, void* stream);
int du_norm_act_bwd_dx(int dtype, const void* x, int64_t ldx, const void* dy, int64_t lddy, void* dx, int64_t lddx,
                       const float* mean, const float* rstd, const float* w, const float* b, const float* bsums, int G,
                       int64_t pix_per_group, int C, int act, float count, int use_batch_stats, void* stream);

int du_msda_forward(int dtype, const void* value, const int64_t* spatial_shapes, const int64_t* level_start_index,
                    const float* sampling_loc, const float* attn_weight, void* out, int N, int S, int M, int D, int L,
                    int Lq, int P, void* stream);
int64_t du_msda_bwd_ws_elems(int N, int S, int M, int D, int L, int Lq, int P);
int du_msda_backward(int dtype, const void* value, const int64_t* spatial_shapes, const int64_t* level_start_index,
                     const float* sampling_loc, const float* attn_weight, const void* grad_out, float* grad_value,
                     float* grad_sampling_loc, float* grad_attn_weight, int N, int S, int M, int D, int L, int Lq, int P,
                     float* ws, int64_t ws_elems, void* stream);

int du_msda_forward_f64(const double* value, const int64_t* spatial_shapes, const int64_t* level_start_index, const double* sampling_loc,
                        const double* attn_weight, double* out, int N, int S, int M, int D, int L, int Lq, int P, void* stream);
int du_msda_backward_f64(const double* value, const int64_t* spatial_shapes, const int64_t* level_start_index, const double* sampling_loc,
                         const double* attn_weight, const double* grad_out, double* grad_value, double* grad_sampling_loc,
                         double* grad_attn_weight, int N, int S, int M, int D, int L, int Lq, int P, void* stream);

int du_msda_backward_bf16gv(const void* value, const int64_t* spatial_shapes, const int64_t* level_start_index, const float* sampling_loc,
                            const float* attn_weight, const void* grad_out, void* grad_value_bf16, float* grad_sampling_loc,
                            float* grad_attn_weight, int N, int S, int M, int D, int L, int Lq, int P, float* ws, int64_t ws_elems,
                            void* stream);

int du_msda_prep(int dtype, const void* raw, int64_t ldr, const float* ref, float* loc, float* attn, int64_t rows, int Lq,
                 int M, int P, int Hs, int Ws, void* stream);
int du_msda_prep_bwd(int dtype, const float* attn, const float* gloc, const float* gattn, void* graw, int64_t ldr,
                     int64_t rows, int M, int P, int Hs, int Ws, void* stream);

int du_dwconv3x3_fwd(int dtype, const void* x, const float* w, const float* bias, void* y, void* z, int64_t ld, int64_t bs, int B, int H,
                     int W, int C, int pyramid, int act, void* stream);
int64_t du_dwconv3x3_bwd_ws_elems(int dtype, int64_t ld, int64_t bs, int B, int H, int W, int C, int pyramid, int act);
int du_dwconv3x3_bwd(int dtype, const void* z, const void* dy, const void* x, const float* w, void* dx, float* dw, float* db, void* dz,
                     int64_t ld, int64_t bs, int B, int H, int W, int C, int pyramid, int act, float* ws, int64_t ws_elems, void* stream);
int du_dwconv3x3_plan_describe(int dtype, int64_t ld, int64_t bs, int B, int H, int W, int C, int pyramid, int act, int64_t* out, int n);
int du_maxpool3x3s2_fwd(int dtype, const void* x, void* y, uint8_t* idx, int B, int H, int W, int C, void* stream);
int du_maxpool3x3s2_bwd(int dtype, const uint8_t* idx, const void* dy, void* dx, int B, int H, int W, int C, void* stream);
int du_bilinear_add_fwd(int src_dtype, int dtype, const void* src, int64_t lds_, const void* base, int64_t ldb, void* out,
                        int64_t ldo, int B, int Hs, int Ws, int Ho, int Wo, int C, void* stream);
int du_bilinear_resize_bwd(int dtype, const void* dy, int64_t lddy, void* dx, int64_t lddx, int B, int Hs, int Ws, int Ho, int Wo,
                           int C, void* stream);
int du_act_bwd(int dtype, const void* z, const void* dy, void* dz, int64_t n, int act, void* stream);

int du_se_gate_fwd(const float* sums, float inv_count, const float* W1, const float* b1, const float* W2, const float* b2,
                   float* hidden, float* gate, int B, int C, int R, void* stream);
int du_se_scale_fwd(int dtype, const void* x, int64_t ldx, const float* gate, const void* shortcut, int64_t ldsc, void* y, int64_t ldy,
                    int B, int64_t P, int C, void* stream);
int du_se_gate_bwd(const float* dsum, const float* sums, float inv_count, const float* gate, const float* hidden, const float* W1,
                   const float* W2, float* dpool, float* dW1, float* db1, float* dW2, float* db2, int B, int C, int R, void* stream);
int du_se_scale_bwd(int dtype, const void* dy, int64_t lddy, const float* gate, const float* dpool, void* dx, int64_t lddx, int B,
                    int64_t P, int C, void* stream);

int64_t du_dice_ce_ws_elems(int B, int K, int64_t HW);
int du_dice_ce_sums(const float* logits, const int64_t* target, float* sums, int B, int K, int64_t HW, float* ws, int64_t ws_elems,
                    void* stream);
int du_dice_ce_finish(const float* sums, float* loss, float* coef, int K, int64_t npix, float smooth, float grad_mult, void* stream);
int du_dice_ce_bwd(const float* logits, const int64_t* target, const float* coef, const float* grad_out, float* dlogits, int B, int K,
                   int64_t HW, void* stream);

int64_t du_dice_ce_masked_ws_elems(int B, int K, int64_t HW);
int du_dice_ce_masked_sums(const float* logits, const int64_t* target, float* sums, int B, int K, int64_t HW, int64_t ignore_label,
                           float* ws, int64_t ws_elems, void* stream);
int du_dice_ce_masked_finish(const float* sums, float* loss, float* coef, int K, float smooth, float grad_mult, void* stream);
int du_dice_ce_masked_bwd(const float* logits, const int64_t* target, const float* coef, const float* grad_out, float* dlogits, int B,
                          int K, int64_t HW, int64_t ignore_label, void* stream);

int64_t du_dice_bce_ws_elems(int B, int R, int64_t HW);
int du_dice_bce_sums(const float* logits, const uint8_t* target, float* sums, int B, int R, int64_t HW, int has_ignore, float* ws,
                     int64_t ws_elems, void* stream);
int du_dice_bce_finish(const float* sums, float* loss, float* coef, int R, int has_ignore, float smooth, float grad_mult, void* stream);
int du_dice_bce_bwd(const float* logits, const uint8_t* target, const float* coef, const float* grad_out, float* dlogits, int B, int R,
                    int64_t HW, int has_ignore, void* stream);
int du_labels_to_regions(const int64_t* seg, const int64_t* table, uint8_t* out, int B, int R, int64_t HW, int has_ignore,
                         int64_t ignore_label, void* stream);

int64_t du_val_dice_ce_ws_elems(int B, int K, int64_t HW);
int du_val_dice_ce(const float* logits, const int64_t* target, float* sums, int64_t* counts, int64_t* accum, int B, int K, int64_t HW,
                   float* ws, int64_t ws_elems, void* stream);
int64_t du_val_dice_ce_masked_ws_elems(int B, int K, int64_t HW);
int du_val_dice_ce_masked(const float* logits, const int64_t* target, float* sums, int64_t* counts, int64_t* accum, int B, int K,
                          int64_t HW, int64_t ignore_label, float* ws, int64_t ws_elems, void* stream);
int64_t du_val_dice_bce_ws_elems(int B, int R, int64_t HW);
int du_val_dice_bce(const float* logits, const uint8_t* target, float* sums, int64_t* counts, int64_t* accum, int B, int R, int64_t HW,
                    int has_ignore, float* ws, int64_t ws_elems, void* stream);

int du_film_fwd(int dtype, const void* gb, const void* z2, void* z, int64_t rows, int R, void* stream);
int du_film_bwd(int dtype, const void* dz, const void* gb, const void* z2, void* dgb, void* dz2, int64_t rows, int R, void* stream);

int du_swiglu_pairs(int dtype, const void* u, void* out, int64_t rows, int64_t h, void* stream);
int du_sample_copy(const float* src, float* dst, const int64_t* idx, int k, int64_t n_per_sample, int scatter, void* stream);
int du_cast(int src_dtype, int dst_dtype, const void* src, void* dst, int64_t n, void* stream);
int du_gemm_slab_count(int K, int split_k);
int du_splitk_reduce_bf16(const float* slabs, void* out, int splits, int64_t n, void* stream);
int du_nchw_to_nhwc_pad(int dst_dtype, const float* src, void* dst, int B, int C, int H, int W, int Cpad, void* stream);
int du_nhwc_to_nchw_f32(int src_dtype, const void* src, int64_t ld, float* dst, int B, int C, int H, int W, void* stream);
int du_patchify16(int dst_dtype, const float* src, void* dst, int B, int C, int H, int W, void* stream);

int du_pack_weights(const int64_t* table, const int64_t* bprefix, int n, int64_t nblocks, void* stream);

int du_aug_spatial(const float* data, const float* seg, const float* params, float* data_out, float* seg_out, int B, int C, int Hi, int Wi,
                   int Ho, int Wo, void* stream);
int du_aug_plane_stats(const float* x, float* stats, int planes, int64_t n, void* stream);
int du_aug_noise_mult(float* x, const float* sigma, const float* mult, int planes, int64_t n, int seed, void* stream);
int du_aug_contrast(float* x, const float* factor, const float* stats, int planes, int64_t n, void* stream);
int du_aug_gamma(float* x, const float* gamma, const float* invert, const float* stats, int planes, int64_t n, void* stream);
int du_aug_affine(float* x, const float* a, const float* b, int planes, int64_t n, void* stream);
int du_aug_blur(const float* x, float* y, const float* sigma, int planes, int H, int W, int axis, void* stream);
int du_aug_lowres(const float* x, float* y, const float* zoom, int planes, int H, int W, void* stream);

int du_seg_head_fwd(const void* x, int64_t ldx, const float* w, const float* bias, float* out, int B, int64_t HW, int C, int K, void* stream);
int du_seg_head_bwd_blocks(int B, int64_t HW);
int du_seg_head_bwd(const void* x, int64_t ldx, const float* w, const float* dl, void* dx, int64_t lddx, float* part, float* dwb, int B,
                    int64_t HW, int C, int K, void* stream);

const char* du_version(void);
int du_device_ok(void);
int du_set_option(int key, int value);
int du_debug_attn_probe(uint64_t* host8);
int du_debug_attn_occupancy(int which);
int du_debug_attn_census(uint64_t* host, int n);

int du_window_accumulate(const float* logits, const float* gauss, const int32_t* coords, float* pred, float* npred, int nb, int K,
                         int ph, int pw, int D, int H, int W, void* stream);
int du_window_normalize(float* pred, const float* npred, int K, int64_t n, void* stream);

#define DU_EXPORT_SOFTMAX 0
#define DU_EXPORT_REGIONS 1
int du_export_seg(const float* sums, const float* npred, uint8_t* seg, float* probs, int32_t* flag, int K, int D, int Hp, int Wp, int y0,
                  int x0, int Hc, int Wc, int Ho, int Wo, int D0, int H0, int W0, int bd, int by, int bx, int mode, int64_t region_order,
                  void* stream);
int64_t du_seg_counts_ws_elems(int64_t n, int R);
int du_seg_counts(const uint8_t* pred, const uint8_t* ref, const int64_t* masks, int64_t* counts, int64_t n, int R, int has_ignore,
                  int ignore_label, int32_t* ws, int64_t ws_elems, void* stream);

int du_ensemble_merge(const void* const* members, int M, int elem_size, int K, int64_t n, int mode, int64_t region_order, uint8_t* seg,
                      float* mean, int32_t* flag, void* stream);

int64_t du_clip_sgd_ws_elems(int nblocks);
int du_clip_sgd(const int64_t* table, const int64_t* bprefix, int n_tensors, int nblocks, const float* hyper, float* ws,
                int64_t ws_elems, void* stream);

int64_t du_surface_border_ws_elems(int64_t n, int R);
int du_surface_border(const uint8_t* pred, const uint8_t* ref, const int64_t* masks, uint16_t* bits, int64_t* counts, int D, int H, int W,
                      int R, int32_t* ws, int64_t ws_elems, void* stream);
int64_t du_surface_ws_elems(int D, int H, int W);
int du_surface_field(const uint16_t* bits, double* field, int D, int H, int W, int bit, double sz, double sy, double sx, void* ws,
                     int64_t ws_elems, void* stream);
int du_surface_gather(const uint16_t* bits, int D, int H, int W, int R, int active, double sz, double sy, double sx,
                      const int64_t* seg_off_host, double* dist_sq, double* sqrt_sums, void* ws, int64_t ws_elems, void* stream);

int64_t du_cc_ws_elems(int D, int H, int W, int keep);
int du_cc_label(const uint8_t* seg, int64_t mask_bits, int32_t* ids, int64_t* stats, int D, int H, int W, int32_t* ws, int64_t ws_elems,
                void* stream);
int du_cc_keep_largest(const uint8_t* seg, int64_t mask_bits, int background_label, uint8_t* out, int64_t* stats, int D, int H, int W,
                       int32_t* ws, int64_t ws_elems, void* stream);

#define DU_PRE_F32 0
#define DU_PRE_F64 1
#define DU_PRE_U8 2
#define DU_PRE_I16 3
#define DU_PRE_I32 4
#define DU_PRE_NORM_NONE 0
#define DU_PRE_NORM_RGB 1
#define DU_PRE_NORM_CT 2
#define DU_PRE_NORM_RESCALE 3
#define DU_PRE_NORM_ZSCORE 4
int64_t du_pre_fill_ws_elems(int D, int H, int W);
int du_pre_nonzero_mask(const void* data, int dtype, int C, int D, int H, int W, uint8_t* mask, int32_t* bbox, int32_t* ws,
                        int64_t ws_elems, void* stream);
int du_pre_crop(const void* data, int dtype, const uint8_t* mask, const int16_t* seg, int C, int D, int H, int W, int z0, int y0, int x0,
                int d, int h, int w, int nonzero_label, float* out, int16_t* seg_out, void* stream);
int64_t du_pre_stats_ws_elems(int C, int D, int64_t HW);
int du_pre_plane_stats(const float* img, const int16_t* seg, float* plane_minmax, double* chan_stats, int C, int D, int64_t HW, double* ws,
                       int64_t ws_elems, void* stream);
int du_pre_sq_dev(const float* img, const int16_t* seg, double* chan_stats, int C, int D, int64_t HW, double* ws, int64_t ws_elems,
                  void* stream);
int du_pre_normalize(float* img, const int16_t* seg, const double* chan_stats, int scheme, float p0, float p1, float p2, float p3,
                     int64_t n, void* stream);
int du_pre_resize_cubic(const float* in, float* out, const float* bounds, double* tmp, int P, int H, int W, int Ho, int Wo, void* stream);
int du_pre_resize_seg(const int16_t* in, int16_t* out, int D, int H, int W, int Ho, int Wo, void* stream);

int64_t du_dl_ws_elems(int D, int H, int W, int G);
int du_dl_class_counts(const int16_t* seg, const int64_t* masks, int G, int D, int H, int W, int32_t* ws, int64_t ws_elems, int64_t* totals,
                       void* stream);
int du_dl_select(const int16_t* seg, const int64_t* masks, int G, int g, int D, int H, int W, const int32_t* ws, int64_t ws_elems,
                 const int64_t* ranks, int64_t m, int32_t* out, void* stream);
int du_dl_gather(const int64_t* jobs, int B, int C, int ph, int pw, float* data_out, void* seg_out, int seg_f32, void* stream);

int64_t du_fp_ws_elems(int C, int64_t n);
int du_fp_moments(const float* img, const int16_t* seg, int C, int64_t n, int mode, double* stats, int32_t* ws, int64_t ws_elems,
                  void* stream);
int du_fp_order_stats(const float* img, const int16_t* seg, int C, int64_t n, const int64_t* ranks, int R, float* out, int32_t* ws,
                      int64_t ws_elems, void* stream);
int du_fp_sample(const float* img, const int16_t* seg, int C, int64_t n, const int64_t* ranks, int64_t m, float* out, int32_t* ws,
                 int64_t ws_elems, void* stream);

#ifdef __cplusplus
}
#endif
#endif
```

Before: 327.1 slices/s.

## Add slab GEMM kernel for skinny-N linears with resident weight ring

```diff
diff --git a/dinounet_amd/_build.py b/dinounet_amd/_build.py
--- a/dinounet_amd/_build.py
+++ b/dinounet_amd/_build.py
@@ -6,12 +6,12 @@
 HERE = os.path.dirname(os.path.abspath(__file__))
 CSRC = os.path.join(HERE, "csrc")
 LIB = os.path.join(HERE, "libdinounet_hip.so")
-SOURCES = ["gemm.hip", "gemm_bf16.hip", "gemm_glds.hip", "gemm_p8.hip", "gemm_rk.hip", "gemm_skinny.hip", "conv_halo.hip", "conv_strip.hip", "attention.hip", "norm.hip", "norm_gemm.hip", "msda.hip", "elementwise.hip", "dwconv.hip", "loss.hip", "optim.hip", "augment.hip", "export.hip", "ensemble.hip", "surface.hip", "cc.hip", "preprocess.hip", "dataload.hip", "fingerprint.hip"]
+SOURCES = ["gemm.hip", "gemm_bf16.hip", "gemm_glds.hip", "gemm_p8.hip", "gemm_slab.hip", "gemm_rk.hip", "gemm_skinny.hip", "conv_halo.hip", "conv_strip.hip", "attention.hip", "norm.hip", "norm_gemm.hip", "msda.hip", "elementwise.hip", "dwconv.hip", "loss.hip", "optim.hip", "augment.hip", "export.hip", "ensemble.hip", "surface.hip", "cc.hip", "preprocess.hip", "dataload.hip", "fingerprint.hip"]
 FLAGS = ["--offload-arch=gfx950", "-O3", "-std=c++17", "-fPIC", "-munsafe-fp-atomics", "-fno-gpu-rdc"]
 if os.environ.get("DINOUNET_DEBUG_KNOBS") == "1":
     FLAGS.append("-DDU_DEBUG_KNOBS")
 EXTRA_FLAGS = {"attention.hip": ["-mllvm", "-amdgpu-mfma-vgpr-form"], "conv_strip.hip": ["-mllvm", "-amdgpu-mfma-vgpr-form"]}
-NO_SCRATCH = ("gemm_bf16.hip", "gemm_glds.hip", "gemm_p8.hip", "gemm_rk.hip", "gemm_skinny.hip", "conv_halo.hip", "conv_strip.hip", "attention.hip", "norm_gemm.hip", "surface.hip", "dwconv.hip", "cc.hip", "preprocess.hip", "dataload.hip", "fingerprint.hip", "ensemble.hip")
+NO_SCRATCH = ("gemm_bf16.hip", "gemm_glds.hip", "gemm_p8.hip", "gemm_slab.hip", "gemm_rk.hip", "gemm_skinny.hip", "conv_halo.hip", "conv_strip.hip", "attention.hip", "norm_gemm.hip", "surface.hip", "dwconv.hip", "cc.hip", "preprocess.hip", "dataload.hip", "fingerprint.hip", "ensemble.hip")
 REMARK = "-Rpass-analysis=kernel-resource-usage"
 import re as _re
 _ABLATION = _re.compile(
diff --git a/dinounet_amd/csrc/gemm_epilogue.h b/dinounet_amd/csrc/gemm_epilogue.h
--- /dev/null
+++ b/dinounet_amd/csrc/gemm_epilogue.h
@@ -0,0 +1,161 @@
+#pragma once
+#include "common.h"
+#include "gemm_params.h"
+
+namespace {
+
+template <typename TC> struct Out4p;
+template <> struct Out4p<float> {
+  static __device__ __forceinline__ void load(const float* p, float* v) { float4 t = *(const float4*)p; v[0] = t.x; v[1] = t.y; v[2] = t.z; v[3] = t.w; }
+  static __device__ __forceinline__ void store(float* p, const float* v) { *(float4*)p = make_float4(v[0], v[1], v[2], v[3]); }
+};
+template <> struct Out4p<bf16_t> {
+  static __device__ __forceinline__ void load(const bf16_t* p, float* v) {
+    bf16x4 t = __builtin_bit_cast(bf16x4, *(const uint2*)p);
+#pragma unroll
+    for (int j = 0; j < 4; j++) v[j] = (float)t[j];
+  }
+  static __device__ __forceinline__ void store(bf16_t* p, const float* v) {
+    bf16x4 t;
+#pragma unroll
+    for (int j = 0; j < 4; j++) t[j] = (bf16_t)v[j];
+    *(uint2*)p = __builtin_bit_cast(uint2, t);
+  }
+};
+
+__device__ __forceinline__ void stage_block_f32(const f32x16& a, float* stg, int ldf, int srow, int scol, int lane) {
+  const int hi = lane >> 5;
+#pragma unroll
+  for (int g = 0; g < 4; g++)
+    *(float4*)(stg + srow * ldf + scol + 8 * g + 4 * hi) = make_float4(a[4 * g], a[4 * g + 1], a[4 * g + 2], a[4 * g + 3]);
+}
+
+template <typename TC, int W> struct RowVec;
+template <> struct RowVec<float, 4> {
+  static __device__ __forceinline__ void load(const float* p, float* v) { const float4 t = *(const float4*)p; v[0] = t.x; v[1] = t.y; v[2] = t.z; v[3] = t.w; }
+  static __device__ __forceinline__ void store(float* p, const float* v) { *(float4*)p = make_float4(v[0], v[1], v[2], v[3]); }
+};
+template <> struct RowVec<bf16_t, 4> {
+  static __device__ __forceinline__ void load(const bf16_t* p, float* v) { Out4p<bf16_t>::load(p, v); }
+  static __device__ __forceinline__ void store(bf16_t* p, const float* v) { Out4p<bf16_t>::store(p, v); }
+};
+template <> struct RowVec<bf16_t, 8> {
+  static __device__ __forceinline__ void load(const bf16_t* p, float* v) {
+    const bf16x8 t = __builtin_bit_cast(bf16x8, *(const uint4*)p);
+#pragma unroll
+    for (int j = 0; j < 8; j++) v[j] = (float)t[j];
+  }
+  static __device__ __forceinline__ void store(bf16_t* p, const float* v) {
+    bf16x8 t;
+#pragma unroll
+    for (int j = 0; j < 8; j++) t[j] = (bf16_t)v[j];
+    *(uint4*)p = __builtin_bit_cast(uint4, t);
+  }
+};
+
+template <typename TC, int TBN, int ACT, int W, int NTHR = 512>
+__device__ __forceinline__ void readout_f32(const GemmParams& P, const float* stg, int ldf, int nrows, int mrow0, int n0, TC* Cb, const TC* Rb,
+                                            int tid) {
+  constexpr int CW = TBN / W, U = W == 8 ? 2 : 4;
+  const int total = nrows * CW;
+  for (int v0 = tid; v0 < total; v0 += NTHR * U) {
+    float rr[U][W];
+    bool live[U];
+#pragma unroll
+    for (int u = 0; u < U; u++) {
+      const int v = v0 + u * NTHR;
+      const int row = v / CW, cw = v % CW;
+      const int m = mrow0 + row, n = n0 + cw * W;
+      live[u] = v < total && m < P.M && n < P.N;
+#pragma unroll
+      for (int e = 0; e < W; e++) rr[u][e] = 0.f;
+      if (Rb && live[u]) RowVec<TC, W>::load(Rb + out_offset(P, m, n, P.ldr), rr[u]);
+    }
+#pragma unroll
+    for (int u = 0; u < U; u++) {
+      if (!live[u]) continue;
+      const int v = v0 + u * NTHR;
+      const int row = v / CW, cw = v % CW;
+      const int m = mrow0 + row, n = n0 + cw * W;
+      float o[W];
+#pragma unroll
+      for (int h = 0; h < W / 4; h++) {
+        const float4 tt = *(const float4*)(stg + row * ldf + cw * W + 4 * h);
+        o[4 * h] = tt.x * P.alpha; o[4 * h + 1] = tt.y * P.alpha; o[4 * h + 2] = tt.z * P.alpha; o[4 * h + 3] = tt.w * P.alpha;
+        if (P.bias) {
+          const float4 bb = *(const float4*)(P.bias + n + 4 * h);
+          o[4 * h] += bb.x; o[4 * h + 1] += bb.y; o[4 * h + 2] += bb.z; o[4 * h + 3] += bb.w;
+        }
+      }
+      if constexpr (ACT == DU_ACT_GELU) {
+#pragma unroll
+        for (int e = 0; e < W; e++) o[e] = apply_act(o[e], DU_ACT_GELU);
+      } else if constexpr (ACT < 0) {
+#pragma unroll
+        for (int e = 0; e < W; e++) o[e] = apply_act(o[e], P.act);
+      }
+      if (P.gamma) {
+#pragma unroll
+        for (int h = 0; h < W / 4; h++) {
+          const float4 gg = *(const float4*)(P.gamma + n + 4 * h);
+          o[4 * h] *= gg.x; o[4 * h + 1] *= gg.y; o[4 * h + 2] *= gg.z; o[4 * h + 3] *= gg.w;
+        }
+      }
+      if (P.row_scale) {
+        const float rs = P.row_scale[m / P.rs_rows];
+#pragma unroll
+        for (int e = 0; e < W; e++) o[e] *= rs;
+      }
+#pragma unroll
+      for (int e = 0; e < W; e++) o[e] += rr[u][e];
+      RowVec<TC, W>::store(Cb + out_offset(P, m, n, P.ldc), o);
+    }
+  }
+}
+template <typename TC, int TBN, int NTHR = 512>
+__device__ __forceinline__ void readout_f32_any(const GemmParams& P, const float* stg, int ldf, int nrows, int mrow0, int n0, TC* Cb,
+                                                const TC* Rb, int tid) {
+  if constexpr (sizeof(TC) == 2) {
+    const bool w8 = P.N % 8 == 0 && P.ldc % 8 == 0 && ((((uintptr_t)Cb) & 15) == 0) && (!Rb || (P.ldr % 8 == 0 && ((((uintptr_t)Rb) & 15) == 0))) &&
+                    (P.store_mode == DU_STORE_PLAIN || P.ps_C % 8 == 0);
+    if (w8) {
+      if (P.act == DU_ACT_NONE) readout_f32<TC, TBN, DU_ACT_NONE, 8, NTHR>(P, stg, ldf, nrows, mrow0, n0, Cb, Rb, tid);
+      else readout_f32<TC, TBN, -1, 8, NTHR>(P, stg, ldf, nrows, mrow0, n0, Cb, Rb, tid);
+      return;
+    }
+  }
+  if (P.act == DU_ACT_NONE) readout_f32<TC, TBN, DU_ACT_NONE, 4, NTHR>(P, stg, ldf, nrows, mrow0, n0, Cb, Rb, tid);
+  else if (P.act == DU_ACT_GELU) readout_f32<TC, TBN, DU_ACT_GELU, 4, NTHR>(P, stg, ldf, nrows, mrow0, n0, Cb, Rb, tid);
+  else readout_f32<TC, TBN, -1, 4, NTHR>(P, stg, ldf, nrows, mrow0, n0, Cb, Rb, tid);
+}
+template <int NTHR = 512>
+__device__ __forceinline__ void readout_msda_prep(const GemmParams& P, const float* stg, int ldf, int nrows, int mrow0, int tid) {
+  const int Mh = P.N / 12, Lq = P.ps_C;
+  const float invW = 1.0f / (float)P.ps_W, invH = 1.0f / (float)P.ps_H;
+  float* loc = (float*)P.C;
+  for (int v = tid; v < nrows * Mh; v += NTHR) {
+    const int row = v / Mh, h = v - row * Mh;
+    const int m = mrow0 + row;
+    if (m >= P.M) continue;
+    const int q = m % Lq;
+    const float rx = P.rope_sin[q * 2], ry = P.rope_sin[q * 2 + 1];
+    const float* so = stg + row * ldf + h * 8;
+    const float* sl = stg + row * ldf + Mh * 8 + h * 4;
+    float off[8], lg[4];
+#pragma unroll
+    for (int e = 0; e < 8; e++) off[e] = so[e] + (P.bias ? P.bias[h * 8 + e] : 0.f);
+#pragma unroll
+    for (int e = 0; e < 4; e++) lg[e] = sl[e] + (P.bias ? P.bias[Mh * 8 + h * 4 + e] : 0.f);
+    const float mx = fmaxf(fmaxf(lg[0], lg[1]), fmaxf(lg[2], lg[3]));
+    float ex[4], sm = 0.f;
+#pragma unroll
+    for (int e = 0; e < 4; e++) { ex[e] = expf(lg[e] - mx); sm += ex[e]; }
+    const float inv = 1.f / sm;
+    float* lo = loc + ((long)m * Mh + h) * 8;
+    *(float4*)lo = make_float4(rx + off[0] * invW, ry + off[1] * invH, rx + off[2] * invW, ry + off[3] * invH);
+    *(float4*)(lo + 4) = make_float4(rx + off[4] * invW, ry + off[5] * invH, rx + off[6] * invW, ry + off[7] * invH);
+    *(float4*)(P.C2 + ((long)m * Mh + h) * 4) = make_float4(ex[0] * inv, ex[1] * inv, ex[2] * inv, ex[3] * inv);
+  }
+}
+
+}
diff --git a/dinounet_amd/csrc/gemm_p8.hip b/dinounet_amd/csrc/gemm_p8.hip
--- a/dinounet_amd/csrc/gemm_p8.hip
+++ b/dinounet_amd/csrc/gemm_p8.hip
@@ -2,6 +2,7 @@
 #include <vector>
 #include "common.h"
 #include "gemm_params.h"
+#include "gemm_epilogue.h"
 #include "gemm_plan.h"
 #include "gemm_skinny_body.h"
 
@@ -14,24 +15,6 @@
 constexpr int BUF_B = 4 * HALF_B;
 constexpr int STG_LD = PBN + 4;
 
-template <typename TC> struct Out4p;
-template <> struct Out4p<float> {
-  static __device__ __forceinline__ void load(const float* p, float* v) { float4 t = *(const float4*)p; v[0] = t.x; v[1] = t.y; v[2] = t.z; v[3] = t.w; }
-  static __device__ __forceinline__ void store(float* p, const float* v) { *(float4*)p = make_float4(v[0], v[1], v[2], v[3]); }
-};
-template <> struct Out4p<bf16_t> {
-  static __device__ __forceinline__ void load(const bf16_t* p, float* v) {
-    bf16x4 t = __builtin_bit_cast(bf16x4, *(const uint2*)p);
-#pragma unroll
-    for (int j = 0; j < 4; j++) v[j] = (float)t[j];
-  }
-  static __device__ __forceinline__ void store(bf16_t* p, const float* v) {
-    bf16x4 t;
-#pragma unroll
-    for (int j = 0; j < 4; j++) t[j] = (bf16_t)v[j];
-    *(uint2*)p = __builtin_bit_cast(uint2, t);
-  }
-};
 
 typedef unsigned u32x4_t __attribute__((ext_vector_type(4)));
 template <int N> struct IC { static constexpr int value = N; };
@@ -144,12 +127,6 @@
     const int n = ncol0 + 8 * g + 4 * hi;
     bv[g] = P.bias ? *(const float4*)(P.bias + (n < P.N ? n : 0)) : make_float4(0.f, 0.f, 0.f, 0.f);
   }
-}
-__device__ __forceinline__ void stage_block_f32(const f32x16& a, float* stg, int ldf, int srow, int scol, int lane) {
-  const int hi = lane >> 5;
-#pragma unroll
-  for (int g = 0; g < 4; g++)
-    *(float4*)(stg + srow * ldf + scol + 8 * g + 4 * hi) = make_float4(a[4 * g], a[4 * g + 1], a[4 * g + 2], a[4 * g + 3]);
 }
 template <int TBN, bool QKV = false, int NTHR = 512>
 __device__ __forceinline__ void readout_bf16(const GemmParams& P, const bf16_t* stg, int ldb, int nrows, int mrow0, int n0, int ncols,
@@ -171,88 +148,6 @@
     }
   }
 }
-template <typename TC, int W> struct RowVec;
-template <> struct RowVec<float, 4> {
-  static __device__ __forceinline__ void load(const float* p, float* v) { const float4 t = *(const float4*)p; v[0] = t.x; v[1] = t.y; v[2] = t.z; v[3] = t.w; }
-  static __device__ __forceinline__ void store(float* p, const float* v) { *(float4*)p = make_float4(v[0], v[1], v[2], v[3]); }
-};
-template <> struct RowVec<bf16_t, 4> {
-  static __device__ __forceinline__ void load(const bf16_t* p, float* v) { Out4p<bf16_t>::load(p, v); }
-  static __device__ __forceinline__ void store(bf16_t* p, const float* v) { Out4p<bf16_t>::store(p, v); }
-};
-template <> struct RowVec<bf16_t, 8> {
-  static __device__ __forceinline__ void load(const bf16_t* p, float* v) {
-    const bf16x8 t = __builtin_bit_cast(bf16x8, *(const uint4*)p);
-#pragma unroll
-    for (int j = 0; j < 8; j++) v[j] = (float)t[j];
-  }
-  static __device__ __forceinline__ void store(bf16_t* p, const float* v) {
-    bf16x8 t;
-#pragma unroll
-    for (int j = 0; j < 8; j++) t[j] = (bf16_t)v[j];
-    *(uint4*)p = __builtin_bit_cast(uint4, t);
-  }
-};
-
-template <typename TC, int TBN, int ACT, int W, int NTHR = 512>
-__device__ __forceinline__ void readout_f32(const GemmParams& P, const float* stg, int ldf, int nrows, int mrow0, int n0, TC* Cb, const TC* Rb,
-                                            int tid) {
-  constexpr int CW = TBN / W, U = W == 8 ? 2 : 4;
-  const int total = nrows * CW;
-  for (int v0 = tid; v0 < total; v0 += NTHR * U) {
-    float rr[U][W];
-    bool live[U];
-#pragma unroll
-    for (int u = 0; u < U; u++) {
-      const int v = v0 + u * NTHR;
-      const int row = v / CW, cw = v % CW;
-      const int m = mrow0 + row, n = n0 + cw * W;
-      live[u] = v < total && m < P.M && n < P.N;
-#pragma unroll
-      for (int e = 0; e < W; e++) rr[u][e] = 0.f;
-      if (Rb && live[u]) RowVec<TC, W>::load(Rb + out_offset(P, m, n, P.ldr), rr[u]);
-    }
-#pragma unroll
-    for (int u = 0; u < U; u++) {
-      if (!live[u]) continue;
-      const int v = v0 + u * NTHR;
-      const int row = v / CW, cw = v % CW;
-      const int m = mrow0 + row, n = n0 + cw * W;
-      float o[W];
-#pragma unroll
-      for (int h = 0; h < W / 4; h++) {
-        const float4 tt = *(const float4*)(stg + row * ldf + cw * W + 4 * h);
-        o[4 * h] = tt.x * P.alpha; o[4 * h + 1] = tt.y * P.alpha; o[4 * h + 2] = tt.z * P.alpha; o[4 * h + 3] = tt.w * P.alpha;
-        if (P.bias) {
-          const float4 bb = *(const float4*)(P.bias + n + 4 * h);
-          o[4 * h] += bb.x; o[4 * h + 1] += bb.y; o[4 * h + 2] += bb.z; o[4 * h + 3] += bb.w;
-        }
-      }
-      if constexpr (ACT == DU_ACT_GELU) {
-#pragma unroll
-        for (int e = 0; e < W; e++) o[e] = apply_act(o[e], DU_ACT_GELU);
-      } else if constexpr (ACT < 0) {
-#pragma unroll
-        for (int e = 0; e < W; e++) o[e] = apply_act(o[e], P.act);
-      }
-      if (P.gamma) {
-#pragma unroll
-        for (int h = 0; h < W / 4; h++) {
-          const float4 gg = *(const float4*)(P.gamma + n + 4 * h);
-          o[4 * h] *= gg.x; o[4 * h + 1] *= gg.y; o[4 * h + 2] *= gg.z; o[4 * h + 3] *= gg.w;
-        }
-      }
-      if (P.row_scale) {
-        const float rs = P.row_scale[m / P.rs_rows];
-#pragma unroll
-        for (int e = 0; e < W; e++) o[e] *= rs;
-      }
-#pragma unroll
-      for (int e = 0; e < W; e++) o[e] += rr[u][e];
-      RowVec<TC, W>::store(Cb + out_offset(P, m, n, P.ldc), o);
-    }
-  }
-}
 struct ResidualTile { float4 r[16]; };
 template <int TBN, int NTHR = 512>
 __device__ __forceinline__ void residual_prefetch(const GemmParams& P, const float* Rb, int mrow0, int n0, int tid, ResidualTile& R) {
@@ -294,51 +189,6 @@
       for (int e = 0; e < 4; e++) o[e] *= rs;
     }
     *(float4*)(Cb + (long)m * P.ldc + n) = make_float4(o[0] + R.r[u].x, o[1] + R.r[u].y, o[2] + R.r[u].z, o[3] + R.r[u].w);
-  }
-}
-template <typename TC, int TBN, int NTHR = 512>
-__device__ __forceinline__ void readout_f32_any(const GemmParams& P, const float* stg, int ldf, int nrows, int mrow0, int n0, TC* Cb,
-                                                const TC* Rb, int tid) {
-  if constexpr (sizeof(TC) == 2) {
-    const bool w8 = P.N % 8 == 0 && P.ldc % 8 == 0 && ((((uintptr_t)Cb) & 15) == 0) && (!Rb || (P.ldr % 8 == 0 && ((((uintptr_t)Rb) & 15) == 0))) &&
-                    (P.store_mode == DU_STORE_PLAIN || P.ps_C % 8 == 0);
-    if (w8) {
-      if (P.act == DU_ACT_NONE) readout_f32<TC, TBN, DU_ACT_NONE, 8, NTHR>(P, stg, ldf, nrows, mrow0, n0, Cb, Rb, tid);
-      else readout_f32<TC, TBN, -1, 8, NTHR>(P, stg, ldf, nrows, mrow0, n0, Cb, Rb, tid);
-      return;
-    }
-  }
-  if (P.act == DU_ACT_NONE) readout_f32<TC, TBN, DU_ACT_NONE, 4, NTHR>(P, stg, ldf, nrows, mrow0, n0, Cb, Rb, tid);
-  else if (P.act == DU_ACT_GELU) readout_f32<TC, TBN, DU_ACT_GELU, 4, NTHR>(P, stg, ldf, nrows, mrow0, n0, Cb, Rb, tid);
-  else readout_f32<TC, TBN, -1, 4, NTHR>(P, stg, ldf, nrows, mrow0, n0, Cb, Rb, tid);
-}
-template <int NTHR = 512>
-__device__ __forceinline__ void readout_msda_prep(const GemmParams& P, const float* stg, int ldf, int nrows, int mrow0, int tid) {
-  const int Mh = P.N / 12, Lq = P.ps_C;
-  const float invW = 1.0f / (float)P.ps_W, invH = 1.0f / (float)P.ps_H;
-  float* loc = (float*)P.C;
-  for (int v = tid; v < nrows * Mh; v += NTHR) {
-    const int row = v / Mh, h = v - row * Mh;
-    const int m = mrow0 + row;
-    if (m >= P.M) continue;
-    const int q = m % Lq;
-    const float rx = P.rope_sin[q * 2], ry = P.rope_sin[q * 2 + 1];
-    const float* so = stg + row * ldf + h * 8;
-    const float* sl = stg + row * ldf + Mh * 8 + h * 4;
-    float off[8], lg[4];
-#pragma unroll
-    for (int e = 0; e < 8; e++) off[e] = so[e] + (P.bias ? P.bias[h * 8 + e] : 0.f);
-#pragma unroll
-    for (int e = 0; e < 4; e++) lg[e] = sl[e] + (P.bias ? P.bias[Mh * 8 + h * 4 + e] : 0.f);
-    const float mx = fmaxf(fmaxf(lg[0], lg[1]), fmaxf(lg[2], lg[3]));
-    float ex[4], sm = 0.f;
-#pragma unroll
-    for (int e = 0; e < 4; e++) { ex[e] = expf(lg[e] - mx); sm += ex[e]; }
-    const float inv = 1.f / sm;
-    float* lo = loc + ((long)m * Mh + h) * 8;
-    *(float4*)lo = make_float4(rx + off[0] * invW, ry + off[1] * invH, rx + off[2] * invW, ry + off[3] * invH);
-    *(float4*)(lo + 4) = make_float4(rx + off[4] * invW, ry + off[5] * invH, rx + off[6] * invW, ry + off[7] * invH);
-    *(float4*)(P.C2 + ((long)m * Mh + h) * 4) = make_float4(ex[0] * inv, ex[1] * inv, ex[2] * inv, ex[3] * inv);
   }
 }
 __device__ __forceinline__ bool bf16_simple(const GemmParams& P, const void* Rb) {
diff --git a/dinounet_amd/csrc/gemm_slab.hip b/dinounet_amd/csrc/gemm_slab.hip
--- /dev/null
+++ b/dinounet_amd/csrc/gemm_slab.hip
@@ -0,0 +1,203 @@
+#include "common.h"
+#include "gemm_params.h"
+#include "gemm_epilogue.h"
+#include "gemm_slab_plan.h"
+
+namespace {
+
+typedef __attribute__((address_space(3))) void lds_void;
+template <int N> struct IC { static constexpr int value = N; };
+
+template <typename TC, int NWN>
+__global__ __launch_bounds__(128 * NWN) void gemm_slab_kernel(GemmParams P, int R) {
+  constexpr int NW = 2 * NWN, NTHR = 64 * NW, TBN = 64 * NWN;
+  constexpr int NA = (SLAB_A_TILE / 1024) / NW;
+  constexpr int NB = (TBN * SLAB_BK * 2 / 1024) / NW;
+  constexpr int W_TILE = TBN * SLAB_BK * 2;
+  constexpr int W_BASE = SLAB_A_RING * SLAB_A_TILE;
+  constexpr int LDF = TBN + 4;
+  constexpr int BIAS_OFF = W_BASE + SLAB_W_RING * W_TILE;
+  static_assert(128 * LDF * 4 <= BIAS_OFF, "the staging tile lies inside the rings");
+  extern __shared__ __attribute__((aligned(16))) unsigned char smem[];
+
+  const int tid = threadIdx.x, lane = tid & 63;
+  const int wave = __builtin_amdgcn_readfirstlane(tid >> 6);
+  const int wm = wave / NWN, wn = wave - wm * NWN;
+  const int row0 = blockIdx.x * R;
+  const int live = min(R, P.M - row0);
+  const int nk = P.K / SLAB_BK;
+  float bias_v = 0.f;
+  if (P.bias && tid < TBN) bias_v = P.bias[tid];
+
+  const bf16_t* Ab = (const bf16_t*)P.a.p + (long)row0 * P.a.ld;
+  const bf16_t* Bb = (const bf16_t*)P.b.p;
+  const long abytes = ((long)live * P.a.ld - (P.a.ld - P.K)) * 2;
+  const long bbytes = ((long)P.N * P.b.ld - (P.b.ld - P.K)) * 2;
+  const auto ra = __builtin_amdgcn_make_buffer_rsrc((void*)Ab, 0, (int)abytes, 0x00020000);
+  const auto rb = __builtin_amdgcn_make_buffer_rsrc((void*)Bb, 0, (int)bbytes, 0x00020000);
+
+  const int sw = ((wave & 1) << 2) | (lane >> 4);
+  const int lc = (lane & 7) ^ sw;
+  const unsigned va0 = (unsigned)(wave * 8 + (lane >> 3)) * (unsigned)(P.a.ld * 2) + lc * 16;
+  const unsigned vb0 = (unsigned)(wave * 8 + (lane >> 3)) * (unsigned)(P.b.ld * 2) + lc * 16;
+  const unsigned vastep = (unsigned)(NW * 8) * (unsigned)(P.a.ld * 2), vbstep = (unsigned)(NW * 8) * (unsigned)(P.b.ld * 2);
+
+  auto issue_a = [&](int slot, int kt) {
+    unsigned char* dst = smem + slot * SLAB_A_TILE + wave * 1024;
+    const unsigned soff = (unsigned)kt * (SLAB_BK * 2);
+#pragma unroll
+    for (int i = 0; i < NA; i++)
+      __builtin_amdgcn_raw_ptr_buffer_load_lds(ra, (lds_void*)(dst + i * NW * 1024), 16, va0 + i * vastep, soff, 0, 0);
+  };
+  auto issue_w = [&](int slot, int kt) {
+    unsigned char* dst = smem + W_BASE + slot * W_TILE + wave * 1024;
+    const unsigned soff = (unsigned)kt * (SLAB_BK * 2);
+#pragma unroll
+    for (int i = 0; i < NB; i++)
+      __builtin_amdgcn_raw_ptr_buffer_load_lds(rb, (lds_void*)(dst + i * NW * 1024), 16, vb0 + i * vbstep, soff, 0, 0);
+  };
+
+  int L[4];
+  {
+    const int x = (lane >> 5) ^ ((lane >> 1) & 7);
+#pragma unroll
+    for (int kk = 0; kk < 4; kk++) L[kk] = (lane & 31) * 128 + ((x ^ (2 * kk)) << 4);
+  }
+  const int aoff = wm * SLAB_WAVE_ROWS * 128, boff = W_BASE + wn * 64 * 128;
+
+  f32x16 acc[3][2];
+#pragma unroll
+  for (int b = 0; b < 3; b++)
+#pragma unroll
+    for (int j = 0; j < 2; j++)
+#pragma unroll
+      for (int r = 0; r < 16; r++) acc[b][j][r] = 0.f;
+
+  bf16x8 FA[2][2][3], FB[2][2][2];
+  auto read_half = [&](auto set_c, const unsigned char* sa, const unsigned char* sb) {
+    constexpr int set = decltype(set_c)::value;
+#pragma unroll
+    for (int h = 0; h < 2; h++) {
+#pragma unroll
+      for (int j = 0; j < 2; j++) FB[set][h][j] = *(const bf16x8*)(sb + j * 4096 + L[2 * set + h]);
+#pragma unroll
+      for (int b = 0; b < 3; b++) FA[set][h][b] = *(const bf16x8*)(sa + b * 4096 + L[2 * set + h]);
+    }
+  };
+  auto mma_half = [&](auto set_c) {
+    constexpr int set = decltype(set_c)::value;
+#pragma unroll
+    for (int h = 0; h < 2; h++)
+#pragma unroll
+      for (int b = 0; b < 3; b++)
+#pragma unroll
+        for (int j = 0; j < 2; j++)
+          acc[b][j] = __builtin_amdgcn_mfma_f32_32x32x16_bf16(FB[set][h][j], FA[set][h][b], acc[b][j], 0, 0, 0);
+  };
+
+  issue_w(0, 0);
+  issue_a(0, 0);
+  issue_a(1, 1);
+  issue_w(1, 1);
+  issue_a(2, 2);
+  asm volatile("s_waitcnt vmcnt(%0)" ::"n"(2 * NA + NB) : "memory");
+  __builtin_amdgcn_s_barrier();
+  __builtin_amdgcn_sched_barrier(0);
+  read_half(IC<0>{}, smem + aoff, smem + boff);
+  int aslot = 0;
+  for (int t = 0; t + 1 < nk; t++) {
+    const int anext = aslot == 2 ? 0 : aslot + 1;
+    read_half(IC<1>{}, smem + aslot * SLAB_A_TILE + aoff, smem + (t & 1) * W_TILE + boff);
+    mma_half(IC<0>{});
+    __builtin_amdgcn_sched_barrier(0);
+    if (t + 2 < nk) asm volatile("s_waitcnt vmcnt(%0)" ::"n"(NA) : "memory");
+    else asm volatile("s_waitcnt vmcnt(0)" ::: "memory");
+    asm volatile("s_waitcnt lgkmcnt(0)" ::: "memory");
+    __builtin_amdgcn_s_barrier();
+    __builtin_amdgcn_sched_barrier(0);
+    if (t + 2 < nk) issue_w(t & 1, t + 2);
+    if (t + 3 < nk) issue_a(aslot, t + 3);
+    read_half(IC<0>{}, smem + anext * SLAB_A_TILE + aoff, smem + ((t + 1) & 1) * W_TILE + boff);
+    mma_half(IC<1>{});
+    aslot = anext;
+  }
+  read_half(IC<1>{}, smem + aslot * SLAB_A_TILE + aoff, smem + ((nk - 1) & 1) * W_TILE + boff);
+  mma_half(IC<0>{});
+  mma_half(IC<1>{});
+  __builtin_amdgcn_sched_barrier(0);
+  if (tid < TBN) ((float*)(smem + BIAS_OFF))[tid] = bias_v;
+  asm volatile("s_waitcnt lgkmcnt(0)" ::: "memory");
+  __builtin_amdgcn_s_barrier();
+
+  float* stg = (float*)smem;
+  TC* Cb = (TC*)P.C;
+  GemmParams Q = P;
+  if (P.bias) Q.bias = (const float*)(smem + BIAS_OFF);
+#pragma unroll
+  for (int p = 0; p < 2; p++) {
+    const int nrows = min(128, live - 128 * p);
+    if (p > 0) {
+      asm volatile("s_waitcnt lgkmcnt(0)" ::: "memory");
+      __builtin_amdgcn_s_barrier();
+    }
+#pragma unroll
+    for (int b = 0; b < 3; b++) {
+      const int g = wm * 3 + b;
+      if ((g >> 2) == p) {
+#pragma unroll
+        for (int j = 0; j < 2; j++) stage_block_f32(acc[b][j], stg, LDF, (g & 3) * 32 + (lane & 31), wn * 64 + j * 32, lane);
+      }
+    }
+    asm volatile("s_waitcnt lgkmcnt(0)" ::: "memory");
+    __builtin_amdgcn_s_barrier();
+    if (nrows > 0) {
+      bool done = false;
+      if constexpr (sizeof(TC) == 4) {
+        if (P.store_mode == DU_STORE_MSDA_PREP) { readout_msda_prep<NTHR>(Q, stg, LDF, nrows, row0 + 128 * p, tid); done = true; }
+      }
+      if (!done) readout_f32_any<TC, TBN, NTHR>(Q, stg, LDF, nrows, row0 + 128 * p, 0, Cb, (const TC*)nullptr, tid);
+    }
+  }
+}
+
+template <typename TC, int NWN>
+int launch_slab(const GemmParams& P, const GemmSlabPlan& pl, hipStream_t st) {
+  void (*kfn)(GemmParams, int) = gemm_slab_kernel<TC, NWN>;
+  static bool attr_set = false;
+  if (!attr_set) {
+    if (hipFuncSetAttribute((const void*)kfn, hipFuncAttributeMaxDynamicSharedMemorySize, pl.lds_bytes) != hipSuccess) return DU_ERR_LAUNCH;
+    attr_set = true;
+  }
+  hipLaunchKernelGGL(kfn, dim3(pl.wgs), dim3(128 * NWN), pl.lds_bytes, st, P, pl.R);
+  return du_check_launch();
+}
+
+template <typename TC>
+int launch_slab_n(const GemmParams& P, const GemmSlabPlan& pl, hipStream_t st) {
+  switch (pl.waves_n) {
+    case 4: return launch_slab<TC, 4>(P, pl, st);
+    case 3: return launch_slab<TC, 3>(P, pl, st);
+    case 2: return launch_slab<TC, 2>(P, pl, st);
+    default: return launch_slab<TC, 1>(P, pl, st);
+  }
+}
+
+}
+
+extern "C" int du_gemm_slab_plan(const du_gemm_args* args, int64_t* out, int n) {
+  if (!args || !out || n < 6) return DU_ERR_BAD_ARG;
+  const GemmSlabPlan pl = du_gemm_slab_plan_of(*args);
+  if (pl.rc == DU_ERR_BAD_ARG) return DU_ERR_BAD_ARG;
+  out[0] = pl.rc == DU_OK ? 1 : 0; out[1] = pl.R; out[2] = pl.wgs; out[3] = pl.waves_m; out[4] = pl.waves_n; out[5] = pl.lds_bytes;
+  return 6;
+}
+
+extern "C" int du_gemm_slab(const du_gemm_args* args, void* stream) {
+  if (!args) return DU_ERR_BAD_ARG;
+  const GemmSlabPlan pl = du_gemm_slab_plan_of(*args);
+  if (pl.rc != DU_OK) return pl.rc;
+  const du_gemm_args& a = *args;
+  const GemmParams P = make_params(a, DU_PLAIN_ROW, DU_PLAIN_ROW, SLAB_ROWS, a.N, SLAB_BK);
+  hipStream_t st = (hipStream_t)stream;
+  return a.out_dtype == DU_BF16 ? launch_slab_n<bf16_t>(P, pl, st) : launch_slab_n<float>(P, pl, st);
+}
diff --git a/dinounet_amd/csrc/gemm_slab_plan.h b/dinounet_amd/csrc/gemm_slab_plan.h
--- /dev/null
+++ b/dinounet_amd/csrc/gemm_slab_plan.h
@@ -0,0 +1,45 @@
+#pragma once
+#include "common.h"
+#include "gemm_plan.h"
+
+constexpr int SLAB_WGS = 256;
+constexpr int SLAB_WAVE_ROWS = 96;
+constexpr int SLAB_ROWS = 192;
+constexpr int SLAB_BK = 64;
+constexpr int SLAB_A_TILE = SLAB_ROWS * SLAB_BK * 2;
+constexpr int SLAB_A_RING = 3;
+constexpr int SLAB_W_RING = 2;
+
+struct GemmSlabPlan {
+  int rc;
+  int R;
+  int wgs;
+  int waves_m, waves_n;
+  int lds_bytes;
+};
+
+inline GemmSlabPlan du_gemm_slab_plan_of(const du_gemm_args& a) {
+  GemmSlabPlan p{DU_ERR_UNSUPPORTED, 0, 0, 0, 0, 0};
+  if (!a.A || !a.B || !a.C) { p.rc = DU_ERR_BAD_ARG; return p; }
+  if (a.dtype != DU_BF16 || a.a_mode != DU_PLAIN_ROW || a.b_mode != DU_PLAIN_ROW) return p;
+  if (a.batch != 1 || a.split_k > 1 || a.alpha != 1.0f || a.residual || a.gamma || a.act != DU_ACT_NONE) return p;
+  if (a.N % 64 || a.N < 64 || a.N > 256 || a.K % SLAB_BK || a.K < 512 || a.K > 4096 || a.M <= 0) return p;
+  const int R = ((a.M + SLAB_WGS - 1) / SLAB_WGS + 7) / 8 * 8;
+  if (R <= SLAB_WAVE_ROWS || R > SLAB_ROWS) return p;
+  if (a.lda % 8 || a.ldb % 8 || a.lda < a.K || a.ldb < a.K || (((uintptr_t)a.A) & 15) || (((uintptr_t)a.B) & 15)) return p;
+  if ((long)a.lda * 2 * SLAB_ROWS > 0x7fffffffL || (long)a.ldb * 2 * a.N > 0x7fffffffL) return p;
+  if (a.store_mode == DU_STORE_MSDA_PREP) {
+    if (!p8_legal(a)) return p;
+  } else {
+    if (a.store_mode != DU_STORE_PLAIN || (a.out_dtype != DU_BF16 && a.out_dtype != DU_F32)) return p;
+    if (a.ldc % 4 || a.ldc < a.N || (((uintptr_t)a.C) & 15)) return p;
+    if (a.row_scale && a.rs_rows <= 0) return p;
+  }
+  p.rc = DU_OK;
+  p.R = R;
+  p.wgs = (a.M + R - 1) / R;
+  p.waves_m = SLAB_ROWS / SLAB_WAVE_ROWS;
+  p.waves_n = a.N / 64;
+  p.lds_bytes = SLAB_A_RING * SLAB_A_TILE + SLAB_W_RING * a.N * SLAB_BK * 2 + a.N * 4;
+  return p;
+}
diff --git a/dinounet_amd/ops.py b/dinounet_amd/ops.py
--- a/dinounet_amd/ops.py
+++ b/dinounet_amd/ops.py
@@ -192,7 +192,7 @@
 
 def gemm_raw(*, dtype, out_dtype, a_mode, b_mode, M, N, K, A, lda, B, ldb, Cmat, ldc, batch=1, abs_=0, bbs=0, cbs=0,
              split_k=1, alpha=1.0, bias=None, act=ACT_NONE, gamma=None, row_scale=None, rs_rows=0, residual=None, ldr=0,
-             store_mode=0, ps=(0, 0, 0), geom=None, a_colsum=None, b_colsum=None, rope=None, c2=None, route_only=False):
+             store_mode=0, ps=(0, 0, 0), geom=None, a_colsum=None, b_colsum=None, rope=None, c2=None, route_only=False, args_only=False):
     a = GemmArgs()
     a.dtype, a.out_dtype, a.a_mode, a.b_mode = dtype, out_dtype, a_mode, b_mode
     a.M, a.N, a.K = M, N, K
@@ -214,6 +214,8 @@
     a.C2 = c2
     if rope is not None:
         a.rope_sin, a.rope_cos, a.rope_prefix, a.rope_qscale = rope
+    if args_only:
+        return a
     if route_only:
         return int(_lib.lib().du_gemm_route(C.byref(a)))
     ws = None
@@ -250,6 +252,40 @@
                      2.0 * M * N * K * batch, float(batch) * (M * kin * es + N * K * es + M * N * eo * (2 if residual is not None else 1)))
         return
     _lib.check(_lib.lib().du_gemm(C.byref(a), _st()), "du_gemm")
+
+
+_GEMM_SLAB = _ab_env("DINOUNET_GEMM_SLAB", "1") == "1"
+_GEMM_SLAB_FC1 = _ab_env("DINOUNET_GEMM_SLAB_FC1", "0") == "1"
+SLAB_LAUNCHES = 0
+
+
+def gemm_slab_plan(**kw):
+    a = gemm_raw(args_only=True, **kw)
+    out = (C.c_int64 * 6)()
+    rc = _lib.lib().du_gemm_slab_plan(C.byref(a), out, 6)
+    return list(out) if rc == 6 and out[0] == 1 else None
+
+
+def gemm_slab_raw(**kw):
+    global SLAB_LAUNCHES
+    a = gemm_raw(args_only=True, **kw)
+    e0 = PROFILE.start() if PROFILE is not None else None
+    _lib.check(_lib.lib().du_gemm_slab(C.byref(a), _st()), "du_gemm_slab")
+    SLAB_LAUNCHES += 1
+    if PROFILE is not None:
+        M, N, K = kw["M"], kw["N"], kw["K"]
+        eo = 2 if kw["out_dtype"] == DU_BF16 else 4
+        tag = "gemm_slab_kernel<bf16,linear>"
+        if PROFILE.detail:
+            tag += f" M{M} N{N} K{K}"
+        PROFILE.stop(tag, e0, 2.0 * M * N * K, float(M * K * 2 + N * K * 2 + M * N * eo))
+
+
+def gemm_slab_or_raw(**kw):
+    if _GEMM_SLAB and gemm_slab_plan(**kw) is not None:
+        gemm_slab_raw(**kw)
+    else:
+        gemm_raw(**kw)
 
 
 def set_corun(n):
@@ -387,7 +423,7 @@
 PACK = WeightPack()
 
 def mm(x, w, *, out=None, out_dtype=None, bias=None, act=ACT_NONE, gamma=None, residual=None, row_scale=None,
-       rs_rows=0, alpha=1.0):
+       rs_rows=0, alpha=1.0, slab=False):
     _req(x, w)
     M, K, lda = _rows2d(x)
     N, K2, ldb = _rows2d(w)
@@ -400,10 +436,11 @@
     if residual is not None:
         assert residual.dtype == out.dtype
         ldr = residual.stride(0)
-    gemm_raw(dtype=_code(x.dtype), out_dtype=_code(out.dtype), a_mode=PLAIN_ROW, b_mode=PLAIN_ROW, M=M, N=N, K=K,
-             A=x.data_ptr(), lda=lda, B=w.data_ptr(), ldb=ldb, Cmat=out.data_ptr(), ldc=ldc, alpha=alpha,
-             bias=_dp(bias), act=act, gamma=_dp(gamma), row_scale=_dp(row_scale), rs_rows=rs_rows,
-             residual=_dp(residual), ldr=ldr)
+    (gemm_slab_or_raw if slab else gemm_raw)(
+        dtype=_code(x.dtype), out_dtype=_code(out.dtype), a_mode=PLAIN_ROW, b_mode=PLAIN_ROW, M=M, N=N, K=K,
+        A=x.data_ptr(), lda=lda, B=w.data_ptr(), ldb=ldb, Cmat=out.data_ptr(), ldc=ldc, alpha=alpha,
+        bias=_dp(bias), act=act, gamma=_dp(gamma), row_scale=_dp(row_scale), rs_rows=rs_rows,
+        residual=_dp(residual), ldr=ldr)
     return out
 
 
@@ -1082,7 +1119,8 @@
                 wq = w.to(x.dtype)
             elif wq.dim() != 2:
                 wq = wq.view(w.shape[0], -1)
-        y = mm(x, wq, bias=_f32(bias), residual=residual, row_scale=row_scale, rs_rows=rs_rows, out_dtype=out_dtype)
+        y = mm(x, wq, bias=_f32(bias), residual=residual, row_scale=row_scale, rs_rows=rs_rows, out_dtype=out_dtype,
+               slab=_GEMM_SLAB_FC1 and getattr(ctx, "slab", False))
         ctx.wT = PACK.get(w, PK_TRANSPOSE, x.dtype) if (_DGRAD_NT and w.dtype != x.dtype and w.shape[0] % 64 == 0) else None
         ctx.save_for_backward(x, wq, row_scale)
         ctx.wrefs = WGRAD.note_use(*([w] if bias is None else [w, bias]))
@@ -1107,7 +1145,7 @@
         dx = None
         if ctx.needs_input_grad[0]:
             if ctx.wT is not None:
-                dx = mm(dyc, ctx.wT, row_scale=ks[0], rs_rows=ks[1]) if ks is not None else mm(dyc, ctx.wT)
+                dx = mm(dyc, ctx.wT, row_scale=ks[0], rs_rows=ks[1], slab=True) if ks is not None else mm(dyc, ctx.wT)
             else:
                 dx = mm_dgrad(dyc, wq)
         dw = db = None
@@ -1721,6 +1759,9 @@
                 kw = dict(dtype=DU_BF16, out_dtype=DU_F32, a_mode=PLAIN_ROW, b_mode=PLAIN_ROW, M=rows, N=Nw, K=K, A=xm.data_ptr(), lda=lda,
                           B=wq.data_ptr(), ldb=ldb, Cmat=loc.data_ptr(), ldc=Nw, bias=_dp(bq), store_mode=STORE_MSDA_PREP, ps=(Hs, Ws, Lq),
                           rope=(ref.data_ptr(), None, 0, 1.0), c2=attn.data_ptr())
+                if _GEMM_SLAB and gemm_slab_plan(**kw) is not None:
+                    gemm_slab_raw(**kw)
+                    return None
                 if gemm_route(**kw) == 3:
                     gemm_raw(**kw)
                     return None
@@ -1814,6 +1855,7 @@
     @staticmethod
     def forward(ctx, x, lnw, lnb, eps, w, bias):
         ln, li = _SubCtx(), _SubCtx()
+        li.slab = True
         y, xres = _LayerNorm.forward(ln, x, lnw, lnb, eps, True)
         h = _Linear.forward(li, y.view(-1, y.shape[-1]), w, bias, None, None, 0, None)
         ctx.save_for_backward(*ln.saved_tensors, *li.saved_tensors[:2])
diff --git a/include/dinounet_hip.h b/include/dinounet_hip.h
--- a/include/dinounet_hip.h
+++ b/include/dinounet_hip.h
@@ -79,6 +79,9 @@
 int du_gemm_route(const du_gemm_args* args);
 int du_gemm_plan_describe(const du_gemm_args* args, int64_t* out, int n);
 
+int du_gemm_slab_plan(const du_gemm_args* args, int64_t* out, int n);
+int du_gemm_slab(const du_gemm_args* args, void* stream);
+
 typedef struct du_tn_job {
   const void* A; int64_t lda;
   const void* B; int64_t ldb;
```

Measured after the change: 328.4 slices/s (median of 6 runs). No clear change (+0.4%).
